# fernandezdaniel/MOBOCMF

Hardware: AMD Instinct MI355X
Metric: ELBO steps/sec (MFDGP d=8 M=512 N=8192 S=8) (higher is better)
Workload: dtype f64

## Files before the change

mobocmf_amd/csrc/api.hip:

```cpp
#include "common.h"

int launch_gram_fwd(const GramArgs& g, hipStream_t s);
int launch_gram_bwd(const GramArgs& g, bool want_dx, hipStream_t s);
void gram_grid(const GramArgs& g, dim3* grid);
int launch_sum_partials(const double* part, int64_t P, int64_t stride, double* out, int64_t len, double scale,
                        int accumulate, hipStream_t s);
int launch_potrf(double* A, int64_t ld, int Mp, int M, double* Dinv, double* Ld, int32_t* info, hipStream_t s);
int launch_trtri(const double* L, int64_t ld, int Mp, const double* Dinv, double* Linv, double* T, double* ws,
                 int64_t ws_elems, hipStream_t s);
int launch_pad_tril(const double* src, int64_t lds, int M, double* dst, int Mp, hipStream_t s);
int launch_pad_vec(const double* src, int64_t n, double* dst, int64_t np, hipStream_t s);
int launch_transpose(const double* in, int64_t ldi, double* out, int64_t ldo, int64_t rows, int64_t cols, hipStream_t s);
int launch_gemv_rows(const double* Mat, int64_t ld, const double* vec, double* out, int rows, int64_t cols, double scale,
                     int accumulate, hipStream_t s);
int launch_kl(const double* L, const double* LSp, const double* U, const double* a, int M, int Mp, double* kl,
              double* part, hipStream_t s);
int launch_moments_finish(const double* qpart, const double* mupart, const double* rpart, int nrb, int64_t Np, int64_t N,
                          const double* knn, int branch, double min_var, double* q, double* r, double* varraw,
                          double* mean, double* var, int32_t* zero_word, hipStream_t s);
int launch_moments_bwd_prep(const double* g_mean, const double* g_var, const double* knn, const double* q,
                            const double* varraw, int branch, double min_var, int64_t N, int64_t Np, double* gmu,
                            double* gv, double* gv2, double* cgv, int32_t* nclamped, int zeroed, int32_t* blkact, hipStream_t s);
int launch_reduce_slabs_sym(const double* slabs, int64_t slab_stride, int nslab, int nslab_diag, double* out, int Mp, const int32_t* flag,
                            const double* fallback, hipStream_t s);
int launch_reduce_slabs_sym2(const double* slabs, const double* slabs2, int64_t slab_stride, int nslab, int nslab_diag,
                             double* out, double* out2, int Mp, const int32_t* flag, hipStream_t s);
int launch_add_kl_terms(double* dU, const double* U, double* da, const double* a, const double* gkl, int Mp, hipStream_t s);
int launch_rank1_add(double* X, const double* u, const double* v, int Mp, hipStream_t s);
int launch_dl_from_t2(const double* T2, const double* L, const double* gkl, int M, int Mp, double* dL, hipStream_t s);
int launch_phi(const double* T3, int Mp, double* P, hipStream_t s);
int launch_symmetrize(const double* S, int Mp, double* G, hipStream_t s);
int launch_gls_out(const double* X, const double* LSp, const double* gkl, int M, int Mp, double* gLS, hipStream_t s);
int launch_copy_block(const double* src, int64_t lds, double* dst, int64_t ldd, int64_t rows, int64_t cols, hipStream_t s);
int launch_tril_inplace(double* A, int64_t ld, int n, hipStream_t s);
int launch_mf_combine(const double* Ks, const double* Kn, int64_t ld, const double* s1, const double* s2, const int32_t* l1,
                      const int32_t* l2, const double* ntab, int64_t n1, int64_t n2, double diag, double* out, int64_t ldo,
                      int64_t rows_p, int64_t cols_p, hipStream_t s);
int launch_copy_pad_identity(const double* src, int64_t lds, int n, double* dst, int np, hipStream_t s);
int launch_exact_gp_mll(const double* L, int64_t ld, const double* a, int n, double* mll, hipStream_t s);
int launch_exact_gp_finish(const double* qpart, const double* mupart, int nparts, int64_t ntp, int64_t nt, const double* kss,
                           double* mean, double* var, hipStream_t s);
int launch_mirror_lower(const double* src, int64_t lds, double* dst, int64_t ldd, int64_t row0, int64_t rows, int64_t cols,
                        int64_t n_real, hipStream_t s);
int launch_potrf_z(double* A, int64_t ld, int Mp, int M, double* Dinv, double* Ld, int32_t* const* info, int nz, int64_t zs,
                   double* zero0, double* zero1, void* sync, int* inverse_done, hipStream_t s);
int launch_chain_outputs_z(const double* X, const double* LSp, const double* LinvT, const double* da_tot, int M, int Mp,
                           const double* const* gkl, double* const* gLS, double* const* gm, int nz, int64_t zs, hipStream_t s);
int launch_pad_params_z(const double* const* LS, const double* const* m, int M, double* LSp, double* mp, int Mp, int nz,
                        int64_t zs, hipStream_t s);
int launch_trtri_z(const double* L, int64_t ld, int Mp, const double* Dinv, double* Linv, double* T, double* ws,
                   int64_t ws_elems, int nz, int64_t zs, hipStream_t s);
int launch_transpose_z(const double* in, int64_t ldi, double* out, int64_t ldo, int64_t rows, int64_t cols, int nz,
                       int64_t zs, hipStream_t s);
int launch_gemv_rows_z(const double* Mat, int64_t ld, const double* vec, double* out, int rows, int64_t cols, double scale,
                       int accumulate, int nz, int64_t zs, hipStream_t s);
int launch_transpose_pad_z(const double* in, double* out, int Mp, const double* const* LS, const double* const* m, int M,
                           double* LSp, double* mp, int nz, int64_t zs, hipStream_t s);
int launch_transpose_gemv_z(const double* in, double* out, int Mp, const double* Mat, const double* vec, double* vout, int nz,
                            int64_t zs, hipStream_t s);
int launch_kl_z(const double* L, const double* LSp, const double* U, const double* a, int M, int Mp, double* const* kl,
                double* part, int nz, int64_t zs, hipStream_t s);
int launch_dutot_y_z(const double* G1, const double* G2, const double* Hc, const double* U, const double* da, const double* a,
                     const double* const* gkl, int Mp, double* dU, double* da_tot, double* Y, int nz, int64_t zs, hipStream_t s);
int launch_dl_from_t2_z(const double* T2, const double* L, const double* const* gkl, int M, int Mp, double* dL, int nz,
                        int64_t zs, hipStream_t s);
int launch_phi_z(const double* T3, int Mp, double* P, int nz, int64_t zs, hipStream_t s);
int launch_symmetrize_z(const double* S, int Mp, double* G, int nz, int64_t zs, hipStream_t s);

static const mobocmf_tuning kDefaultTuning = {(uint32_t)sizeof(mobocmf_tuning), 384, 512, 0, 0, 1024, 32, 0, 1, 0};
static thread_local const mobocmf_tuning* t_tuning = nullptr;
static thread_local void* const* t_probe = nullptr;
const mobocmf_tuning& tune() { return t_tuning ? *t_tuning : kDefaultTuning; }
bool tuning_ok(const mobocmf_tuning* t) {
    if (!t) return true;
    return t->struct_size == sizeof(mobocmf_tuning) && t->small_gemm_max >= 1 && t->small_gemm_max <= 512 &&
           t->small_panel_max >= 1 && t->small_panel_max <= 512 && (t->tile_rows == 0 || t->tile_rows == 64 || t->tile_rows == 128) &&
           t->pair_mode >= 0 && t->pair_mode <= 2 && t->mid_gemm_max >= 0 && t->mid_gemm_max <= 4096 &&
           (t->mid_gemm_waves == 4 || t->mid_gemm_waves == 8 || t->mid_gemm_waves == 32) &&
           (t->syrk_workgroups == 0 || (t->syrk_workgroups >= 16 && t->syrk_workgroups <= 4096)) &&
           (t->sparse_backward == 0 || t->sparse_backward == 1) && (t->potrf_cols == 0 || t->potrf_cols == 1 || t->potrf_cols == 4);
}
TuneScope::TuneScope(const mobocmf_tuning* t, void* const* probe) : prev_t(t_tuning), prev_p(t_probe) {
    t_tuning = t;
    t_probe = probe;
}
TuneScope::~TuneScope() {
    t_tuning = prev_t;
    t_probe = prev_p;
}
void probe_at(int i, hipStream_t s) {
    if (t_probe && i < MOBOCMF_PROBE_EVENTS && t_probe[i]) (void)hipEventRecord((hipEvent_t)t_probe[i], s);
}
static void set_pairing(GemmArgs& g) { g.pair_mode = tune().pair_mode; }
static int panel_tile_rows(int, int64_t) { return tune().tile_rows; }

#define TRY(x)              \
    do {                    \
        int _rc = (x);      \
        if (_rc) return _rc; \
    } while (0)

namespace {

struct Bump {
    uintptr_t base;
    size_t off, cap;
    bool ok;
    Bump(void* p, size_t c) : base((uintptr_t)p), off(0), cap(c), ok(true) {}
    double* take(int64_t n) {
        size_t bytes = ((size_t)n * sizeof(double) + 255) & ~(size_t)255;
        if (bytes > cap || off > cap - bytes) { ok = false; off += bytes; return nullptr; }
        double* r = base ? (double*)(base + off) : nullptr;
        off += bytes;
        return r;
    }
};

struct Dims {
    int M, Mp, nrb, H;
    int64_t N, Np, nbase;
    int splitk;
    dim3 ggrid_mn, ggrid_mm;
};

GemmArgs gemm_args(const double* A, int64_t lda, const double* B, int64_t ldb, double* C, int64_t ldc, int Mr, int64_t Nc,
                   int64_t Kd, int tri, double alpha) {
    GemmArgs g = {};
    g.A = A; g.lda = lda; g.B = B; g.ldb = ldb; g.C = C; g.ldc = ldc;
    g.Mr = Mr; g.Nc = Nc; g.Kd = Kd; g.tri = tri; g.alpha = alpha;
    return g;
}

int syrk_splitk(int Mp, int64_t Np, int* sD) {
    const int nrb = Mp / TILE;
    const int64_t nF = (int64_t)nrb * (nrb - 1) / 2, nD = nrb, ksteps = Np / 16;
    int cap = (int)(ksteps / 8);
    if (cap > 128) cap = 128;
    if (cap < 1) cap = 1;
    *sD = 0;
    if (nF == 0) {
        int sk = 512 < cap ? 512 : cap;
        if (sk >= 8) sk &= ~7;
        return sk;
    }
    int budget = tune().syrk_workgroups;
    if (budget <= 0) budget = Np <= 16384 ? 256 : 512;
    double best = 1e30;
    int bF = 1, bD = 1;
    for (int f = 1; f <= cap; ++f)
        for (int d = 1; d <= f; ++d) {
            if (nF * f + nD * d > budget) break;
            const double cf = (double)((ksteps + f - 1) / f), cd = 0.625 * (double)((ksteps + d - 1) / d);
            double c = cf > cd ? cf : cd;
            if ((f & 7) || (d & 7)) c *= 1.10;
            c += 1e-3 * (f + d);
            if (c < best) { best = c; bF = f; bD = d; }
        }
    *sD = bD;
    return bF;
}
int64_t syrk_slab_elems(int Mp, int64_t Np) {
    int sD;
    const int sk = syrk_splitk(Mp, Np, &sD);
    return (int64_t)(sk > 16 ? sk : 16) * Mp * Mp;
}
int weighted_syrk(const double* A, int64_t lda, const double* w, int Mp, int64_t Np, double* slabs, double* H,
                  const int32_t* skip, const double* fallback, const int32_t* kact, hipStream_t s) {
    const int64_t mm = (int64_t)Mp * Mp;
    GemmArgs ga = gemm_args(A, lda, A, lda, slabs, Mp, Mp, Mp, Np, TRI_NONE, 1.0);
    ga.bscale = w; ga.lower_out = 1; ga.sym_out = 1; ga.slab_stride = mm; ga.skip_if_zero = skip;
    ga.kact = kact;
    int sD = 0;
    const int sF = syrk_splitk(Mp, Np, &sD);
    const int nsl = gemm_nt_slabs(ga, sF);
    if (gemm_nt_is_small(ga) && !skip) {
        ga.C = H; ga.ldc = Mp; ga.sym_full = 1;
        return launch_gemm(ga, true, 1, s);
    }
    if (nsl > 1) ga.splitk_diag = sD;
    TRY(launch_gemm(ga, true, nsl, s));
    return launch_reduce_slabs_sym(slabs, mm, nsl, (nsl > 1 && sD > 0) ? sD : nsl, H, Mp, skip, fallback, s);
}

int weighted_syrk_pair(const double* A, int64_t lda, const double* w, const double* w2, int Mp, int64_t Np, double* slabs,
                       double* slabs2, double* H, double* Hc, const int32_t* flag, const int32_t* kact, hipStream_t s) {
    const int64_t mm = (int64_t)Mp * Mp;
    GemmArgs ga = gemm_args(A, lda, A, lda, slabs, Mp, Mp, Mp, Np, TRI_NONE, 1.0);
    ga.bscale = w; ga.lower_out = 1; ga.sym_out = 1; ga.slab_stride = mm;
    int sD = 0;
    const int sF = syrk_splitk(Mp, Np, &sD);
    const int nsl = gemm_nt_slabs(ga, sF);
    if (gemm_nt_is_small(ga)) {
        ga.C = H; ga.ldc = Mp; ga.sym_full = 1;
        ga.bscale2 = w2; ga.C2 = Hc;
        return launch_gemm(ga, true, 1, s);
    }
    if (nsl <= 1) {
        TRY(weighted_syrk(A, lda, w, Mp, Np, slabs, H, nullptr, nullptr, kact, s));
        return weighted_syrk(A, lda, w2, Mp, Np, slabs, Hc, flag, H, kact, s);
    }
    ga.splitk_diag = sD;
    ga.dual_flag = flag; ga.bscale2 = w2; ga.C2 = slabs2; ga.kact = kact;
    TRY(launch_gemm(ga, true, nsl, s));
    return launch_reduce_slabs_sym2(slabs, slabs2, mm, nsl, sD > 0 ? sD : nsl, H, Hc, Mp, flag, s);
}

bool valid_desc(const mobocmf_layer_desc* d) {
    return d && tuning_ok(d->tuning) && (d->kind == 0 || d->kind == 1) && d->d >= 1 && d->d <= MOBOCMF_MAX_D && d->M >= 1 && d->xdiv >= 1 &&
           d->xdiv <= MOBOCMF_MAX_XDIV && d->Np >= 1 && d->Np % d->xdiv == 0 && (d->branch == 0 || d->branch == 1) && d->phase >= 0 &&
           d->phase <= MOBOCMF_PHASE_PANEL_INPUTS;
}

Dims dims_of(const mobocmf_layer_desc* d) {
    Dims D;
    D.M = d->M;
    D.Mp = (int)round_up(d->M, TILE);
    D.nrb = D.Mp / TILE;
    D.N = d->Np;
    D.Np = round_up(d->Np, TILE);
    D.nbase = d->Np / d->xdiv;
    D.H = hyp_len(d->kind, d->d);
    { int sD; D.splitk = syrk_splitk(D.Mp, D.Np, &sD); }
    GramArgs g = {};
    g.xdiv = d->xdiv;
    g.Np = D.Np;
    g.Mp = D.Mp;
    gram_grid(g, &D.ggrid_mn);
    g.xdiv = 1;
    g.Np = D.Mp;
    gram_grid(g, &D.ggrid_mm);
    return D;
}

struct ChainWs {
    double *L, *Linv, *LinvT, *U, *UT, *LSp, *a, *mp;
    double *Dinv, *Ld, *T, *ws, *klpart;
    int64_t ws_elems;
    double *H, *Hc, *da, *flag;
    double *W[8], *da_tot, *slabs, *hyp_part2, *df_part2, *dzf_part2;
    int64_t slab_elems;
};

struct PanelSaved { double *A, *C, *knn, *q, *r, *varraw; };
struct PanelFwd { double *K, *qpart, *mupart, *rpart; };
struct PanelBwd { double *gmu, *gv, *gv2, *cgv, *dA, *dK, *slabs, *slabs2, *dapart, *hyp_part, *df_part, *dzf_part, *dx_part; int64_t slab_elems; int32_t* blkact; };

void carve_chain_state(Bump& b, const Dims& D, ChainWs& S) {
    int64_t mm = (int64_t)D.Mp * D.Mp;
    S.L = b.take(mm); S.Linv = b.take(mm); S.LinvT = b.take(mm); S.U = b.take(mm); S.UT = b.take(mm); S.LSp = b.take(mm);
    S.a = b.take(D.Mp); S.mp = b.take(D.Mp);
}
void carve_panel_saved(Bump& b, const Dims& D, PanelSaved& S) {
    int64_t mn = (int64_t)D.Mp * D.Np;
    S.A = b.take(mn); S.C = b.take(mn);
    S.knn = b.take(D.Np); S.q = b.take(D.Np); S.r = b.take(D.Np); S.varraw = b.take(D.Np);
}
void carve_chain_fwd(Bump& b, const Dims& D, ChainWs& S) {
    S.Dinv = b.take((int64_t)(D.Mp / NB) * NB * NB);
    S.Ld = b.take((int64_t)(D.Mp / NB) * NB * NB);
    S.T = b.take((int64_t)D.Mp * D.Mp);
    S.ws_elems = (int64_t)16 * D.Mp * D.Mp;
    S.ws = b.take(S.ws_elems);
    S.klpart = b.take(D.Mp);
}
void carve_panel_fwd(Bump& b, const Dims& D, PanelFwd& S) {
    S.K = b.take((int64_t)D.Mp * D.Np);
    S.qpart = b.take((int64_t)4 * D.nrb * D.Np);
    S.mupart = b.take((int64_t)4 * D.nrb * D.Np);
    S.rpart = b.take((int64_t)4 * D.nrb * D.Np);
}
void carve_chain_bwd_in(Bump& b, const Dims& D, ChainWs& S) {
    int64_t mm = (int64_t)D.Mp * D.Mp;
    S.H = b.take(mm); S.Hc = b.take(mm); S.da = b.take(D.Mp); S.flag = b.take(4);
}
void carve_chain_bwd(Bump& b, const Dims& D, ChainWs& S) {
    int64_t mm = (int64_t)D.Mp * D.Mp;
    for (int i = 0; i < 8; ++i) S.W[i] = b.take(mm);
    S.da_tot = b.take(D.Mp);
    S.hyp_part2 = b.take((int64_t)D.ggrid_mm.x * D.ggrid_mm.y * hyp_len(1, MOBOCMF_MAX_D));
    S.df_part2 = b.take((int64_t)D.ggrid_mm.y * D.Mp);
    S.dzf_part2 = b.take((int64_t)D.ggrid_mm.x * D.Mp);
}
void carve_panel_bwd(Bump& b, const Dims& D, const mobocmf_layer_desc* d, PanelBwd& S) {
    int64_t mm = (int64_t)D.Mp * D.Mp, mn = (int64_t)D.Mp * D.Np;
    S.gmu = b.take(D.Np); S.gv = b.take(D.Np); S.gv2 = b.take(D.Np); S.cgv = b.take(D.Np);
    S.blkact = (int32_t*)b.take((D.Np / TILE + 1) / 2);
    S.dA = b.take(mn); S.dK = b.take(mn);
    S.slab_elems = syrk_slab_elems(D.Mp, D.Np);
    S.slabs = b.take(S.slab_elems);
    S.slabs2 = d->branch == 0 ? b.take(S.slab_elems) : nullptr;
    S.dapart = b.take((D.Np <= 8192 ? D.Np / 16 : D.Np / 64) * (int64_t)D.Mp);
    S.hyp_part = b.take((int64_t)D.ggrid_mn.x * D.ggrid_mn.y * D.H);
    S.df_part = S.dzf_part = nullptr;
    if (d->kind == 1) {
        S.df_part = b.take((int64_t)D.ggrid_mn.y * D.Np);
        S.dzf_part = b.take((int64_t)D.ggrid_mn.x * D.Mp);
    }
    S.dx_part = d->want_dx ? b.take((int64_t)D.ggrid_mn.y * D.nbase * d->d) : nullptr;
}

bool carve_single_saved(void* saved, size_t bytes, const Dims& D, ChainWs& c, PanelSaved& p, size_t* used = nullptr) {
    Bump b(saved, bytes);
    carve_chain_state(b, D, c);
    carve_panel_saved(b, D, p);
    if (used) *used = b.off;
    return b.ok;
}
bool carve_single_fwd(void* scratch, size_t bytes, const Dims& D, ChainWs& c, PanelFwd& p, size_t* used = nullptr) {
    Bump b(scratch, bytes);
    carve_chain_fwd(b, D, c);
    carve_panel_fwd(b, D, p);
    if (used) *used = b.off;
    return b.ok;
}
bool carve_single_bwd(void* scratch, size_t bytes, const Dims& D, const mobocmf_layer_desc* d, ChainWs& c, PanelBwd& p,
                      size_t* used = nullptr) {
    Bump b(scratch, bytes);
    carve_panel_bwd(b, D, d, p);
    carve_chain_bwd_in(b, D, c);
    carve_chain_bwd(b, D, c);
    c.slabs = p.slabs;
    c.slab_elems = p.slab_elems;
    if (used) *used = b.off;
    return b.ok;
}
bool carve_chain_block(void* block, size_t bytes, const Dims& D, ChainWs& c, size_t* state_bytes = nullptr,
                       size_t* used = nullptr) {
    Bump b(block, bytes);
    carve_chain_state(b, D, c);
    if (state_bytes) *state_bytes = b.off;
    carve_chain_fwd(b, D, c);
    carve_chain_bwd_in(b, D, c);
    carve_chain_bwd(b, D, c);
    c.slabs = c.ws;
    c.slab_elems = c.ws_elems;
    if (used) *used = b.off;
    return b.ok;
}

struct ChainIO {
    const mobocmf_layer_desc* const* desc;
    const double* const* Zx; const double* const* zf; const double* const* hyp;
    const double* const* m; const double* const* L_S;
    double* const* kl; int32_t* const* info;
    const double* const* g_kl; double* const* g_zf; double* const* g_hyp;
    double* const* g_m; double* const* g_LS;
};

GramArgs kmm_gram(const mobocmf_layer_desc* d, const Dims& D, const double* Zx, const double* zf, const double* hyp) {
    GramArgs g = {};
    g.kind = d->kind; g.d = d->d; g.xdiv = 1; g.zdiv = 1;
    g.x = Zx; g.f = zf; g.nbase = D.M; g.Zx = Zx; g.zf = zf; g.M = D.M; g.hyp = hyp;
    g.ldk = D.Mp; g.Mp = D.Mp; g.Np = D.Mp; g.knn = nullptr; g.jitter = d->jitter; g.is_kmm = 1;
    return g;
}

int chain_gemm(GemmArgs g, bool B_T, const ChainWs& c, int n, int64_t zs, hipStream_t s) {
    if (n > 1) { g.zlayers = n; g.zsA = g.zsB = g.zsC = zs; }
    return launch_gemm_auto(g, B_T, c.slabs, c.slab_elems, s);
}

int chain_forward(int n, const ChainWs& c, int64_t zs, const ChainIO& io, const Dims& D, hipStream_t s) {
    const int Mp = D.Mp;
    const int64_t mm = (int64_t)Mp * Mp;
    for (int z = 0; z < n; ++z) {
        GramArgs g = kmm_gram(io.desc[z], D, io.Zx[z], io.zf[z], io.hyp[z]);
        g.K = c.L + z * zs;
        TRY(launch_gram_fwd(g, s));
    }
    int inv_done = 0;
    TRY(launch_potrf_z(c.L, Mp, Mp, D.M, c.Dinv, c.Ld, io.info, n, zs, c.Linv, c.U, c.ws, &inv_done, s));
    if (!inv_done) TRY(launch_trtri_z(c.L, Mp, Mp, c.Dinv, c.Linv, c.T, c.ws, c.ws_elems, n, zs, s));
    TRY(launch_transpose_pad_z(c.Linv, c.LinvT, Mp, io.L_S, io.m, D.M, c.LSp, c.mp, n, zs, s));
    {
        GemmArgs ga = gemm_args(c.Linv, Mp, c.LSp, Mp, c.U, Mp, Mp, Mp, Mp, TRI_LOWER_A | TRI_LOWER_B, 1.0);
        ga.lower_out = 1;
        ga.Kreal = D.M;
        GemmArgs gz = ga;
        if (n > 1) { gz.zlayers = n; gz.zsA = gz.zsB = gz.zsC = zs; }
        TRY(launch_gemm_auto(gz, false, c.ws, c.ws_elems, s));
    }
    TRY(launch_transpose_gemv_z(c.U, c.UT, Mp, c.Linv, c.mp, c.a, n, zs, s));
    TRY(launch_kl_z(c.L, c.LSp, c.U, c.a, D.M, Mp, io.kl, c.klpart, n, zs, s));
    return MOBOCMF_OK;
}

int panel_forward(const mobocmf_layer_desc* desc, const Dims& D, const ChainWs& c, const PanelSaved& P, const PanelFwd& F,
                  const double* x, const double* f, const double* Zx, const double* zf, const double* hyp, double* mean,
                  double* var, bool block_layout, hipStream_t s) {
    const int Mp = D.Mp;
    const int64_t Np = D.Np;
    GramArgs g = {};
    g.kind = desc->kind; g.d = desc->d; g.zdiv = 1; g.Zx = Zx; g.zf = zf; g.M = D.M; g.hyp = hyp; g.Mp = Mp;
    g.xdiv = desc->xdiv; g.x = x; g.f = f; g.nbase = D.nbase; g.jitter = desc->jitter;
    g.K = F.K; g.ldk = Np; g.Np = Np; g.knn = P.knn; g.is_kmm = 0;
    probe_at(9, s);
    TRY(launch_gram_fwd(g, s));
    probe_at(0, s);
    GemmArgs ga = gemm_args(c.Linv, Mp, F.K, Np, P.A, Np, Mp, Np, Mp, TRI_LOWER_A, 1.0);
    ga.epi = EPI_COLSTATS; ga.colsq_part = F.qpart; ga.coldot_part = F.mupart; ga.avec = c.a;
    ga.Kreal = D.M;
    ga.rm = panel_tile_rows(Mp, Np);
    set_pairing(ga);
    TRY(launch_gemm(ga, false, 1, s));
    probe_at(1, s);
    GemmArgs gc = gemm_args(c.UT, Mp, P.A, Np, P.C, Np, Mp, Np, Mp, TRI_UPPER_A, 1.0);
    gc.epi = EPI_COLSTATS; gc.colsq_part = F.rpart; gc.coldot_part = nullptr; gc.avec = c.a;
    gc.Kreal = D.M;
    gc.stream_out = (desc->branch == 0 && Np * Mp * 8 >= ((int64_t)64 << 20)) ? 1 : 0;
    gc.rm = ga.rm; gc.pair_mode = ga.pair_mode;
    TRY(launch_gemm(gc, false, 1, s));
    probe_at(2, s);
    TRY(launch_moments_finish(F.qpart, F.mupart, F.rpart, gemm_colstat_rows(ga), Np, D.N, P.knn, desc->branch, desc->min_var, P.q, P.r,
                              P.varraw, mean, var, block_layout ? (int32_t*)c.flag : nullptr, s));
    return MOBOCMF_OK;
}

int panel_backward(const mobocmf_layer_desc* desc, const Dims& D, const ChainWs& c, const PanelSaved& P, const PanelBwd& B,
                   bool inputs_only, bool block_layout, const double* x, const double* f, const double* Zx, const double* zf,
                   const double* hyp, const double* g_mean, const double* g_var, double* g_f, double* g_zf, double* g_hyp,
                   double* g_x, hipStream_t s) {
    const int Mp = D.Mp;
    const int64_t Np = D.Np, mm = (int64_t)Mp * Mp;
    int32_t* nclamped = (int32_t*)c.flag;
    double* Hc = desc->branch != 0 ? c.H : c.Hc;
    const int32_t* act = tune().sparse_backward ? B.blkact : nullptr;
    TRY(launch_moments_bwd_prep(g_mean, g_var, P.knn, P.q, P.varraw, desc->branch, desc->min_var, D.N, Np, B.gmu, B.gv,
                                B.gv2, B.cgv, nclamped, block_layout ? 1 : 0, (int32_t*)act, s));
    int da_parts = 0;
    {
        GemmArgs ga = gemm_args(c.U, Mp, P.C, Np, B.dA, Np, Mp, Np, Mp, TRI_LOWER_A, 2.0);
        ga.bscale = B.gv; ga.epi = EPI_DA; ga.avec = c.a; ga.gmu = B.gmu; ga.cgv = B.cgv; ga.Aaux = P.A;
        ga.Kreal = D.M;
        ga.rowdot_part = inputs_only ? nullptr : B.dapart;
        ga.colact = act;
        ga.rm = panel_tile_rows(Mp, Np);
        set_pairing(ga);
        probe_at(3, s);
        TRY(launch_gemm(ga, false, 1, s));
        probe_at(4, s);
        da_parts = inputs_only ? 0 : gemm_rowdot_parts(ga);
    }
    if (!inputs_only) {
        probe_at(5, s);
        if (desc->branch == 0) TRY(weighted_syrk_pair(P.A, Np, B.gv, B.cgv, Mp, Np, B.slabs, B.slabs2, c.H, Hc, nclamped, act, s));
        else TRY(weighted_syrk(P.A, Np, B.gv, Mp, Np, B.slabs, c.H, nullptr, nullptr, act, s));
        probe_at(6, s);
    }
    {
        GemmArgs ga = gemm_args(c.LinvT, Mp, B.dA, Np, B.dK, Np, Mp, Np, Mp, TRI_UPPER_A, 1.0);
        ga.Kreal = D.M;
        ga.rm = panel_tile_rows(Mp, Np);
        set_pairing(ga);
        ga.colact = act;
        probe_at(7, s);
        TRY(launch_gemm(ga, false, 1, s));
        probe_at(8, s);
    }
    GramArgs g = {};
    g.kind = desc->kind; g.d = desc->d; g.zdiv = 1; g.Zx = Zx; g.zf = zf; g.M = D.M; g.hyp = hyp; g.Mp = Mp;
    g.xdiv = desc->xdiv; g.x = x; g.f = f; g.nbase = D.nbase;
    g.ldk = Np; g.Np = Np; g.G = B.dK; g.gknn = B.cgv; g.colact = act;
    g.hyp_part = B.hyp_part; g.df_part = B.df_part; g.dzf_part = B.dzf_part; g.dx_part = B.dx_part;
    TRY(launch_gram_bwd(g, desc->want_dx != 0, s));
    probe_at(10, s);
    SumTask tk[5];
    int nt = 0;
    if (da_parts > 0) tk[nt++] = {B.dapart, da_parts, Mp, nullptr, 0, 0, c.da, Mp, 0};
    tk[nt++] = {B.hyp_part, (int64_t)D.ggrid_mn.x * D.ggrid_mn.y, D.H, nullptr, 0, 0, g_hyp, D.H, 0};
    if (desc->kind == 1) {
        tk[nt++] = {B.df_part, D.ggrid_mn.y, Np, nullptr, 0, 0, g_f, D.N, 0};
        tk[nt++] = {B.dzf_part, D.ggrid_mn.x, Mp, nullptr, 0, 0, g_zf, D.M, 0};
    }
    if (desc->want_dx)
        tk[nt++] = {B.dx_part, D.ggrid_mn.y, D.nbase * desc->d, nullptr, 0, 0, g_x, D.nbase * desc->d, 0};
    return launch_sum_partials_multi(tk, nt, s);
}

int chain_backward(int n, const ChainWs& c, int64_t zs, const ChainIO& io, const Dims& D, const bool* zero, const int* acc,
                   const bool* fold, hipStream_t s) {
    const int Mp = D.Mp;
    const int64_t mm = (int64_t)Mp * Mp;
    double *G1 = c.W[0], *G2 = c.W[1], *X = c.W[2], *dU = c.W[3], *Y = c.W[4], *T1 = c.W[5], *T2 = c.W[6], *LT = c.W[7];
    double *dL = G1, *T4 = G2, *Gm = X;
    bool any_clamp_branch = false;
    for (int z = 0; z < n; ++z) {
        if (zero[z]) {
            TRY(launch_zero32(c.H + z * zs, mm * 2, s));
            TRY(launch_zero32(c.Hc + z * zs, mm * 2, s));
            TRY(launch_zero32(c.da + z * zs, (int64_t)Mp * 2, s));
        }
        any_clamp_branch = any_clamp_branch || io.desc[z]->branch == 0;
    }
    for (int z = 0; z < n; ++z)
        if (io.desc[z]->branch != 0 && !zero[z] && (n > 1 || any_clamp_branch))
            TRY(launch_copy_block(c.H + z * zs, Mp, c.Hc + z * zs, Mp, Mp, Mp, s));
    const double* Hc = (n == 1 && io.desc[0]->branch != 0) ? c.H : c.Hc;
    {
        GemmArgs g1 = gemm_args(c.UT, Mp, c.H, Mp, G1, Mp, Mp, Mp, Mp, TRI_UPPER_A, 1.0);
        g1.Kreal = D.M;
        TRY(chain_gemm(g1, false, c, n, zs, s));
        GemmArgs g2 = gemm_args(c.U, Mp, G1, Mp, G2, Mp, Mp, Mp, Mp, TRI_LOWER_A, 1.0);
        g2.Kreal = D.M;
        TRY(chain_gemm(g2, false, c, n, zs, s));
        TRY(launch_dutot_y_z(G1, G2, Hc, c.U, c.da, c.a, io.g_kl, Mp, dU, c.da_tot, Y, n, zs, s));
    }
    {
        GemmArgs g4 = gemm_args(dU, Mp, c.UT, Mp, Y, Mp, Mp, Mp, Mp, TRI_LOWER_A | TRI_UPPER_B, 1.0);
        g4.accumulate = 1;
        g4.Kreal = D.M;
        GemmArgs ga = gemm_args(c.LinvT, Mp, dU, Mp, T1, Mp, Mp, Mp, Mp, TRI_UPPER_A | TRI_LOWER_B, 1.0);
        ga.lower_out = 1;
        ga.Kreal = D.M;
        if (n > 1) {
            g4.zlayers = ga.zlayers = n;
            g4.zsA = g4.zsB = g4.zsC = ga.zsA = ga.zsB = ga.zsC = zs;
        }
        TRY(launch_gemm_auto_pair(g4, ga, c.slabs, c.slab_elems, s));
        TRY(launch_chain_outputs_z(T1, c.LSp, c.LinvT, c.da_tot, D.M, Mp, io.g_kl, io.g_LS, io.g_m, n, zs, s));
    }
    {
        GemmArgs ga = gemm_args(c.LinvT, Mp, Y, Mp, T2, Mp, Mp, Mp, Mp, TRI_UPPER_A, 1.0);
        ga.lower_out = 1;
        ga.Kreal = D.M;
        TRY(chain_gemm(ga, false, c, n, zs, s));
        TRY(launch_dl_from_t2_z(T2, c.L, io.g_kl, D.M, Mp, dL, n, zs, s));
    }
    {
        TRY(launch_transpose_z(c.L, Mp, LT, Mp, Mp, Mp, n, zs, s));
        GemmArgs ga = gemm_args(LT, Mp, dL, Mp, T2, Mp, Mp, Mp, Mp, TRI_UPPER_A | TRI_LOWER_B, 1.0);
        ga.Kreal = D.M;
        TRY(chain_gemm(ga, false, c, n, zs, s));
        TRY(launch_phi_z(T2, Mp, T1, n, zs, s));
        GemmArgs gb = gemm_args(c.LinvT, Mp, T1, Mp, T4, Mp, Mp, Mp, Mp, TRI_UPPER_A | TRI_LOWER_B, 1.0);
        gb.Kreal = D.M;
        TRY(chain_gemm(gb, false, c, n, zs, s));
        GemmArgs gc = gemm_args(T4, Mp, c.Linv, Mp, T2, Mp, Mp, Mp, Mp, TRI_LOWER_B, 1.0);
        gc.Kreal = D.M;
        TRY(chain_gemm(gc, false, c, n, zs, s));
        TRY(launch_symmetrize_z(T2, Mp, Gm, n, zs, s));
    }
    SumTask tk[2 * MAX_ZL];
    int nt = 0;
    for (int z = 0; z < n; ++z) {
        const mobocmf_layer_desc* d = io.desc[z];
        GramArgs g = kmm_gram(d, D, io.Zx[z], io.zf[z], io.hyp[z]);
        g.G = Gm + z * zs; g.gknn = nullptr;
        g.hyp_part = c.hyp_part2 + z * zs; g.df_part = c.df_part2 + z * zs; g.dzf_part = c.dzf_part2 + z * zs;
        g.dx_part = nullptr;
        TRY(launch_gram_bwd(g, false, s));
        const int H = hyp_len(d->kind, d->d);
        tk[nt++] = {g.hyp_part, (int64_t)D.ggrid_mm.x * D.ggrid_mm.y, H, nullptr, 0, 0, io.g_hyp[z], H, acc[z]};
        if (d->kind == 1) {
            if (fold[z])
                tk[nt++] = {g.df_part, D.ggrid_mm.y, Mp, g.dzf_part, D.ggrid_mm.x, Mp, io.g_m[z - 1], D.M, 1,
                            acc[z] ? io.g_zf[z] : nullptr};
            else
                tk[nt++] = {g.df_part, D.ggrid_mm.y, Mp, g.dzf_part, D.ggrid_mm.x, Mp, io.g_zf[z], D.M, acc[z], nullptr};
        }
    }
    return launch_sum_partials_multi(tk, nt, s);
}

bool same_chain_shape(int n, const mobocmf_layer_desc* const* d) {
    for (int z = 0; z < n; ++z)
        if (!valid_desc(d[z]) || d[z]->M != d[0]->M) return false;
    return true;
}

}

namespace {
int64_t gcd64(int64_t a, int64_t b) { while (b) { int64_t t = a % b; a = b; b = t; } return a; }
int64_t covpanel_cols(const mobocmf_layer_desc* d, int64_t Np) {
    const int64_t l = (int64_t)TILE / gcd64(TILE, d->xdiv) * d->xdiv;
    int64_t w = l * (2048 / l > 1 ? 2048 / l : 1);
    return w < Np ? w : Np;
}
struct CovWs { double *Knm, *AT, *CT, *Cv; };
bool carve_cov(void* scratch, size_t bytes, const mobocmf_layer_desc* d, const Dims& D, CovWs& w, size_t* used = nullptr) {
    Bump b(scratch, bytes);
    const int64_t nm = D.Np * D.Mp;
    w.Knm = b.take(nm); w.AT = b.take(nm); w.CT = b.take(nm);
    w.Cv = b.take(D.Np * covpanel_cols(d, D.Np));
    if (used) *used = b.off;
    return b.ok;
}
}

extern "C" {

int mobocmf_version(void) { return 200; }

int mobocmf_device_arch_ok(void) {
    int dev = 0;
    if (hipGetDevice(&dev) != hipSuccess) return 0;
    hipDeviceProp_t p;
    if (hipGetDeviceProperties(&p, dev) != hipSuccess) return 0;
    const char* a = p.gcnArchName;
    return (a[0] == 'g' && a[1] == 'f' && a[2] == 'x' && a[3] == '9' && a[4] == '5' && a[5] == '0') ? 1 : 0;
}

int mobocmf_layer_workspace_bytes(const mobocmf_layer_desc* desc, size_t* saved_bytes, size_t* scratch_bytes) {
    if (!valid_desc(desc) || !saved_bytes || !scratch_bytes) return MOBOCMF_BAD_ARG;
    TuneScope tune_scope(desc->tuning, desc->probe_events);
    Dims D = dims_of(desc);
    const size_t big = ~(size_t)0 >> 1;
    ChainWs c;
    PanelSaved P;
    PanelFwd F;
    PanelBwd B;
    size_t sv = 0, sf = 0, sb = 0;
    carve_single_saved(nullptr, big, D, c, P, &sv);
    carve_single_fwd(nullptr, big, D, c, F, &sf);
    carve_single_bwd(nullptr, big, D, desc, c, B, &sb);
    *saved_bytes = sv;
    *scratch_bytes = sf > sb ? sf : sb;
    return MOBOCMF_OK;
}

int mobocmf_layer_chain_state_bytes(const mobocmf_layer_desc* desc, size_t* bytes) {
    if (!valid_desc(desc) || !bytes) return MOBOCMF_BAD_ARG;
    TuneScope tune_scope(desc->tuning, desc->probe_events);
    Dims D = dims_of(desc);
    Bump b(nullptr, ~(size_t)0 >> 1);
    ChainWs c;
    carve_chain_state(b, D, c);
    *bytes = b.off;
    return MOBOCMF_OK;
}

int mobocmf_layer_forward(const mobocmf_layer_desc* desc, const double* x, const double* f, const double* Zx,
                          const double* zf, const double* hyp, const double* m, const double* L_S, double* mean,
                          double* var, double* kl, int32_t* info, void* saved, size_t saved_bytes, void* scratch,
                          size_t scratch_bytes, mobocmf_stream_t stream) {
    if (!valid_desc(desc) || desc->phase == MOBOCMF_PHASE_CHAIN_ONLY || !Zx || !hyp || !saved || !scratch)
        return MOBOCMF_BAD_ARG;
    TuneScope tune_scope(desc->tuning, desc->probe_events);
    const bool do_chain = desc->phase == MOBOCMF_PHASE_ALL || desc->phase == MOBOCMF_PHASE_CHAIN;
    const bool do_panel = desc->phase != MOBOCMF_PHASE_CHAIN;
    if (do_chain && (!m || !L_S || !kl || !info)) return MOBOCMF_BAD_ARG;
    if (do_panel && (!x || !mean || !var)) return MOBOCMF_BAD_ARG;
    if (desc->kind == 1 && (!zf || (do_panel && !f))) return MOBOCMF_BAD_ARG;
    hipStream_t s = (hipStream_t)stream;
    Dims D = dims_of(desc);
    ChainWs c = {};
    PanelSaved P;
    PanelFwd F;
    if (!carve_single_saved(saved, saved_bytes, D, c, P) || !carve_single_fwd(scratch, scratch_bytes, D, c, F))
        return MOBOCMF_WORKSPACE_TOO_SMALL;
    if (do_chain) {
        ChainIO io = {};
        io.desc = &desc; io.Zx = &Zx; io.zf = &zf; io.hyp = &hyp; io.m = &m; io.L_S = &L_S; io.kl = &kl; io.info = &info;
        TRY(chain_forward(1, c, 0, io, D, s));
    }
    if (!do_panel) return MOBOCMF_OK;
    return panel_forward(desc, D, c, P, F, x, f, Zx, zf, hyp, mean, var, false, s);
}

int mobocmf_layer_backward(const mobocmf_layer_desc* desc, const double* x, const double* f, const double* Zx,
                           const double* zf, const double* hyp, const double* m, const double* L_S,
                           const double* g_mean, const double* g_var, const double* g_kl, double* g_f, double* g_zf,
                           double* g_hyp, double* g_m, double* g_LS, double* g_x, void* saved, size_t saved_bytes,
                           void* scratch, size_t scratch_bytes, mobocmf_stream_t stream) {
    if (!valid_desc(desc) || !Zx || !hyp || !g_hyp || !saved || !scratch) return MOBOCMF_BAD_ARG;
    TuneScope tune_scope(desc->tuning, desc->probe_events);
    const bool inputs_only = desc->phase == MOBOCMF_PHASE_PANEL_INPUTS;
    const bool do_panel = desc->phase == MOBOCMF_PHASE_ALL || desc->phase == MOBOCMF_PHASE_PANEL || inputs_only;
    const bool do_chain = desc->phase == MOBOCMF_PHASE_ALL || desc->phase == MOBOCMF_PHASE_CHAIN ||
                          desc->phase == MOBOCMF_PHASE_CHAIN_ONLY;
    if (do_panel && (!x || !g_mean || !g_var || (desc->want_dx && !g_x))) return MOBOCMF_BAD_ARG;
    if (do_chain && (!g_kl || !g_m || !g_LS)) return MOBOCMF_BAD_ARG;
    if (desc->kind == 1 && (!zf || !g_zf || (do_panel && (!f || !g_f)))) return MOBOCMF_BAD_ARG;
    hipStream_t s = (hipStream_t)stream;
    Dims D = dims_of(desc);
    ChainWs c = {};
    PanelSaved P;
    PanelBwd B;
    if (!carve_single_saved(saved, saved_bytes, D, c, P) || !carve_single_bwd(scratch, scratch_bytes, D, desc, c, B))
        return MOBOCMF_WORKSPACE_TOO_SMALL;
    if (do_panel)
        TRY(panel_backward(desc, D, c, P, B, inputs_only, false, x, f, Zx, zf, hyp, g_mean, g_var, g_f, g_zf, g_hyp, g_x, s));
    if (!do_chain) return MOBOCMF_OK;
    ChainIO io = {};
    io.desc = &desc; io.Zx = &Zx; io.zf = &zf; io.hyp = &hyp; io.m = &m; io.L_S = &L_S;
    io.g_kl = &g_kl; io.g_zf = &g_zf; io.g_hyp = &g_hyp; io.g_m = &g_m; io.g_LS = &g_LS;
    const bool zero = desc->phase == MOBOCMF_PHASE_CHAIN_ONLY;
    const int acc = desc->phase == MOBOCMF_PHASE_ALL ? 1 : 0;
    const bool fold = false;
    return chain_backward(1, c, 0, io, D, &zero, &acc, &fold, s);
}

int mobocmf_chain_block_bytes(const mobocmf_layer_desc* desc, size_t* block_bytes, size_t* state_bytes) {
// ... 90 lines not shown
    PanelSaved P;
    PanelFwd F;
    carve_panel_saved(bs, D, P);
    carve_panel_fwd(bf, D, F);
    if (!bs.ok || !bf.ok) return MOBOCMF_WORKSPACE_TOO_SMALL;
    return panel_forward(desc, D, c, P, F, x, f, Zx, zf, hyp, mean, var, true, (hipStream_t)stream);
}

int mobocmf_layer_panel_backward(const mobocmf_layer_desc* desc, const double* x, const double* f, const double* Zx,
                                 const double* zf, const double* hyp, const double* g_mean, const double* g_var,
                                 double* g_f, double* g_zf, double* g_hyp, double* g_x, void* chain_block,
                                 size_t block_bytes, void* saved, size_t saved_bytes, void* scratch, size_t scratch_bytes,
                                 mobocmf_stream_t stream) {
    if (!valid_desc(desc) || !x || !Zx || !hyp || !g_mean || !g_var || !g_hyp || !chain_block || !saved || !scratch ||
        (desc->want_dx && !g_x))
        return MOBOCMF_BAD_ARG;
    TuneScope tune_scope(desc->tuning, desc->probe_events);
    if (desc->kind == 1 && (!zf || !f || !g_f || !g_zf)) return MOBOCMF_BAD_ARG;
    Dims D = dims_of(desc);
    ChainWs c = {};
    if (!carve_chain_block(chain_block, block_bytes, D, c)) return MOBOCMF_WORKSPACE_TOO_SMALL;
    Bump bs(saved, saved_bytes), bb(scratch, scratch_bytes);
    PanelSaved P;
    PanelBwd B;
    carve_panel_saved(bs, D, P);
    carve_panel_bwd(bb, D, desc, B);
    if (!bs.ok || !bb.ok) return MOBOCMF_WORKSPACE_TOO_SMALL;
    return panel_backward(desc, D, c, P, B, desc->phase == MOBOCMF_PHASE_PANEL_INPUTS, true, x, f, Zx, zf, hyp, g_mean, g_var,
                          g_f, g_zf, g_hyp, g_x, (hipStream_t)stream);
}

int mobocmf_predictive_covariance_workspace_bytes(const mobocmf_layer_desc* desc, size_t* scratch_bytes) {
    if (!valid_desc(desc) || !scratch_bytes) return MOBOCMF_BAD_ARG;
    TuneScope tune_scope(desc->tuning, desc->probe_events);
    Dims D = dims_of(desc);
    CovWs w;
    carve_cov(nullptr, ~(size_t)0 >> 1, desc, D, w, scratch_bytes);
    return MOBOCMF_OK;
}

int mobocmf_predictive_covariance(const mobocmf_layer_desc* desc, const double* x, const double* f, const double* Zx,
                                  const double* zf, const double* hyp, double* cov, int64_t ldcov, const void* chain_state,
                                  size_t chain_state_bytes, void* scratch, size_t scratch_bytes, mobocmf_stream_t stream) {
    if (!valid_desc(desc) || !x || !Zx || !hyp || !cov || !chain_state || !scratch || ldcov < desc->Np) return MOBOCMF_BAD_ARG;
    TuneScope tune_scope(desc->tuning, desc->probe_events);
    if (desc->kind == 1 && (!f || !zf)) return MOBOCMF_BAD_ARG;
    hipStream_t s = (hipStream_t)stream;
    Dims D = dims_of(desc);
    ChainWs cw = {};
    {
        Bump b((void*)chain_state, chain_state_bytes);
        carve_chain_state(b, D, cw);
        if (!b.ok) return MOBOCMF_WORKSPACE_TOO_SMALL;
    }
    CovWs w;
    if (!carve_cov(scratch, scratch_bytes, desc, D, w)) return MOBOCMF_WORKSPACE_TOO_SMALL;
    const int Mp = D.Mp;
    const int64_t Np = D.Np;
    if (Np > 0x7fffff80) return MOBOCMF_BAD_ARG;
    GramArgs g = {};
    g.kind = desc->kind; g.d = desc->d; g.xdiv = 1; g.zdiv = desc->xdiv;
    g.x = Zx; g.f = zf; g.nbase = D.M; g.Zx = x; g.zf = f; g.M = (int)D.N; g.hyp = hyp;
    g.K = w.Knm; g.ldk = Mp; g.Mp = (int)Np; g.Np = Mp; g.knn = nullptr; g.jitter = 0.0; g.is_kmm = 0;
    TRY(launch_gram_fwd(g, s));
    {
        GemmArgs ga = gemm_args(w.Knm, Mp, cw.Linv, Mp, w.AT, Mp, (int)Np, Mp, Mp, TRI_UPPER_B, 1.0);
        TRY(launch_gemm(ga, true, 1, s));
        GemmArgs gc = gemm_args(w.AT, Mp, cw.U, Mp, w.CT, Mp, (int)Np, Mp, Mp, TRI_LOWER_B, 1.0);
        TRY(launch_gemm(gc, false, 1, s));
    }
    const int64_t W = covpanel_cols(desc, Np);
    for (int64_t J0 = 0; J0 < Np && J0 < D.N; J0 += W) {
        const int64_t Wp = Np - J0 < W ? Np - J0 : W, R = Np - J0, b0 = J0 / desc->xdiv;
        GramArgs k = {};
        k.kind = desc->kind; k.d = desc->d; k.xdiv = desc->xdiv; k.zdiv = desc->xdiv;
        k.x = x + b0 * desc->d; k.f = f ? f + J0 : nullptr; k.nbase = D.nbase - b0;
        k.Zx = x + b0 * desc->d; k.zf = f ? f + J0 : nullptr; k.M = (int)(D.N - J0); k.hyp = hyp;
        k.K = w.Cv; k.ldk = Wp; k.Mp = (int)R; k.Np = Wp; k.knn = nullptr; k.jitter = 0.0; k.is_kmm = 0;
        TRY(launch_gram_fwd(k, s));
        GemmArgs ga = gemm_args(w.AT + J0 * Mp, Mp, w.AT + J0 * Mp, Mp, w.Cv, Wp, (int)R, Wp, Mp, TRI_NONE, -1.0);
        ga.accumulate = 1; ga.lower_out = 1;
        TRY(launch_gemm(ga, true, 1, s));
        GemmArgs gc = gemm_args(w.CT + J0 * Mp, Mp, w.CT + J0 * Mp, Mp, w.Cv, Wp, (int)R, Wp, Mp, TRI_NONE, 1.0);
        gc.accumulate = 1; gc.lower_out = 1;
        TRY(launch_gemm(gc, true, 1, s));
        TRY(launch_mirror_lower(w.Cv, Wp, cov, ldcov, J0, R, Wp, D.N, s));
    }
    return MOBOCMF_OK;
}

}

namespace {
struct ExactState { double *L, *Linv, *a, *yp; };
struct ExactFactorWs { double *Dinv, *Ld, *T, *ws; int64_t ws_elems; };
void carve_exact_state(Bump& b, int np, ExactState& S) {
    const int64_t mm = (int64_t)np * np;
    S.L = b.take(mm); S.Linv = b.take(mm); S.a = b.take(np); S.yp = b.take(np);
}
void carve_exact_factor(Bump& b, int np, ExactFactorWs& W) {
    W.Dinv = b.take((int64_t)(np / NB) * NB * NB);
    W.Ld = b.take((int64_t)(np / NB) * NB * NB);
    W.T = b.take((int64_t)np * np);
    W.ws_elems = (int64_t)16 * np * np;
    W.ws = b.take(W.ws_elems);
}
struct ExactPredictWs { double *Kp, *A, *qpart, *mupart; };
void carve_exact_predict(Bump& b, int np, int64_t ntp, ExactPredictWs& W) {
    W.Kp = b.take((int64_t)np * ntp); W.A = b.take((int64_t)np * ntp);
    W.qpart = b.take((int64_t)4 * (np / TILE) * ntp); W.mupart = b.take((int64_t)4 * (np / TILE) * ntp);
}
}

extern "C" {

int mobocmf_mf_kernel_combine(int64_t n1, int64_t n2, const double* Ks, const double* Kn, int64_t ld, const double* s1,
                              const double* s2, const int32_t* l1, const int32_t* l2, const double* ntab, double diag,
                              double* out, int64_t ldo, int64_t rows_p, int64_t cols_p, mobocmf_stream_t stream) {
    if (n1 < 1 || n2 < 1 || !Ks || !Kn || !l1 || !l2 || !ntab || !out || ld < n2 || rows_p < n1 || cols_p < n2 || ldo < cols_p)
        return MOBOCMF_BAD_ARG;
    return launch_mf_combine(Ks, Kn, ld, s1, s2, l1, l2, ntab, n1, n2, diag, out, ldo, rows_p, cols_p, (hipStream_t)stream);
}

int mobocmf_exact_gp_workspace_bytes(int32_t n, int64_t nt, size_t* state_bytes, size_t* scratch_bytes) {
    if (n < 1 || nt < 0 || !state_bytes || !scratch_bytes) return MOBOCMF_BAD_ARG;
    const int np = (int)round_up(n, TILE);
    const int64_t ntp = round_up(nt > 0 ? nt : 1, TILE);
    const size_t big = ~(size_t)0 >> 1;
    Bump bs(nullptr, big), bf(nullptr, big), bp(nullptr, big);
    ExactState S; ExactFactorWs F; ExactPredictWs P;
    carve_exact_state(bs, np, S);
    carve_exact_factor(bf, np, F);
    carve_exact_predict(bp, np, ntp, P);
    *state_bytes = bs.off;
    *scratch_bytes = bf.off > bp.off ? bf.off : bp.off;
    return MOBOCMF_OK;
}

int mobocmf_exact_gp_factor(int32_t n, const double* K, int64_t ldk, const double* y, double* mll, int32_t* info, void* state,
                            size_t state_bytes, void* scratch, size_t scratch_bytes, const mobocmf_tuning* tuning,
                            mobocmf_stream_t stream) {
    if (n < 1 || !K || ldk < n || !y || !mll || !info || !state || !scratch || !tuning_ok(tuning)) return MOBOCMF_BAD_ARG;
    TuneScope tune_scope(tuning);
    hipStream_t s = (hipStream_t)stream;
    const int np = (int)round_up(n, TILE);
    Bump bs(state, state_bytes), bf(scratch, scratch_bytes);
    ExactState S; ExactFactorWs F;
    carve_exact_state(bs, np, S);
    carve_exact_factor(bf, np, F);
    if (!bs.ok || !bf.ok) return MOBOCMF_WORKSPACE_TOO_SMALL;
    TRY(launch_copy_pad_identity(K, ldk, n, S.L, np, s));
    TRY(launch_pad_vec(y, n, S.yp, np, s));
    int inv_done = 0;
    TRY(launch_potrf_z(S.L, np, np, n, F.Dinv, F.Ld, &info, 1, 0, S.Linv, nullptr, F.ws, &inv_done, s));
    if (!inv_done) TRY(launch_trtri(S.L, np, np, F.Dinv, S.Linv, F.T, F.ws, F.ws_elems, s));
    TRY(launch_gemv_rows(S.Linv, np, S.yp, S.a, np, np, 1.0, 0, s));
    return launch_exact_gp_mll(S.L, np, S.a, n, mll, s);
}

int mobocmf_exact_gp_predict(int32_t n, int64_t nt, const double* Kts, int64_t ld, const double* kss, double* mean,
                             double* var, const void* state, size_t state_bytes, void* scratch, size_t scratch_bytes,
                             const mobocmf_tuning* tuning, mobocmf_stream_t stream) {
    if (n < 1 || nt < 1 || !Kts || ld < nt || !kss || !mean || !var || !state || !scratch || !tuning_ok(tuning)) return MOBOCMF_BAD_ARG;
    TuneScope tune_scope(tuning);
    hipStream_t s = (hipStream_t)stream;
    const int np = (int)round_up(n, TILE);
    const int64_t ntp = round_up(nt, TILE);
    Bump bs((void*)state, state_bytes), bp(scratch, scratch_bytes);
    ExactState S; ExactPredictWs P;
    carve_exact_state(bs, np, S);
    carve_exact_predict(bp, np, ntp, P);
    if (!bs.ok || !bp.ok) return MOBOCMF_WORKSPACE_TOO_SMALL;
    TRY(launch_zero32(P.Kp, (int64_t)np * ntp * 2, s));
    TRY(launch_copy_block(Kts, ld, P.Kp, ntp, n, nt, s));
    GemmArgs ga = gemm_args(S.Linv, np, P.Kp, ntp, P.A, ntp, np, ntp, np, TRI_LOWER_A, 1.0);
    ga.epi = EPI_COLSTATS; ga.colsq_part = P.qpart; ga.coldot_part = P.mupart; ga.avec = S.a;
    ga.Kreal = n;
    TRY(launch_gemm(ga, false, 1, s));
    return launch_exact_gp_finish(P.qpart, P.mupart, gemm_colstat_rows(ga), ntp, nt, kss, mean, var, s);
}

}

extern "C" {

int mobocmf_gemm_f64(int32_t tri, int32_t trans_b, int32_t Mr, int64_t Nc, int64_t Kd, const double* A, int64_t lda,
                     const double* B, int64_t ldb, double* C, int64_t ldc, double alpha, int32_t accumulate,
                     const mobocmf_tuning* tuning, mobocmf_stream_t stream) {
    if (!A || !B || !C || Mr <= 0 || Nc <= 0 || Kd <= 0 || (lda & 1) || (ldb & 1) || !tuning_ok(tuning)) return MOBOCMF_BAD_ARG;
    TuneScope tune_scope(tuning);
    GemmArgs g = gemm_args(A, lda, B, ldb, C, ldc, Mr, Nc, Kd, tri, alpha);
    g.accumulate = accumulate;
    return launch_gemm_auto(g, trans_b != 0, nullptr, 0, (hipStream_t)stream);
}

int mobocmf_gram_forward(int32_t kind, int32_t d, const double* x1, const double* f1, int64_t n1, const double* x2,
                         const double* f2, int64_t n2, const double* hyp, double* K, int64_t ldk, mobocmf_stream_t stream) {
    if ((kind != 0 && kind != 1) || d < 1 || d > MOBOCMF_MAX_D || !x1 || !x2 || !hyp || !K || n1 < 1 || n2 < 1 ||
        n1 > 0x7fffffff || ldk < n2 || (kind == 1 && (!f1 || !f2)))
        return MOBOCMF_BAD_ARG;
    GramArgs g = {};
    g.kind = kind; g.d = d; g.xdiv = 1; g.zdiv = 1;
    g.x = x2; g.f = f2; g.nbase = n2; g.Zx = x1; g.zf = f1; g.M = (int)n1; g.hyp = hyp;
    g.K = K; g.ldk = ldk; g.Mp = (int)round_up(n1, 32); g.Np = n2; g.knn = nullptr; g.jitter = 0.0; g.is_kmm = 0;
    return launch_gram_fwd(g, (hipStream_t)stream);
}

int mobocmf_gemm_f64_epilogue(int32_t tri, int32_t epi, int32_t Mr, int64_t Nc, int64_t Kd, const double* A, int64_t lda,
                              const double* B, int64_t ldb, double* C, int64_t ldc, double alpha, int32_t stream_out,
                              double* colsq_part, double* coldot_part, const double* avec, const double* bscale,
                              const double* gmu, const double* cgv, const double* Aaux, double* rowdot_part,
                              const int32_t* col_activity, const mobocmf_tuning* tuning, mobocmf_stream_t stream) {
    if (!A || !B || !C || Mr <= 0 || Nc <= 0 || Kd <= 0 || (lda & 1) || (ldb & 1) || !tuning_ok(tuning)) return MOBOCMF_BAD_ARG;
    if (epi < EPI_STORE || epi > EPI_DA) return MOBOCMF_BAD_ARG;
    if (epi == EPI_COLSTATS && (!colsq_part || !avec)) return MOBOCMF_BAD_ARG;
    if (epi == EPI_DA && (!avec || !gmu || !cgv || !Aaux)) return MOBOCMF_BAD_ARG;
    TuneScope tune_scope(tuning);
    GemmArgs g = gemm_args(A, lda, B, ldb, C, ldc, Mr, Nc, Kd, tri, alpha);
    g.epi = epi; g.stream_out = stream_out;
    g.colsq_part = colsq_part; g.coldot_part = coldot_part; g.avec = avec;
    g.bscale = epi == EPI_DA ? bscale : nullptr; g.gmu = gmu; g.cgv = cgv; g.Aaux = Aaux; g.rowdot_part = rowdot_part;
    g.rm = panel_tile_rows(Mr, Nc);
    set_pairing(g);
    g.colact = col_activity;
    return launch_gemm(g, false, 1, (hipStream_t)stream);
}

int mobocmf_gemm_colstat_rows(int32_t tri, int32_t Mr, int64_t Nc, int64_t Kd, const mobocmf_tuning* tuning, int32_t* rows) {
    if (!rows || Mr <= 0 || Nc <= 0 || Kd <= 0 || !tuning_ok(tuning)) return MOBOCMF_BAD_ARG;
    TuneScope tune_scope(tuning);
    GemmArgs g = gemm_args(nullptr, Kd, nullptr, Nc, nullptr, Nc, Mr, Nc, Kd, tri, 1.0);
    g.epi = EPI_COLSTATS;
    g.rm = panel_tile_rows(Mr, Nc);
    *rows = gemm_colstat_rows(g);
    return MOBOCMF_OK;
}

int mobocmf_syrk_workspace_bytes(int32_t Mr, int64_t Kd, const mobocmf_tuning* tuning, size_t* bytes) {
    if (!bytes || Mr <= 0 || Kd <= 0 || Mr % TILE || Kd % TILE || !tuning_ok(tuning)) return MOBOCMF_BAD_ARG;
    TuneScope tune_scope(tuning);
    *bytes = (size_t)syrk_slab_elems(Mr, Kd) * sizeof(double);
    return MOBOCMF_OK;
}

int mobocmf_syrk_weighted_f64(int32_t Mr, int64_t Kd, const double* A, int64_t lda, const double* w, double* H,
                              void* workspace, int64_t workspace_bytes, const int32_t* k_activity,
                              const mobocmf_tuning* tuning, mobocmf_stream_t stream) {
    if (!A || !w || !H || !workspace || Mr <= 0 || Kd <= 0 || Mr % TILE || Kd % TILE || (lda & 1) || !tuning_ok(tuning))
        return MOBOCMF_BAD_ARG;
    TuneScope tune_scope(tuning);
    if (workspace_bytes < syrk_slab_elems(Mr, Kd) * (int64_t)sizeof(double)) return MOBOCMF_WORKSPACE_TOO_SMALL;
    return weighted_syrk(A, lda, w, Mr, Kd, (double*)workspace, H, nullptr, nullptr, k_activity, (hipStream_t)stream);
}

int mobocmf_tuning_init(mobocmf_tuning* t) {
    if (!t) return MOBOCMF_BAD_ARG;
    *t = kDefaultTuning;
    return MOBOCMF_OK;
}

#ifdef MOBOCMF_HOST_FUZZ
static void touch(double* p, int64_t n, int* cnt) {
    if (!p || n <= 0) return;
    p[0] = 1.0;
    p[n - 1] = 2.0;
    ++*cnt;
}
int mobocmf_debug_touch_workspaces(const mobocmf_layer_desc* desc, void* saved, size_t saved_bytes, void* scratch,
                                   size_t scratch_bytes, void* block, size_t block_bytes, void* psaved, size_t psaved_bytes,
                                   void* pscratch, size_t pscratch_bytes, void* cov, size_t cov_bytes, int32_t* regions) {
    if (!valid_desc(desc) || !regions) return MOBOCMF_BAD_ARG;
    TuneScope tune_scope(desc->tuning, desc->probe_events);
    Dims D = dims_of(desc);
    const int64_t mm = (int64_t)D.Mp * D.Mp, mn = (int64_t)D.Mp * D.Np;
    int n = 0;
    auto chain_state = [&](ChainWs& c) {
        touch(c.L, mm, &n); touch(c.Linv, mm, &n); touch(c.LinvT, mm, &n); touch(c.U, mm, &n); touch(c.UT, mm, &n);
        touch(c.LSp, mm, &n); touch(c.a, D.Mp, &n); touch(c.mp, D.Mp, &n);
    };
    auto chain_fwd = [&](ChainWs& c) {
        touch(c.Dinv, (int64_t)(D.Mp / NB) * NB * NB, &n); touch(c.Ld, (int64_t)(D.Mp / NB) * NB * NB, &n);
        touch(c.T, mm, &n); touch(c.ws, c.ws_elems, &n); touch(c.klpart, D.Mp, &n);
    };
    auto chain_bwd = [&](ChainWs& c) {
        touch(c.H, mm, &n); touch(c.Hc, mm, &n); touch(c.da, D.Mp, &n); touch(c.flag, 4, &n);
        for (int i = 0; i < 8; ++i) touch(c.W[i], mm, &n);
        touch(c.da_tot, D.Mp, &n);
        touch(c.hyp_part2, (int64_t)D.ggrid_mm.x * D.ggrid_mm.y * hyp_len(1, MOBOCMF_MAX_D), &n);
        touch(c.df_part2, (int64_t)D.ggrid_mm.y * D.Mp, &n); touch(c.dzf_part2, (int64_t)D.ggrid_mm.x * D.Mp, &n);
        touch(c.slabs, c.slab_elems, &n);
    };
    auto panel_saved = [&](PanelSaved& P) {
        touch(P.A, mn, &n); touch(P.C, mn, &n); touch(P.knn, D.Np, &n); touch(P.q, D.Np, &n); touch(P.r, D.Np, &n);
        touch(P.varraw, D.Np, &n);
    };
    auto panel_fwd = [&](PanelFwd& F) {
        touch(F.K, mn, &n); touch(F.qpart, (int64_t)2 * D.nrb * D.Np, &n); touch(F.mupart, (int64_t)2 * D.nrb * D.Np, &n);
        touch(F.rpart, (int64_t)2 * D.nrb * D.Np, &n);
    };
    auto panel_bwd = [&](PanelBwd& B) {
        touch(B.gmu, D.Np, &n); touch(B.gv, D.Np, &n); touch(B.gv2, D.Np, &n); touch(B.cgv, D.Np, &n);
        touch((double*)B.blkact, (D.Np / TILE + 1) / 2, &n);
        touch(B.dA, mn, &n); touch(B.dK, mn, &n); touch(B.slabs, B.slab_elems, &n); touch(B.slabs2, B.slab_elems, &n);
        touch(B.dapart, (D.Np <= 8192 ? D.Np / 16 : D.Np / 64) * (int64_t)D.Mp, &n);
        touch(B.hyp_part, (int64_t)D.ggrid_mn.x * D.ggrid_mn.y * D.H, &n);
        if (desc->kind == 1) { touch(B.df_part, (int64_t)D.ggrid_mn.y * D.Np, &n); touch(B.dzf_part, (int64_t)D.ggrid_mn.x * D.Mp, &n); }
        if (desc->want_dx) touch(B.dx_part, (int64_t)D.ggrid_mn.y * D.nbase * desc->d, &n);
    };
    if (saved && scratch) {
        ChainWs c = {}; PanelSaved P; PanelFwd F; PanelBwd B;
        if (!carve_single_saved(saved, saved_bytes, D, c, P) || !carve_single_fwd(scratch, scratch_bytes, D, c, F))
            return MOBOCMF_WORKSPACE_TOO_SMALL;
        chain_state(c); panel_saved(P); chain_fwd(c); panel_fwd(F);
        ChainWs c2 = {};
        if (!carve_single_saved(saved, saved_bytes, D, c2, P) || !carve_single_bwd(scratch, scratch_bytes, D, desc, c2, B))
            return MOBOCMF_WORKSPACE_TOO_SMALL;
        panel_bwd(B); chain_bwd(c2);
    }
    if (block) {
        ChainWs c = {};
        if (!carve_chain_block(block, block_bytes, D, c)) return MOBOCMF_WORKSPACE_TOO_SMALL;
        chain_state(c); chain_fwd(c); chain_bwd(c);
    }
    if (psaved && pscratch) {
        Bump bs(psaved, psaved_bytes), bf(pscratch, pscratch_bytes), bb(pscratch, pscratch_bytes);
        PanelSaved P; PanelFwd F; PanelBwd B;
        carve_panel_saved(bs, D, P); carve_panel_fwd(bf, D, F); carve_panel_bwd(bb, D, desc, B);
        if (!bs.ok || !bf.ok || !bb.ok) return MOBOCMF_WORKSPACE_TOO_SMALL;
        panel_saved(P); panel_fwd(F); panel_bwd(B);
    }
    if (cov) {
        CovWs w;
        if (!carve_cov(cov, cov_bytes, desc, D, w)) return MOBOCMF_WORKSPACE_TOO_SMALL;
        touch(w.Knm, mn, &n); touch(w.AT, mn, &n); touch(w.CT, mn, &n); touch(w.Cv, D.Np * covpanel_cols(desc, D.Np), &n);
    }
    *regions = n;
    return MOBOCMF_OK;
}
#endif

int mobocmf_check_info(const int32_t* info, int32_t* pivot, mobocmf_stream_t stream) {
    int32_t h = 0;
    if (hipMemcpyAsync(&h, info, sizeof(int32_t), hipMemcpyDeviceToHost, (hipStream_t)stream) != hipSuccess)
        return MOBOCMF_HIP_ERROR;
    if (hipStreamSynchronize((hipStream_t)stream) != hipSuccess) return MOBOCMF_HIP_ERROR;
    if (pivot) *pivot = h;
    return h == 0 ? MOBOCMF_OK : MOBOCMF_NOT_PD;
}

}
```

mobocmf_amd/csrc/chol.hip:

```cpp
#include "common.h"
#include "inlaunch.h"
#include "tile16.h"
#include <cstdlib>

typedef double v4f64 __attribute__((ext_vector_type(4)));

__device__ __forceinline__ double bcast(double v, int src) {
    int lo = __builtin_amdgcn_readlane(__double2loint(v), src);
    int hi = __builtin_amdgcn_readlane(__double2hiint(v), src);
    return __hiloint2double(hi, lo);
}

typedef double v2f64c __attribute__((ext_vector_type(2)));

__device__ __forceinline__ double rsqrt_nr(double a) {
    double y = __builtin_amdgcn_rsq(a);
    y = y * (1.5 - (0.5 * a) * y * y);
    const double t = a * y;
    const double e = __builtin_fma(-t, y, 1.0);
    return __builtin_fma(0.5 * y, e, y);
}

struct InfoZ { int32_t* p[MAX_ZL]; };

// ... 731 lines not shown
            pc_load64(S1, Dinv + (int64_t)jb * NB * NB, NB, tid);
            pc_load64(S2, A + (int64_t)(jb + 1) * NB * ld + j0, ld, tid);
            if (tw == 0) {
                do_row(jb, jb + 2, true);
                if (NR == 0)
                    for (int i = jb + 3; i < nreal; ++i) do_row(jb, i, false);
            } else {
                for (int i = jb + 3 + tw - 1; i < nreal; i += NR) do_row(jb, i, false);
            }
            if (!il_barrier<2>(BART, (unsigned)NT, status, ticks, &flag)) return;
            if (tw == 0 && NI > 0) il_publish_store(XD, (unsigned long long)(jb + 1));
            const int nrem = nreal - jb - 2, ntr = nrem * (nrem + 1) / 2;
            auto task = [&](int u) {
                int b = 0, rest = u;
                while (rest >= nrem - b) { rest -= nrem - b; ++b; }
                const int ci = jb + 2 + b, ri = ci + rest;
                return PcTask{A + (int64_t)ri * NB * ld + j0, ld, A + (int64_t)ci * NB * ld + j0, ld,
                              A + (int64_t)ri * NB * ld + (int64_t)ci * NB, ld};
            };
            const int nspecial = nrem >= 2 ? 3 : 1;
            auto rest_task = [&](int v) {
                int u = v + (nrem >= 2 ? 2 : 1);
                if (nrem >= 2 && u >= nrem) ++u;
                return task(u);
            };
            if (tw == 0) {
                if (nrem >= 2) pc_tasks<true>(0, 2, 1, [&](int v) { return task(v ? nrem : 1); }, -1.0, S0, S3, tid, wr, wc, lane);
                if (NR == 0) pc_tasks<true>(0, ntr - nspecial, 1, rest_task, -1.0, S0, S3, tid, wr, wc, lane);
            } else {
                pc_tasks<true>(tw - 1, ntr - nspecial, NR, rest_task, -1.0, S0, S3, tid, wr, wc, lane);
                if (jb + 3 < nreal && !il_barrier<2>(BART + 3, (unsigned)NR, status, ticks, &flag))
                    return;
            }
        }
        return;
    }
    const int iw = w - NT - 1;
    const int64_t ldi = (int64_t)nblk * NB;
    for (int u = iw; u < nblk * nblk; u += NI) {
        const int bi = u / nblk, bj = u - bi * nblk;
        pc_gw g = (pc_gw)(Linv + (int64_t)bi * NB * ldi + (int64_t)bj * NB);
        const bool eye = bi == bj && bi >= nreal;
#pragma unroll
        for (int q = 0; q < 8; ++q) {
            const int r = (tid >> 6) + 8 * q, c = tid & 63;
            g[(int64_t)r * ldi + c] = eye && r == c ? 1.0 : 0.0;
        }
    }
    if (!il_barrier<2>(BARI, (unsigned)NI, status, ticks, &flag)) return;
    for (int jb = 0; jb < nreal; ++jb) {
        if (!il_wait_ge<2>(F, (unsigned long long)(jb + 1), status, ticks, &flag) ||
            (jb + 2 < nreal && !il_wait_ge<2>(XD, (unsigned long long)(jb + 1), status, ticks, &flag)))
            return;
        const int64_t j0 = (int64_t)jb * NB;
        pc_load64(S1, Dinv + (int64_t)jb * NB * NB, NB, tid);
        __syncthreads();
        for (int c = iw; c <= jb; c += NI) {
            double* Xc = Linv + (int64_t)jb * NB * ldi + (int64_t)c * NB;
            if (c == jb) {
#pragma unroll
                for (int q = 0; q < 8; ++q) {
                    const int r = (tid >> 6) + 8 * q, cc = tid & 63;
                    ((pc_gw)Xc)[(int64_t)r * ldi + cc] = S1[r * LD64 + cc];
                }
            } else {
                pc_load64(S0, Xc, ldi, tid);
                __syncthreads();
                v4f64 acc[2];
                pc_mm64<false>(S1, S0, acc, wr, wc, lane);
#pragma unroll
                for (int t = 0; t < 2; ++t)
#pragma unroll
                    for (int r = 0; r < 4; ++r)
                        ((pc_gw)Xc)[(int64_t)(wr * 32 + t * 16 + lk + 4 * r) * ldi + wc * 16 + li] = -acc[t][r];
                __syncthreads();
            }
        }
        if (jb + 1 == nreal) break;
        if (!il_barrier<2>(BARI, (unsigned)NI, status, ticks, &flag)) return;
        const int nc = jb + 1, ntask = (nreal - jb - 1) * nc;
        pc_tasks<false>(iw, ntask, NI,
                        [&](int u) {
                            const int i = jb + 1 + u / nc, c = u % nc;
                            return PcTask{A + (int64_t)i * NB * ld + j0, ld, Linv + (int64_t)jb * NB * ldi + (int64_t)c * NB, ldi,
                                          Linv + (int64_t)i * NB * ldi + (int64_t)c * NB, ldi};
                        },
                        1.0, S0, S3, tid, wr, wc, lane);
        if (!il_barrier<2>(BARI, (unsigned)NI, status, ticks, &flag)) return;
    }
}

__global__ void tril_inplace_kernel(double* A, int64_t ld, int n) {
    int64_t idx = (int64_t)blockIdx.x * blockDim.x + threadIdx.x;
    if (idx >= (int64_t)n * n) return;
    int i = (int)(idx / n), j = (int)(idx % n);
    if (j > i) A[(int64_t)i * ld + j] = 0.0;
}

int launch_tril_inplace(double* A, int64_t ld, int n, hipStream_t s) {
    int64_t n2 = (int64_t)n * n;
    hipLaunchKernelGGL(tril_inplace_kernel, dim3((unsigned)((n2 + 255) / 256)), dim3(256), 0, s, A, ld, n);
    return hipGetLastError() == hipSuccess ? MOBOCMF_OK : MOBOCMF_HIP_ERROR;
}

__global__ void finish_l_kernel(double* A, int64_t ld, int n, double* Ld, double* Dinv, int nreal, int64_t zs, double* z0,
                                double* z1, const unsigned long long* sync, InfoZ infoz, double* Linv) {
    int64_t idx = (int64_t)blockIdx.x * blockDim.x + threadIdx.x;
    if (idx >= (int64_t)n * n) return;
    A += blockIdx.z * zs; Ld += blockIdx.z * zs; Dinv += blockIdx.z * zs;
    if (z0) z0[blockIdx.z * zs + idx] = 0.0;
    if (z1) z1[blockIdx.z * zs + idx] = 0.0;
    int i = (int)(idx / n), j = (int)(idx % n);
    if (sync && *(const unsigned*)(sync + blockIdx.z * PC_WORDS + PC_STATUS) != 0) {
        if (idx == 0) *infoz.p[blockIdx.z] = -1;
        if (i == j) {
            const double nan = __builtin_nan("");
            A[(int64_t)i * ld + i] = nan;
            Dinv[(int64_t)(i / NB) * NB * NB + (i % NB) * (NB + 1)] = nan;
            if (Linv) Linv[blockIdx.z * zs + idx] = nan;
            return;
        }
    }
    if (i / NB == j / NB) {
        const int b = i / NB;
        const int64_t e = (int64_t)b * NB * NB + (i % NB) * NB + (j % NB);
        if (b >= nreal) {
            const double v = i == j ? 1.0 : 0.0;
            Ld[e] = v;
            Dinv[e] = v;
            A[(int64_t)i * ld + j] = v;
            return;
        }
        A[(int64_t)i * ld + j] = j > i ? 0.0 : Ld[e];
        return;
    }
    if (j > i) A[(int64_t)i * ld + j] = 0.0;
}

static void potrf_coop_workgroups(int nreal, int nz, bool inverse, int& nt, int& ni) {
    int cap = 84 / nz - 1;
    cap = cap < 15 ? 15 : cap;
    const int y0 = (nreal - 2) * (nreal - 1) / 2, z0 = inverse ? ((nreal + 1) / 2) * (nreal / 2) : 0;
    ni = z0 > 16 ? 16 : z0;
    if (ni > cap / 3 + 2) ni = cap / 3 + 2;
    nt = y0 < 1 ? 1 : y0 > 32 ? 32 : y0;
    if (nt > cap - ni) nt = cap - ni;
#ifdef PC_STAMPS
    if (const char* e = getenv("MOBOCMF_DEBUG_POTRF_NT")) nt = atoi(e);
    if (const char* e = getenv("MOBOCMF_DEBUG_POTRF_NI")) ni = inverse ? atoi(e) : 0;
#endif
}
int64_t potrf_sync_bytes(int nz) { return (int64_t)nz * PC_WORDS * 8; }

int launch_potrf_z(double* A, int64_t ld, int Mp, int M, double* Dinv, double* Ld, int32_t* const* info, int nz, int64_t zs,
                   double* zero0, double* zero1, void* sync, int* inverse_done, hipStream_t s) {
    if (inverse_done) *inverse_done = 0;
    const int nblk = Mp / NB;
    const int nreal = (M + NB - 1) / NB;
    InfoZ iz = {};
    for (int z = 0; z < nz; ++z) iz.p[z] = info[z];
    bool one_launch = false;
    double* linv = nullptr;
    if (sync && tune().potrf_cols == 0 && nreal >= 3 && nreal <= 16) {
        double* Linv = inverse_done && zero0 ? zero0 : nullptr;
        int NT = 1, NI = 0;
        potrf_coop_workgroups(nreal, nz, Linv != nullptr, NT, NI);
        const int G = 1 + NT + NI;
        const size_t shm = (size_t)PC_LDS_DOUBLES * sizeof(double);
        IlGuard gd;
        if (const int rc = il_guard((const void*)potrf_coop_kernel, PC_T, shm, (int)shm, gd)) return rc;
        if ((int64_t)G * nz <= gd.resident) {
            HIP_TRY(hipMemsetAsync(sync, 0, (size_t)potrf_sync_bytes(nz), s));
            hipLaunchKernelGGL(potrf_coop_kernel, dim3(G, nz), dim3(PC_T), shm, s, A, ld, nreal, Dinv, Ld, iz, zs,
                               (unsigned long long*)sync, Linv, Mp / NB, NT, gd.wait_ticks);
            one_launch = true;
            if (Linv) {
                *inverse_done = 1;
                linv = Linv;
                zero0 = nullptr;
            }
        }
    }
    for (int jb = 0; jb < nreal && !one_launch; ++jb) {
        int nact = M - jb * NB;
        nact = nact >= NB ? NB : (nact + 15) & ~15;
        const dim3 grid(nreal - jb, nz);
        if (nact == 16) hipLaunchKernelGGL(potrf_panel_pad_kernel<16>, grid, dim3(64), 0, s, A, ld, jb, Dinv, Ld, iz, zs);
        else if (tune().potrf_cols == 1)
            hipLaunchKernelGGL(potrf_panel2_kernel, grid, dim3(128), 0, s, A, ld, jb, Dinv, Ld, iz, zs);
        else hipLaunchKernelGGL(potrf_panel4_kernel, grid, dim3(128), 0, s, A, ld, jb, Dinv, Ld, iz, zs);
        int nt = nreal - jb - 1;
        if (nt > 0) hipLaunchKernelGGL(syrk64_update_kernel, dim3(nt, nt, nz), dim3(256), 0, s, A, ld, jb, zs);
    }
    (void)nblk;
    int64_t n2 = (int64_t)Mp * Mp;
    hipLaunchKernelGGL(finish_l_kernel, dim3((unsigned)((n2 + 255) / 256), 1, nz), dim3(256), 0, s, A, ld, Mp, Ld, Dinv, nreal,
                       zs, zero0, zero1, one_launch ? (const unsigned long long*)sync : nullptr, iz, linv);
    return hipGetLastError() == hipSuccess ? MOBOCMF_OK : MOBOCMF_HIP_ERROR;
}

int launch_potrf(double* A, int64_t ld, int Mp, int M, double* Dinv, double* Ld, int32_t* info, hipStream_t s) {
    int32_t* one[1] = {info};
    return launch_potrf_z(A, ld, Mp, M, Dinv, Ld, one, 1, 0, nullptr, nullptr, nullptr, nullptr, s);
}

__global__ __launch_bounds__(256) void trtri_level0_kernel(const double* L, int64_t ld, const double* Dinv, double* Linv,
                                                           int64_t ldi, int64_t zs) {
    const int b = blockIdx.x;
    L += blockIdx.y * zs; Dinv += blockIdx.y * zs; Linv += blockIdx.y * zs;
    __shared__ double S0[NB * LD64], S1[NB * LD64];
    const int tid = threadIdx.x, lane = tid & 63, wave = tid >> 6, wr = wave >> 1, wc = wave & 1;
    const int li = lane & 15, lk = lane >> 4;
    const double* D0 = Dinv + (int64_t)(2 * b) * NB * NB;
    const double* D1 = Dinv + (int64_t)(2 * b + 1) * NB * NB;
    const int64_t o = (int64_t)b * 128;
    load64(S0, L + (o + 64) * ld + o, ld, tid);
    load64(S1, D0, NB, tid);
    __syncthreads();
    v4f64 acc[2][2];
#pragma unroll
    for (int i = 0; i < 2; ++i)
#pragma unroll
        for (int j = 0; j < 2; ++j) acc[i][j] = (v4f64){0, 0, 0, 0};
    mm64<false>(S0, S1, acc, wr, wc, lane);
    __syncthreads();
    {
        const int r = tid >> 2, c0 = (tid & 3) * 16;
#pragma unroll
        for (int c = 0; c < 16; ++c) {
            Linv[(o + r) * ldi + o + c0 + c] = S1[r * LD64 + c0 + c];
            Linv[(o + r) * ldi + o + 64 + c0 + c] = 0.0;
        }
    }
    __syncthreads();
#pragma unroll
    for (int i = 0; i < 2; ++i)
#pragma unroll
        for (int j = 0; j < 2; ++j)
#pragma unroll
            for (int r = 0; r < 4; ++r) S0[(wr * 32 + i * 16 + lk + 4 * r) * LD64 + wc * 32 + j * 16 + li] = acc[i][j][r];
    load64(S1, D1, NB, tid);
    __syncthreads();
    {
        const int r = tid >> 2, c0 = (tid & 3) * 16;
#pragma unroll
        for (int c = 0; c < 16; ++c) Linv[(o + 64 + r) * ldi + o + 64 + c0 + c] = S1[r * LD64 + c0 + c];
    }
#pragma unroll
    for (int i = 0; i < 2; ++i)
#pragma unroll
        for (int j = 0; j < 2; ++j) acc[i][j] = (v4f64){0, 0, 0, 0};
    mm64<false>(S1, S0, acc, wr, wc, lane);
#pragma unroll
    for (int i = 0; i < 2; ++i)
#pragma unroll
        for (int j = 0; j < 2; ++j)
#pragma unroll
            for (int r = 0; r < 4; ++r)
                Linv[(o + 64 + wr * 32 + i * 16 + lk + 4 * r) * ldi + o + wc * 32 + j * 16 + li] = -acc[i][j][r];
}

int launch_trtri_z(const double* L, int64_t ld, int Mp, const double* Dinv, double* Linv, double* T, double* ws,
                   int64_t ws_elems, int nz, int64_t zs, hipStream_t s) {
    const int nb = Mp / TILE;
    const int zl = nz > 1 ? nz : 0;
    auto layered = [&](GemmArgs& g) { g.zlayers = zl; g.zsA = g.zsB = g.zsC = zs; };
    hipLaunchKernelGGL(trtri_level0_kernel, dim3(nb, nz), dim3(256), 0, s, L, ld, Dinv, Linv, (int64_t)Mp, zs);
    if ((nb & (nb - 1)) == 0) {
        for (int sz = TILE; sz < Mp; sz *= 2) {
            const int nmerge = Mp / (2 * sz);
            const int64_t bs = (int64_t)2 * sz * Mp + 2 * sz;
            GemmArgs g = {};
            g.A = L + (int64_t)sz * ld;  g.lda = ld;
            g.B = Linv;                  g.ldb = Mp;
            g.C = T + (int64_t)sz * Mp;  g.ldc = Mp;
            g.Mr = sz; g.Nc = sz; g.Kd = sz; g.tri = TRI_LOWER_B; g.alpha = 1.0;
            GemmArgs h = {};
            h.A = Linv + (int64_t)sz * Mp + sz; h.lda = Mp;
            h.B = T + (int64_t)sz * Mp;         h.ldb = Mp;
            h.C = Linv + (int64_t)sz * Mp;      h.ldc = Mp;
            h.Mr = sz; h.Nc = sz; h.Kd = sz; h.tri = TRI_LOWER_A; h.alpha = -1.0;
            layered(g);
            layered(h);
            int rc;
            if (nmerge > 1) {
                g.batched = h.batched = nmerge;
                g.strideA = (int64_t)2 * sz * ld + 2 * sz; g.strideB = bs; g.strideC = bs;
                h.strideA = bs; h.strideB = bs; h.strideC = bs;
                rc = launch_gemm(g, false, 1, s);
                if (rc) return rc;
                rc = launch_gemm(h, false, 1, s);
            } else {
                rc = launch_gemm_auto(g, false, ws, ws_elems, s);
                if (rc) return rc;
                rc = launch_gemm_auto(h, false, ws, ws_elems, s);
            }
            if (rc) return rc;
        }
        return hipGetLastError() == hipSuccess ? MOBOCMF_OK : MOBOCMF_HIP_ERROR;
    }
    for (int i = 1; i < nb; ++i) {
        GemmArgs g = {};
        g.A = L + (int64_t)i * TILE * ld;
        g.lda = ld;
        g.B = Linv;
        g.ldb = Mp;
        g.C = T;
        g.ldc = Mp;
        g.Mr = TILE;
        g.Nc = (int64_t)i * TILE;
        g.Kd = (int64_t)i * TILE;
        g.tri = TRI_LOWER_B;
        g.alpha = 1.0;
        layered(g);
        int rc = launch_gemm_auto(g, false, ws, ws_elems, s);
        if (rc) return rc;
        GemmArgs h = {};
        h.A = Linv + (int64_t)i * TILE * Mp + (int64_t)i * TILE;
        h.lda = Mp;
        h.B = T;
        h.ldb = Mp;
        h.C = Linv + (int64_t)i * TILE * Mp;
        h.ldc = Mp;
        h.Mr = TILE;
        h.Nc = (int64_t)i * TILE;
        h.Kd = TILE;
        h.alpha = -1.0;
        layered(h);
        rc = zl ? launch_gemm_auto(h, false, ws, ws_elems, s) : launch_gemm(h, false, 1, s);
        if (rc) return rc;
    }
    return hipGetLastError() == hipSuccess ? MOBOCMF_OK : MOBOCMF_HIP_ERROR;
}

int launch_trtri(const double* L, int64_t ld, int Mp, const double* Dinv, double* Linv, double* T, double* ws,
                 int64_t ws_elems, hipStream_t s) {
    return launch_trtri_z(L, ld, Mp, Dinv, Linv, T, ws, ws_elems, 1, 0, s);
}
```

mobocmf_amd/csrc/common.h:

```cpp
#pragma once
#include <hip/hip_runtime.h>
#include <stdint.h>

#include "../../include/mobocmf_hip.h"

#define TILE 128
#define NB 64

static inline int64_t round_up(int64_t v, int64_t m) { return (v + m - 1) / m * m; }

#define HIP_TRY(expr)                                   \
    do {                                                \
        hipError_t _e = (expr);                         \
        if (_e != hipSuccess) return MOBOCMF_HIP_ERROR; \
    } while (0)

const mobocmf_tuning& tune();
bool tuning_ok(const mobocmf_tuning* t);
void probe_at(int i, hipStream_t s);
struct TuneScope {
    const mobocmf_tuning* prev_t;
    void* const* prev_p;
    explicit TuneScope(const mobocmf_tuning* t, void* const* probe = nullptr);
    ~TuneScope();
    TuneScope(const TuneScope&) = delete;
    TuneScope& operator=(const TuneScope&) = delete;
};

enum { TRI_NONE = 0, TRI_LOWER_A = 1, TRI_UPPER_A = 2, TRI_LOWER_B = 4, TRI_UPPER_B = 8 };
enum { EPI_STORE = 0, EPI_COLSTATS = 1, EPI_DA = 2 };

struct GemmArgs {
    const double* A;
    const double* B;
    double* C;
    int64_t lda, ldb, ldc;
    int Mr;
    int64_t Nc;
    int64_t Kd;
    int tri;
    int lower_out;
    int sym_out;
    int sym_full;
    int splitk_diag;
    double alpha;
    int accumulate;
    int rm;
    int pair_mode;
    int64_t slab_stride;
    int64_t strideA, strideB, strideC;
    int batched;
    int zlayers;
    int64_t zsA, zsB, zsC;
    const double* bscale;
    int64_t Kreal;
    double* rowdot_part;
    int stream_out;
    const int32_t* skip_if_zero;
    const int32_t* dual_flag;
    const double* bscale2;
    double* C2;
    const int32_t* colact;
    const int32_t* kact;
    int epi;
    double* colsq_part;
    double* coldot_part;
    const double* avec;
    const double* gmu;
    const double* cgv;
    const double* Aaux;
};

int launch_gemm(const GemmArgs& g, bool B_T, int splitk, hipStream_t s);
struct SumTask {
    const double* part; int64_t P, stride;
    const double* part2; int64_t P2, stride2;
    double* out; int64_t len; int accumulate;
    const double* extra;
};
int launch_sum_partials_multi(const SumTask* tasks, int n, hipStream_t s);
int gemm_nt_slabs(const GemmArgs& g, int splitk);
bool gemm_nt_is_small(const GemmArgs& g);
int gemm_rowdot_parts(const GemmArgs& g);
int gemm_colstat_rows(const GemmArgs& g);
int launch_gemm_auto(const GemmArgs& g, bool B_T, double* ws, int64_t ws_elems, hipStream_t s);
int launch_gemm_auto_pair(const GemmArgs& a, const GemmArgs& b, double* ws, int64_t ws_elems, hipStream_t s);
int launch_reduce_slabs(const double* slabs, int64_t slab_stride, int nslab, double* out, int64_t ld, int Mr,
                        double scale, int lower_only, int accumulate, hipStream_t s);

int launch_zero32(void* ptr, int64_t nwords, hipStream_t s);
int launch_zero32_z(void* ptr, int64_t nwords, int nz, int64_t zs_bytes, hipStream_t s);
#define MAX_ZL 4

struct GramArgs {
    int kind, d, xdiv, zdiv;
    const double* x;
    const double* f;
    int64_t nbase;
    const double* Zx;
    const double* zf;
    int M;
    const double* hyp;
    double* K;
    int64_t ldk;
    int Mp;
    int64_t Np;
    double* knn;
    double jitter;
    int is_kmm;
    int gm;
    const double* G;
    const double* gknn;
    double* hyp_part;
    double* df_part;
    double* dzf_part;
    double* dx_part;
    const int32_t* colact;
};

static inline int hyp_len(int kind, int d) { return kind == 0 ? 1 + d : 5 + 2 * d; }
#define MAX_D MOBOCMF_MAX_D

__device__ __forceinline__ void philox4x32_10(uint32_t c0, uint32_t c1, uint32_t c2, uint32_t c3, uint32_t k0, uint32_t k1,
                                              uint32_t (&out)[4]) {
#pragma unroll
    for (int r = 0; r < 10; ++r) {
        const uint32_t hi0 = __umulhi(0xD2511F53u, c0), lo0 = 0xD2511F53u * c0;
        const uint32_t hi1 = __umulhi(0xCD9E8D57u, c2), lo1 = 0xCD9E8D57u * c2;
        c0 = hi1 ^ c1 ^ k0; c1 = lo1; c2 = hi0 ^ c3 ^ k1; c3 = lo0;
        k0 += 0x9E3779B9u; k1 += 0xBB67AE85u;
    }
    out[0] = c0; out[1] = c1; out[2] = c2; out[3] = c3;
}
__device__ __forceinline__ double philox_normal(uint64_t seed, uint64_t call, uint64_t idx) {
    uint32_t r[4];
    philox4x32_10((uint32_t)idx, (uint32_t)(idx >> 32), (uint32_t)call, (uint32_t)(call >> 32), (uint32_t)seed,
                  (uint32_t)(seed >> 32), r);
    const double u1 = ((double)(((uint64_t)(r[0] >> 5) << 26) | (uint64_t)(r[1] >> 6)) + 0.5) * 1.1102230246251565e-16;
    const double u2 = ((double)(((uint64_t)(r[2] >> 5) << 26) | (uint64_t)(r[3] >> 6)) + 0.5) * 1.1102230246251565e-16;
    return sqrt(-2.0 * log(u1)) * cospi(2.0 * u2);
}
__device__ __forceinline__ double philox_uniform(uint64_t seed, uint64_t call, uint64_t idx) {
    uint32_t r[4];
    philox4x32_10((uint32_t)idx, (uint32_t)(idx >> 32), (uint32_t)call, (uint32_t)(call >> 32), (uint32_t)seed,
                  (uint32_t)(seed >> 32), r);
    return ((double)(((uint64_t)(r[0] >> 5) << 26) | (uint64_t)(r[1] >> 6)) + 0.5) * 1.1102230246251565e-16;
}
```

mobocmf_amd/csrc/elementwise.hip:

```cpp
#include "common.h"

#define LOG_2PI 1.8378770664093454835606594728112

__device__ __forceinline__ double wave_sum(double v) {
    v += __shfl_xor(v, 1);
    v += __shfl_xor(v, 2);
    v += __shfl_xor(v, 4);
    v += __shfl_xor(v, 8);
    v += __shfl_xor(v, 16);
    v += __shfl_xor(v, 32);
    return v;
}

__device__ __forceinline__ double block_sum(double v, double* sh) {
    v = wave_sum(v);
    const int lane = threadIdx.x & 63, wave = threadIdx.x >> 6;
    __syncthreads();
    if (lane == 0) sh[wave] = v;
    __syncthreads();
    double t = 0.0;
    if (threadIdx.x == 0)
        for (int w = 0; w < (int)(blockDim.x >> 6); ++w) t += sh[w];
    return t;
}

__device__ __forceinline__ double block_sum_wide(double v, double* sh) {
    v = wave_sum(v);
    const int lane = threadIdx.x & 63, wave = threadIdx.x >> 6;
    __syncthreads();
    if (lane == 0) sh[wave] = v;
    __syncthreads();
    double t = 0.0;
    if (threadIdx.x == 0)
        for (int w = 0; w < (int)((blockDim.x + 63) >> 6); ++w) t += sh[w];
    return t;
}

#define GRID1(n) dim3((unsigned)(((n) + 255) / 256)), dim3(256)
#define CHECK_LAUNCH() (hipGetLastError() == hipSuccess ? MOBOCMF_OK : MOBOCMF_HIP_ERROR)

__global__ void zero32_kernel(uint32_t* p, int64_t n) {
    int64_t i = (int64_t)blockIdx.x * blockDim.x + threadIdx.x;
    if (i < n) p[i] = 0u;
}
int launch_zero32(void* ptr, int64_t nwords, hipStream_t s) {
    if (nwords <= 0) return MOBOCMF_OK;
    hipLaunchKernelGGL(zero32_kernel, GRID1(nwords), 0, s, (uint32_t*)ptr, nwords);
    return CHECK_LAUNCH();
}
#define GRIDZ(n, nz) dim3((unsigned)(((n) + 255) / 256), 1, (unsigned)(nz)), dim3(256)
struct ScalZ { const double* p[MAX_ZL]; };
__global__ void zero32_z_kernel(uint32_t* p, int64_t n, int64_t zs_words) {
    int64_t i = (int64_t)blockIdx.x * blockDim.x + threadIdx.x;
    if (i < n) p[blockIdx.z * zs_words + i] = 0u;
}
int launch_zero32_z(void* ptr, int64_t nwords, int nz, int64_t zs_bytes, hipStream_t s) {
    if (nwords <= 0) return MOBOCMF_OK;
    hipLaunchKernelGGL(zero32_z_kernel, GRIDZ(nwords, nz), 0, s, (uint32_t*)ptr, nwords, zs_bytes / 4);
    return CHECK_LAUNCH();
}

__global__ void pad_tril_kernel(const double* src, int64_t lds, int M, double* dst, int Mp) {
    int64_t idx = (int64_t)blockIdx.x * blockDim.x + threadIdx.x;
    if (idx >= (int64_t)Mp * Mp) return;
    int i = (int)(idx / Mp), j = (int)(idx % Mp);
    dst[idx] = (i < M && j <= i) ? src[(int64_t)i * lds + j] : 0.0;
}
int launch_pad_tril(const double* src, int64_t lds, int M, double* dst, int Mp, hipStream_t s) {
    hipLaunchKernelGGL(pad_tril_kernel, GRID1((int64_t)Mp * Mp), 0, s, src, lds, M, dst, Mp);
    return CHECK_LAUNCH();
}

__global__ void pad_vec_kernel(const double* src, int64_t n, double* dst, int64_t np) {
    int64_t i = (int64_t)blockIdx.x * blockDim.x + threadIdx.x;
    if (i < np) dst[i] = (src && i < n) ? src[i] : 0.0;
}
int launch_pad_vec(const double* src, int64_t n, double* dst, int64_t np, hipStream_t s) {
    hipLaunchKernelGGL(pad_vec_kernel, GRID1(np), 0, s, src, n, dst, np);
    return CHECK_LAUNCH();
}

struct PadZ { const double* LS[MAX_ZL]; const double* m[MAX_ZL]; };
__global__ void pad_params_z_kernel(PadZ t, int M, double* LSp, double* mp, int Mp, int64_t zs) {
    int64_t idx = (int64_t)blockIdx.x * blockDim.x + threadIdx.x;
    if (idx >= (int64_t)Mp * Mp) return;
    const int z = blockIdx.z;
    int i = (int)(idx / Mp), j = (int)(idx % Mp);
    LSp[z * zs + idx] = (i < M && j <= i) ? t.LS[z][(int64_t)i * M + j] : 0.0;
    if (idx < Mp) mp[z * zs + idx] = idx < M ? t.m[z][idx] : 0.0;
}
int launch_pad_params_z(const double* const* LS, const double* const* m, int M, double* LSp, double* mp, int Mp, int nz,
                        int64_t zs, hipStream_t s) {
    PadZ t = {};
    for (int z = 0; z < nz; ++z) { t.LS[z] = LS[z]; t.m[z] = m[z]; }
    hipLaunchKernelGGL(pad_params_z_kernel, GRIDZ((int64_t)Mp * Mp, nz), 0, s, t, M, LSp, mp, Mp, zs);
    return CHECK_LAUNCH();
}

__global__ void transpose_kernel(const double* in, int64_t ldi, double* out, int64_t ldo, int64_t rows, int64_t cols,
                                 int64_t zs) {
    __shared__ double t[32][33];
    in += blockIdx.z * zs;
    out += blockIdx.z * zs;
    int64_t c = (int64_t)blockIdx.x * 32 + threadIdx.x, r0 = (int64_t)blockIdx.y * 32;
    for (int k = threadIdx.y; k < 32; k += 8)
        if (r0 + k < rows && c < cols) t[k][threadIdx.x] = in[(r0 + k) * ldi + c];
    __syncthreads();
    int64_t r = r0 + threadIdx.x, c0 = (int64_t)blockIdx.x * 32;
    for (int k = threadIdx.y; k < 32; k += 8)
        if (c0 + k < cols && r < rows) out[(c0 + k) * ldo + r] = t[threadIdx.x][k];
}
int launch_transpose_z(const double* in, int64_t ldi, double* out, int64_t ldo, int64_t rows, int64_t cols, int nz,
                       int64_t zs, hipStream_t s) {
    dim3 grid((unsigned)((cols + 31) / 32), (unsigned)((rows + 31) / 32), (unsigned)nz);
    hipLaunchKernelGGL(transpose_kernel, grid, dim3(32, 8), 0, s, in, ldi, out, ldo, rows, cols, zs);
    return CHECK_LAUNCH();
}
__global__ void transpose_pad_z_kernel(const double* in, double* out, int Mp, int64_t zs, PadZ t, int M, double* LSp, double* mp) {
    __shared__ double tl[32][33];
    const int z = blockIdx.z;
    in += z * zs; out += z * zs;
    const int64_t c = (int64_t)blockIdx.x * 32 + threadIdx.x, r0 = (int64_t)blockIdx.y * 32;
    for (int k = threadIdx.y; k < 32; k += 8) {
        const int64_t i = r0 + k;
        tl[k][threadIdx.x] = in[i * Mp + c];
        LSp[z * zs + i * Mp + c] = (i < M && c <= i) ? t.LS[z][i * M + c] : 0.0;
        if (i == 0) mp[z * zs + c] = c < M ? t.m[z][c] : 0.0;
    }
    __syncthreads();
    const int64_t r = r0 + threadIdx.x, c0 = (int64_t)blockIdx.x * 32;
    for (int k = threadIdx.y; k < 32; k += 8) out[(c0 + k) * Mp + r] = tl[threadIdx.x][k];
}
int launch_transpose_pad_z(const double* in, double* out, int Mp, const double* const* LS, const double* const* m, int M,
                           double* LSp, double* mp, int nz, int64_t zs, hipStream_t s) {
    PadZ t = {};
    for (int z = 0; z < nz; ++z) { t.LS[z] = LS[z]; t.m[z] = m[z]; }
    hipLaunchKernelGGL(transpose_pad_z_kernel, dim3((unsigned)(Mp / 32), (unsigned)(Mp / 32), (unsigned)nz), dim3(32, 8), 0, s, in,
                       out, Mp, zs, t, M, LSp, mp);
    return CHECK_LAUNCH();
}
__global__ void transpose_gemv_z_kernel(const double* in, double* out, int Mp, int64_t zs, const double* Mat, const double* vec,
                                        double* vout) {
    __shared__ double tl[32][33];
    const int z = blockIdx.z;
    in += z * zs; out += z * zs; Mat += z * zs; vec += z * zs; vout += z * zs;
    const int64_t c = (int64_t)blockIdx.x * 32 + threadIdx.x, r0 = (int64_t)blockIdx.y * 32;
    for (int k = threadIdx.y; k < 32; k += 8) tl[k][threadIdx.x] = in[(r0 + k) * Mp + c];
    {
        const int tid = threadIdx.y * 32 + threadIdx.x, wave = tid >> 6, lane = tid & 63;
        const int nblk = gridDim.x * gridDim.y, b = blockIdx.y * gridDim.x + blockIdx.x;
        for (int row = 4 * b + wave; row < Mp; row += 4 * nblk) {
            const double* p = Mat + (int64_t)row * Mp;
            double sacc = 0.0;
            for (int j = lane; j < Mp; j += 64) sacc += p[j] * vec[j];
            sacc = wave_sum(sacc);
            if (lane == 0) vout[row] = sacc;
        }
    }
    __syncthreads();
    const int64_t r = r0 + threadIdx.x, c0 = (int64_t)blockIdx.x * 32;
    for (int k = threadIdx.y; k < 32; k += 8) out[(c0 + k) * Mp + r] = tl[threadIdx.x][k];
}
int launch_transpose_gemv_z(const double* in, double* out, int Mp, const double* Mat, const double* vec, double* vout, int nz,
                            int64_t zs, hipStream_t s) {
    hipLaunchKernelGGL(transpose_gemv_z_kernel, dim3((unsigned)(Mp / 32), (unsigned)(Mp / 32), (unsigned)nz), dim3(32, 8), 0, s, in,
                       out, Mp, zs, Mat, vec, vout);
    return CHECK_LAUNCH();
}
int launch_transpose(const double* in, int64_t ldi, double* out, int64_t ldo, int64_t rows, int64_t cols, hipStream_t s) {
    return launch_transpose_z(in, ldi, out, ldo, rows, cols, 1, 0, s);
}

__global__ void gemv_rows_kernel(const double* Mat, int64_t ld, const double* vec, double* out, int rows, int64_t cols,
                                 double scale, int accumulate, int64_t zs) {
    int row = blockIdx.x * 4 + (threadIdx.x >> 6);
    int lane = threadIdx.x & 63;
    if (row >= rows) return;
    Mat += blockIdx.z * zs; vec += blockIdx.z * zs; out += blockIdx.z * zs;
    const double* p = Mat + (int64_t)row * ld;
    double s = 0.0;
    for (int64_t j = lane; j < cols; j += 64) s += p[j] * vec[j];
    s = wave_sum(s) * scale;
    if (lane == 0) out[row] = accumulate ? out[row] + s : s;
}
int launch_gemv_rows_z(const double* Mat, int64_t ld, const double* vec, double* out, int rows, int64_t cols, double scale,
                       int accumulate, int nz, int64_t zs, hipStream_t s) {
    hipLaunchKernelGGL(gemv_rows_kernel, dim3((rows + 3) / 4, 1, nz), dim3(256), 0, s, Mat, ld, vec, out, rows, cols, scale,
                       accumulate, zs);
    return CHECK_LAUNCH();
}
int launch_gemv_rows(const double* Mat, int64_t ld, const double* vec, double* out, int rows, int64_t cols, double scale,
                     int accumulate, hipStream_t s) {
    return launch_gemv_rows_z(Mat, ld, vec, out, rows, cols, scale, accumulate, 1, 0, s);
}

__global__ void kl_part_kernel(const double* L, const double* LSp, const double* U, const double* a, int M, int Mp,
                               double* part, int64_t zs) {
    __shared__ double sh[4];
    double s = 0.0;
    const int r0 = blockIdx.x * 4;
    L += blockIdx.z * zs; LSp += blockIdx.z * zs; U += blockIdx.z * zs; a += blockIdx.z * zs; part += blockIdx.z * zs;
    for (int rr = 0; rr < 4; ++rr) {
        const int i = r0 + rr;
        if (i >= M) break;
        const double* u = U + (int64_t)i * Mp;
        for (int j = threadIdx.x; j <= i; j += 256) s += u[j] * u[j];
        if (threadIdx.x == 0) {
            double l = L[(int64_t)i * Mp + i], ls = LSp[(int64_t)i * Mp + i];
            s += 2.0 * log(l) - log(ls * ls) + a[i] * a[i];
        }
    }
    s = block_sum(s, sh);
    if (threadIdx.x == 0) part[blockIdx.x] = s;
}
struct KlZ { double* p[MAX_ZL]; };
__global__ void kl_final_kernel(const double* part, int np, int M, KlZ kl, int64_t zs) {
    __shared__ double sh[4];
    double s = 0.0;
    part += blockIdx.x * zs;
    for (int i = threadIdx.x; i < np; i += 256) s += part[i];
    s = block_sum(s, sh);
    if (threadIdx.x == 0) kl.p[blockIdx.x][0] = 0.5 * (s - (double)M);
}
__global__ __launch_bounds__(1024) void kl_one_kernel(const double* L, const double* LSp, const double* U, const double* a, int M,
                                                      int Mp, KlZ kl, int64_t zs) {
    __shared__ double sh[16];
    const int z = blockIdx.x;
    L += z * zs; LSp += z * zs; U += z * zs; a += z * zs;
    double s = 0.0;
    const int total = M * Mp;
#pragma unroll 4
    for (int e = threadIdx.x; e < total; e += 1024) {
        const int i = e / Mp, j = e - i * Mp;
        const double u = U[e];
        s += j <= i ? u * u : 0.0;
    }
    for (int i = threadIdx.x; i < M; i += 1024) {
        const double l = L[(int64_t)i * Mp + i], ls = LSp[(int64_t)i * Mp + i];
        s += 2.0 * log(l) - log(ls * ls) + a[i] * a[i];
    }
    s = wave_sum(s);
    if ((threadIdx.x & 63) == 0) sh[threadIdx.x >> 6] = s;
    __syncthreads();
    if (threadIdx.x == 0) {
        double t = 0.0;
        for (int w = 0; w < 16; ++w) t += sh[w];
        kl.p[z][0] = 0.5 * (t - (double)M);
    }
}
int launch_kl_z(const double* L, const double* LSp, const double* U, const double* a, int M, int Mp, double* const* kl,
                double* part, int nz, int64_t zs, hipStream_t s) {
    if (M <= 128) {
        KlZ kz1 = {};
        for (int z = 0; z < nz; ++z) kz1.p[z] = kl[z];
        hipLaunchKernelGGL(kl_one_kernel, dim3(nz), dim3(1024), 0, s, L, LSp, U, a, M, Mp, kz1, zs);
        return CHECK_LAUNCH();
    }
    const int nb = (M + 3) / 4;
    hipLaunchKernelGGL(kl_part_kernel, dim3(nb, 1, nz), dim3(256), 0, s, L, LSp, U, a, M, Mp, part, zs);
    KlZ kz = {};
    for (int z = 0; z < nz; ++z) kz.p[z] = kl[z];
    hipLaunchKernelGGL(kl_final_kernel, dim3(nz), dim3(256), 0, s, (const double*)part, nb, M, kz, zs);
    return CHECK_LAUNCH();
}
int launch_kl(const double* L, const double* LSp, const double* U, const double* a, int M, int Mp, double* kl,
              double* part, hipStream_t s) {
    double* one[1] = {kl};
    return launch_kl_z(L, LSp, U, a, M, Mp, one, part, 1, 0, s);
}

__global__ void moments_finish_kernel(const double* qpart, const double* mupart, const double* rpart, int nrb,
                                      int64_t Np, int64_t N, const double* knn, int branch, double min_var, double* q,
                                      double* r, double* varraw, double* mean, double* var, int32_t* zero_word) {
    int64_t n = (int64_t)blockIdx.x * blockDim.x + threadIdx.x;
    if (n == 0 && zero_word) zero_word[0] = 0;
    if (n >= Np) return;
    double qs = 0, ms = 0, rs = 0;
    for (int b = 0; b < nrb; ++b) {
        qs += qpart[(int64_t)b * Np + n];
        ms += mupart[(int64_t)b * Np + n];
        rs += rpart[(int64_t)b * Np + n];
    }
    double sres = knn[n] - qs;
    if (!branch && sres < 0.0) sres = 0.0;
    double v = sres + rs;
    q[n] = qs;
    r[n] = rs;
    varraw[n] = v;
    if (n < N) {
        mean[n] = ms;
        var[n] = v < min_var ? min_var : v;
    }
}
int launch_moments_finish(const double* qpart, const double* mupart, const double* rpart, int nrb, int64_t Np, int64_t N,
                          const double* knn, int branch, double min_var, double* q, double* r, double* varraw,
                          double* mean, double* var, int32_t* zero_word, hipStream_t s) {
    hipLaunchKernelGGL(moments_finish_kernel, GRID1(Np), 0, s, qpart, mupart, rpart, nrb, Np, N, knn, branch, min_var, q,
                       r, varraw, mean, var, zero_word);
    return CHECK_LAUNCH();
}

__global__ void moments_bwd_prep_kernel(const double* g_mean, const double* g_var, const double* knn, const double* q,
                                        const double* varraw, int branch, double min_var, int64_t N, int64_t Np,
                                        double* gmu, double* gv, double* gv2, double* cgv, int32_t* nclamped, int32_t* blkact) {
    __shared__ int any_w[4];
    int64_t n = (int64_t)blockIdx.x * blockDim.x + threadIdx.x;
    double gm = 0.0, g = 0.0, c = 0.0;
    if (n < N) {
        gm = g_mean ? g_mean[n] : 0.0;
        g = (g_var && varraw[n] > min_var) ? g_var[n] : 0.0;
        c = (branch || knn[n] - q[n] > 0.0) ? g : 0.0;
        if (c != g) atomicAdd(nclamped, 1);
    }
    if (n < Np) {
        gmu[n] = gm;
        gv[n] = g;
        gv2[n] = 2.0 * g;
        cgv[n] = c;
    }
    if (blkact) {
        const bool any = !(gm == 0.0) || !(g == 0.0);
        const unsigned long long b = __ballot(any);
        if ((threadIdx.x & 63) == 0) any_w[threadIdx.x >> 6] = b != 0ull ? 1 : 0;
        __syncthreads();
        if (threadIdx.x < 2) {
            const int64_t blk = (int64_t)blockIdx.x * 2 + threadIdx.x;
            if (blk * 128 < Np) blkact[blk] = any_w[2 * threadIdx.x] | any_w[2 * threadIdx.x + 1];
        }
    }
}
int launch_moments_bwd_prep(const double* g_mean, const double* g_var, const double* knn, const double* q,
                            const double* varraw, int branch, double min_var, int64_t N, int64_t Np, double* gmu,
                            double* gv, double* gv2, double* cgv, int32_t* nclamped, int zeroed, int32_t* blkact, hipStream_t s) {
    if (!zeroed && launch_zero32(nclamped, 1, s)) return MOBOCMF_HIP_ERROR;
    hipLaunchKernelGGL(moments_bwd_prep_kernel, GRID1(Np), 0, s, g_mean, g_var, knn, q, varraw, branch, min_var, N, Np,
                       gmu, gv, gv2, cgv, nclamped, blkact);
    return CHECK_LAUNCH();
}

__device__ __forceinline__ double slab_sum(const double* p, int64_t slab_stride, int ns) {
    double v = 0.0;
    int z = 0;
    for (; z + 8 <= ns; z += 8) {
        double t[8];
#pragma unroll
        for (int b = 0; b < 8; ++b) t[b] = p[(z + b) * slab_stride];
#pragma unroll
        for (int b = 0; b < 8; ++b) v += t[b];
    }
    for (; z < ns; ++z) v += p[z * slab_stride];
    return v;
}

__global__ void reduce_slabs_sym_kernel(const double* slabs, int64_t slab_stride, int nslab, int nslab_diag, double* out,
                                        int Mp, const int32_t* flag, const double* fallback) {
    int64_t idx = (int64_t)blockIdx.x * blockDim.x + threadIdx.x;
    if (idx >= (int64_t)Mp * Mp) return;
    int i = (int)(idx / Mp), j = (int)(idx % Mp);
    if (flag && *flag == 0) {
        out[idx] = fallback[idx];
        return;
    }
    if (j / TILE > i / TILE) return;
    const double* p = j > i ? slabs + (int64_t)j * Mp + i : slabs + (int64_t)i * Mp + j;
    const int ns = (i / TILE == j / TILE) ? nslab_diag : nslab;
    const double v = slab_sum(p, slab_stride, ns);
    out[idx] = v;
    if (j / TILE < i / TILE) out[(int64_t)j * Mp + i] = v;
}
__global__ void reduce_slabs_sym2_kernel(const double* slabs, const double* slabs2, int64_t slab_stride, int nslab,
                                         int nslab_diag, double* out, double* out2, int Mp, const int32_t* flag) {
    int64_t idx = (int64_t)blockIdx.x * blockDim.x + threadIdx.x;
    if (idx >= (int64_t)Mp * Mp) return;
    int i = (int)(idx / Mp), j = (int)(idx % Mp);
    if (j / TILE > i / TILE) return;
    const int64_t off = j > i ? (int64_t)j * Mp + i : (int64_t)i * Mp + j;
    const int ns = (i / TILE == j / TILE) ? nslab_diag : nslab;
    const double v = slab_sum(slabs + off, slab_stride, ns);
    double v2 = v;
    if (*flag != 0) v2 = slab_sum(slabs2 + off, slab_stride, ns);
    out[idx] = v;
    out2[idx] = v2;
    if (j / TILE < i / TILE) { out[(int64_t)j * Mp + i] = v; out2[(int64_t)j * Mp + i] = v2; }
}
int launch_reduce_slabs_sym2(const double* slabs, const double* slabs2, int64_t slab_stride, int nslab, int nslab_diag,
                             double* out, double* out2, int Mp, const int32_t* flag, hipStream_t s) {
    hipLaunchKernelGGL(reduce_slabs_sym2_kernel, GRID1((int64_t)Mp * Mp), 0, s, slabs, slabs2, slab_stride, nslab, nslab_diag,
                       out, out2, Mp, flag);
    return CHECK_LAUNCH();
}
int launch_reduce_slabs_sym(const double* slabs, int64_t slab_stride, int nslab, int nslab_diag, double* out, int Mp,
                            const int32_t* flag, const double* fallback, hipStream_t s) {
    hipLaunchKernelGGL(reduce_slabs_sym_kernel, GRID1((int64_t)Mp * Mp), 0, s, slabs, slab_stride, nslab, nslab_diag, out, Mp,
                       flag, fallback);
    return CHECK_LAUNCH();
}

__global__ void dutot_y_kernel(const double* G1, const double* G2, const double* Hc, const double* U, const double* da,
                               const double* a, ScalZ gklz, int Mp, double* dU, double* da_tot, double* Y, int64_t zs) {
    __shared__ double tl[32][33];
    const double* gkl = gklz.p[blockIdx.z];
    const double g = gkl ? gkl[0] : 0.0;
    const int64_t zo = blockIdx.z * zs;
    G1 += zo; G2 += zo; Hc += zo; U += zo; da += zo; a += zo; dU += zo; da_tot += zo; Y += zo;
    const int nt = Mp / 32, ti = blockIdx.x / nt, tj = blockIdx.x % nt;
    const int tx = threadIdx.x & 31, ty = threadIdx.x >> 5;
    if (tj <= ti) {
#pragma unroll
        for (int r = ty; r < 32; r += 8) tl[r][tx] = G1[(int64_t)(tj * 32 + r) * Mp + ti * 32 + tx];
    }
    __syncthreads();
#pragma unroll
    for (int r = ty; r < 32; r += 8) {
        const int i = ti * 32 + r, j = tj * 32 + tx;
        const int64_t idx = (int64_t)i * Mp + j;
        const double ai = a[i], aj = a[j], dai = da[i], daj = da[j];
        dU[idx] = j <= i ? 2.0 * tl[tx][r] + g * U[idx] : 0.0;
        Y[idx] = 2.0 * (G2[idx] - Hc[idx]) + ai * daj + (dai + g * ai) * aj;
        if (tj == 0 && tx == 0) da_tot[i] = dai + g * ai;
    }
}
int launch_dutot_y_z(const double* G1, const double* G2, const double* Hc, const double* U, const double* da, const double* a,
                     const double* const* gkl, int Mp, double* dU, double* da_tot, double* Y, int nz, int64_t zs, hipStream_t s) {
    ScalZ t = {};
    for (int z = 0; z < nz; ++z) t.p[z] = gkl[z];
    const int nt = Mp / 32;
    hipLaunchKernelGGL(dutot_y_kernel, dim3((unsigned)(nt * nt), 1, (unsigned)nz), dim3(256), 0, s, G1, G2, Hc, U, da, a, t, Mp,
                       dU, da_tot, Y, zs);
    return CHECK_LAUNCH();
}


__global__ void add_kl_terms_kernel(double* dU, const double* U, double* da, const double* a, const double* gkl, int Mp) {
    int64_t idx = (int64_t)blockIdx.x * blockDim.x + threadIdx.x;
    const double g = gkl ? gkl[0] : 0.0;
    if (idx < (int64_t)Mp * Mp) dU[idx] += g * U[idx];
    if (idx < Mp) da[idx] += g * a[idx];
}
int launch_add_kl_terms(double* dU, const double* U, double* da, const double* a, const double* gkl, int Mp, hipStream_t s) {
    hipLaunchKernelGGL(add_kl_terms_kernel, GRID1((int64_t)Mp * Mp), 0, s, dU, U, da, a, gkl, Mp);
    return CHECK_LAUNCH();
}

__global__ void rank1_add_kernel(double* X, const double* u, const double* v, int Mp) {
    int64_t idx = (int64_t)blockIdx.x * blockDim.x + threadIdx.x;
    if (idx >= (int64_t)Mp * Mp) return;
    int i = (int)(idx / Mp), j = (int)(idx % Mp);
    X[idx] += u[i] * v[j];
}
int launch_rank1_add(double* X, const double* u, const double* v, int Mp, hipStream_t s) {
    hipLaunchKernelGGL(rank1_add_kernel, GRID1((int64_t)Mp * Mp), 0, s, X, u, v, Mp);
    return CHECK_LAUNCH();
}

__global__ void dl_from_t2_kernel(const double* T2, const double* L, ScalZ gklz, int M, int Mp, double* dL, int64_t zs) {
    int64_t idx = (int64_t)blockIdx.x * blockDim.x + threadIdx.x;
    if (idx >= (int64_t)Mp * Mp) return;
    const double* gkl = gklz.p[blockIdx.z];
    T2 += blockIdx.z * zs; L += blockIdx.z * zs; dL += blockIdx.z * zs;
    int i = (int)(idx / Mp), j = (int)(idx % Mp);
    double v = 0.0;
    if (i < M && j <= i) {
        v = -T2[idx];
        if (i == j && gkl) v += gkl[0] / L[idx];
    }
    dL[idx] = v;
}
int launch_dl_from_t2_z(const double* T2, const double* L, const double* const* gkl, int M, int Mp, double* dL, int nz,
                        int64_t zs, hipStream_t s) {
    ScalZ t = {};
    for (int z = 0; z < nz; ++z) t.p[z] = gkl[z];
    hipLaunchKernelGGL(dl_from_t2_kernel, GRIDZ((int64_t)Mp * Mp, nz), 0, s, T2, L, t, M, Mp, dL, zs);
    return CHECK_LAUNCH();
}
int launch_dl_from_t2(const double* T2, const double* L, const double* gkl, int M, int Mp, double* dL, hipStream_t s) {
    const double* one[1] = {gkl};
    return launch_dl_from_t2_z(T2, L, one, M, Mp, dL, 1, 0, s);
}

__global__ void phi_kernel(const double* T3, int Mp, double* P, int64_t zs) {
    int64_t idx = (int64_t)blockIdx.x * blockDim.x + threadIdx.x;
    if (idx >= (int64_t)Mp * Mp) return;
    T3 += blockIdx.z * zs; P += blockIdx.z * zs;
    int i = (int)(idx / Mp), j = (int)(idx % Mp);
    P[idx] = j < i ? T3[idx] : (j == i ? 0.5 * T3[idx] : 0.0);
}
int launch_phi_z(const double* T3, int Mp, double* P, int nz, int64_t zs, hipStream_t s) {
    hipLaunchKernelGGL(phi_kernel, GRIDZ((int64_t)Mp * Mp, nz), 0, s, T3, Mp, P, zs);
    return CHECK_LAUNCH();
}
int launch_phi(const double* T3, int Mp, double* P, hipStream_t s) { return launch_phi_z(T3, Mp, P, 1, 0, s); }

__global__ void symmetrize_kernel(const double* S, int Mp, double* G, int64_t zs) {
    int64_t idx = (int64_t)blockIdx.x * blockDim.x + threadIdx.x;
    if (idx >= (int64_t)Mp * Mp) return;
    S += blockIdx.z * zs; G += blockIdx.z * zs;
    int i = (int)(idx / Mp), j = (int)(idx % Mp);
    G[idx] = 0.5 * (S[idx] + S[(int64_t)j * Mp + i]);
}
int launch_symmetrize_z(const double* S, int Mp, double* G, int nz, int64_t zs, hipStream_t s) {
    hipLaunchKernelGGL(symmetrize_kernel, GRIDZ((int64_t)Mp * Mp, nz), 0, s, S, Mp, G, zs);
    return CHECK_LAUNCH();
}
int launch_symmetrize(const double* S, int Mp, double* G, hipStream_t s) { return launch_symmetrize_z(S, Mp, G, 1, 0, s); }

__global__ void gls_out_kernel(const double* X, const double* LSp, const double* gkl, int M, int Mp, double* gLS) {
    int64_t idx = (int64_t)blockIdx.x * blockDim.x + threadIdx.x;
    if (idx >= (int64_t)M * M) return;
    int i = (int)(idx / M), j = (int)(idx % M);
    double v = 0.0;
    if (j <= i) {
        v = X[(int64_t)i * Mp + j];
        if (i == j && gkl) v -= gkl[0] / LSp[(int64_t)i * Mp + i];
    }
    gLS[idx] = v;
}
int launch_gls_out(const double* X, const double* LSp, const double* gkl, int M, int Mp, double* gLS, hipStream_t s) {
    hipLaunchKernelGGL(gls_out_kernel, GRID1((int64_t)M * M), 0, s, X, LSp, gkl, M, Mp, gLS);
    return CHECK_LAUNCH();
}

struct ChainOutZ { const double* gkl[MAX_ZL]; double* gLS[MAX_ZL]; double* gm[MAX_ZL]; };
__global__ void chain_outputs_z_kernel(const double* X, const double* LSp, const double* LinvT, const double* da_tot, int M,
                                       int Mp, ChainOutZ t, int nb_ls, int64_t zs) {
    const int z = blockIdx.y;
    X += z * zs; LSp += z * zs; LinvT += z * zs; da_tot += z * zs;
    if ((int)blockIdx.x < nb_ls) {
        const int64_t idx = (int64_t)blockIdx.x * blockDim.x + threadIdx.x;
        if (idx >= (int64_t)M * M) return;
        const int i = (int)(idx / M), j = (int)(idx % M);
        double v = 0.0;
        if (j <= i) {
            v = X[(int64_t)i * Mp + j];
            if (i == j && t.gkl[z]) v -= t.gkl[z][0] / LSp[(int64_t)i * Mp + i];
        }
        t.gLS[z][idx] = v;
        return;
    }
    const int row = ((int)blockIdx.x - nb_ls) * 4 + (threadIdx.x >> 6), lane = threadIdx.x & 63;
    if (row >= M) return;
    const double* p = LinvT + (int64_t)row * Mp;
    double sacc = 0.0;
    for (int j = lane; j < Mp; j += 64) sacc += p[j] * da_tot[j];
    sacc = wave_sum(sacc);
    if (lane == 0) t.gm[z][row] = sacc;
}
int launch_chain_outputs_z(const double* X, const double* LSp, const double* LinvT, const double* da_tot, int M, int Mp,
                           const double* const* gkl, double* const* gLS, double* const* gm, int nz, int64_t zs, hipStream_t s) {
    ChainOutZ t = {};
    for (int z = 0; z < nz; ++z) { t.gkl[z] = gkl[z]; t.gLS[z] = gLS[z]; t.gm[z] = gm[z]; }
    const int nb_ls = (int)(((int64_t)M * M + 255) / 256), nb_m = (M + 3) / 4;
    hipLaunchKernelGGL(chain_outputs_z_kernel, dim3((unsigned)(nb_ls + nb_m), (unsigned)nz), dim3(256), 0, s, X, LSp, LinvT, da_tot,
                       M, Mp, t, nb_ls, zs);
    return CHECK_LAUNCH();
}

__global__ void copy_block_kernel(const double* src, int64_t lds, double* dst, int64_t ldd, int64_t rows, int64_t cols) {
    int64_t idx = (int64_t)blockIdx.x * blockDim.x + threadIdx.x;
    if (idx >= rows * cols) return;
    int64_t i = idx / cols, j = idx % cols;
    dst[i * ldd + j] = src[i * lds + j];
}
int launch_copy_block(const double* src, int64_t lds, double* dst, int64_t ldd, int64_t rows, int64_t cols, hipStream_t s) {
    hipLaunchKernelGGL(copy_block_kernel, GRID1(rows * cols), 0, s, src, lds, dst, ldd, rows, cols);
    return CHECK_LAUNCH();
}

__global__ __launch_bounds__(256) void mirror_lower_kernel(const double* src, int64_t lds_, double* dst, int64_t ldd,
                                                           int64_t row0, int64_t rows, int64_t cols, int64_t n_real) {
    __shared__ double t[32][33];
    const int64_t ti = blockIdx.y, tj = blockIdx.x;
    if (tj > ti) return;
    const int tx = threadIdx.x & 31, ty = threadIdx.x >> 5;
    for (int r = ty; r < 32; r += 8) {
        const int64_t i = ti * 32 + r, j = tj * 32 + tx;
        double v = 0.0;
        if (i < rows && j < cols) v = src[i * lds_ + j];
        t[r][tx] = v;
        if (i >= j && row0 + i < n_real && row0 + j < n_real && j < cols) dst[(row0 + i) * ldd + row0 + j] = v;
    }
    __syncthreads();
    for (int r = ty; r < 32; r += 8) {
        const int64_t j = tj * 32 + r, i = ti * 32 + tx;
        if (i > j && row0 + i < n_real && row0 + j < n_real && j < cols && i < rows) dst[(row0 + j) * ldd + row0 + i] = t[tx][r];
    }
}
int launch_mirror_lower(const double* src, int64_t lds_, double* dst, int64_t ldd, int64_t row0, int64_t rows, int64_t cols,
                        int64_t n_real, hipStream_t s) {
    const dim3 grid((unsigned)((cols + 31) / 32), (unsigned)((rows + 31) / 32));
    hipLaunchKernelGGL(mirror_lower_kernel, grid, dim3(256), 0, s, src, lds_, dst, ldd, row0, rows, cols, n_real);
    return CHECK_LAUNCH();
}

__global__ void mf_combine_kernel(const double* Ks, const double* Kn, int64_t ld, const double* s1, const double* s2,
                                  const int32_t* l1, const int32_t* l2, const double* ntab, int64_t n1, int64_t n2,
                                  double diag, double* out, int64_t ldo, int64_t rows_p, int64_t cols_p) {
    const int64_t idx = (int64_t)blockIdx.x * blockDim.x + threadIdx.x;
    if (idx >= rows_p * cols_p) return;
    const int64_t i = idx / cols_p, j = idx % cols_p;
    double v = 0.0;
    if (i < n1 && j < n2) {
        const int a = l1[i], b = l2[j];
        v = (s1 ? s1[i] : 1.0) * (s2 ? s2[j] : 1.0) * Ks[i * ld + j] + ntab[a < b ? a : b] * Kn[i * ld + j];
        if (i == j) v += diag;
    } else if (i == j && diag != 0.0) {
        v = 1.0;
    }
    out[i * ldo + j] = v;
}
int launch_mf_combine(const double* Ks, const double* Kn, int64_t ld, const double* s1, const double* s2, const int32_t* l1,
                      const int32_t* l2, const double* ntab, int64_t n1, int64_t n2, double diag, double* out, int64_t ldo,
                      int64_t rows_p, int64_t cols_p, hipStream_t s) {
    hipLaunchKernelGGL(mf_combine_kernel, GRID1(rows_p * cols_p), 0, s, Ks, Kn, ld, s1, s2, l1, l2, ntab, n1, n2, diag, out,
                       ldo, rows_p, cols_p);
    return CHECK_LAUNCH();
}
__global__ void copy_pad_identity_kernel(const double* src, int64_t lds_, int n, double* dst, int np) {
    const int64_t idx = (int64_t)blockIdx.x * blockDim.x + threadIdx.x;
    if (idx >= (int64_t)np * np) return;
    const int i = (int)(idx / np), j = (int)(idx % np);
    dst[idx] = (i < n && j < n) ? src[(int64_t)i * lds_ + j] : (i == j ? 1.0 : 0.0);
}
int launch_copy_pad_identity(const double* src, int64_t lds_, int n, double* dst, int np, hipStream_t s) {
    hipLaunchKernelGGL(copy_pad_identity_kernel, GRID1((int64_t)np * np), 0, s, src, lds_, n, dst, np);
    return CHECK_LAUNCH();
}
__global__ void exact_gp_mll_kernel(const double* L, int64_t ld, const double* a, int n, double* mll) {
    __shared__ double sh[4];
    double s = 0.0;
    for (int i = threadIdx.x; i < n; i += blockDim.x) s += -0.5 * a[i] * a[i] - log(L[(int64_t)i * ld + i]);
    s = block_sum(s, sh);
    if (threadIdx.x == 0) mll[0] = s - 0.5 * n * 1.8378770664093453;
}
int launch_exact_gp_mll(const double* L, int64_t ld, const double* a, int n, double* mll, hipStream_t s) {
    hipLaunchKernelGGL(exact_gp_mll_kernel, dim3(1), dim3(256), 0, s, L, ld, a, n, mll);
    return CHECK_LAUNCH();
}
__global__ void exact_gp_finish_kernel(const double* qpart, const double* mupart, int nparts, int64_t ntp, int64_t nt,
                                       const double* kss, double* mean, double* var) {
    const int64_t j = (int64_t)blockIdx.x * blockDim.x + threadIdx.x;
    if (j >= nt) return;
    double q = 0.0, m = 0.0;
    for (int p = 0; p < nparts; ++p) { q += qpart[(int64_t)p * ntp + j]; m += mupart[(int64_t)p * ntp + j]; }
    mean[j] = m;
    var[j] = kss[j] - q;
}
int launch_exact_gp_finish(const double* qpart, const double* mupart, int nparts, int64_t ntp, int64_t nt, const double* kss,
                           double* mean, double* var, hipStream_t s) {
    hipLaunchKernelGGL(exact_gp_finish_kernel, GRID1(nt), 0, s, qpart, mupart, nparts, ntp, nt, kss, mean, var);
    return CHECK_LAUNCH();
}

__global__ void propagate_fwd_kernel(const double* mean, const double* var, const double* eps, double* f, int64_t n,
                                     int div) {
    int64_t i = (int64_t)blockIdx.x * blockDim.x + threadIdx.x;
    if (i >= n) return;
    int64_t b = i / div;
    f[i] = mean[b] + sqrt(var[b]) * eps[i];
}
__global__ void propagate_rng_fwd_kernel(const double* mean, const double* var, int64_t* rng_state, double* f, double* eps_out,
                                         int64_t n, int div) {
    const uint64_t seed = (uint64_t)rng_state[0], call = (uint64_t)__atomic_load_n(&rng_state[1], __ATOMIC_RELAXED);
    const int64_t i = (int64_t)blockIdx.x * blockDim.x + threadIdx.x;
    if (i < n) {
        const int64_t b = i / div;
        const double e = philox_normal(seed, call, (uint64_t)i);
        eps_out[i] = e;
        f[i] = mean[b] + sqrt(var[b]) * e;
    }
    __syncthreads();
    if (threadIdx.x == 0) {
        const unsigned long long t = atomicAdd((unsigned long long*)&rng_state[2], 1ull);
        if (t == (unsigned long long)gridDim.x - 1) {
            __atomic_store_n(&rng_state[2], (int64_t)0, __ATOMIC_RELAXED);
            __atomic_store_n(&rng_state[1], (int64_t)(call + 1), __ATOMIC_RELAXED);
        }
    }
}
__global__ void propagate_bwd_kernel(const double* var, const double* eps, const double* gf, double* gmean, double* gvar,
                                     int64_t nbase, int div, int64_t nprev, const double* add_mean, const double* add_var) {
    int64_t b = (int64_t)blockIdx.x * blockDim.x + threadIdx.x;
    if (b >= nprev) return;
    const double am = add_mean ? add_mean[b] : 0.0, av = add_var ? add_var[b] : 0.0;
    if (b >= nbase) {
        gmean[b] = am;
        gvar[b] = av;
        return;
    }
    double sm = 0.0, sv = 0.0;
    for (int s = 0; s < div; ++s) {
        double g = gf[b * div + s];
        sm += g;
        sv += g * eps[b * div + s];
    }
    gmean[b] = sm + am;
    gvar[b] = sv * 0.5 / sqrt(var[b]) + av;
}

__device__ __forceinline__ double elp_term(double y, double mu, double v, double tau, double ltau) {
    double dlt = y - mu;
    return -0.5 * ((dlt * dlt + v) / tau + ltau + LOG_2PI);
}
__global__ void elbo_fwd_kernel(const double* mean, const double* var, const double* y, const double* fid,
                                const double* tau_p, double lo, double hi, double level, int64_t n, int div, double* part) {
    __shared__ double sh[4];
    const double tau = hi > lo ? lo + (hi - lo) / (1.0 + exp(-tau_p[0])) : tau_p[0], ltau = log(tau);
// ... 818 lines not shown
```

mobocmf_amd/csrc/gemm_f64.hip:

```cpp
#include "common.h"
#include <type_traits>
#include <atomic>

typedef double v4f64 __attribute__((ext_vector_type(4)));
typedef double v2f64 __attribute__((ext_vector_type(2)));

#define BM 128
#define BN 128
#define BK 16
#define KL_MAX 1024
#define TILE_ELEMS (BM * BK)

#ifndef GEMM_MI
#define GEMM_MI 16
#endif
#if GEMM_MI == 16
#define IMG_SWZ(row) ((((row) >> 1) & 1) | ((((row) >> 3) & 1) << 2))
#else
#define IMG_SWZ(row) ((((row) >> 1) & 1) << 2)
#endif


template <int CTRL>
__device__ __forceinline__ double dpp_mov(double v) {
// ... 1156 lines not shown
        __syncthreads();                                                                                    \
          \
        MD_FETCH(((ST) + 2 < nst ? (ST) + 2 : nst - 1), RA, RB)                                             \
              \
        MD_LOADF(0, fa0, fb0)                                                                               \
        MD_LOADF(1, fa1, fb1) MD_MMA(fa0, fb0) __builtin_amdgcn_sched_barrier(0);                           \
        MD_LOADF(2, fa0, fb0) MD_MMA(fa1, fb1) __builtin_amdgcn_sched_barrier(0);                           \
        MD_LOADF(3, fa1, fb1) MD_MMA(fa0, fb0) __builtin_amdgcn_sched_barrier(0);                           \
        MD_MMA(fa1, fb1)                                                                                    \
    }
    v2f64 fa0[2][4], fa1[2][4];
    double fb0[2][2], fb1[2][2];
#define MD_LOADF(G, FA, FB)                                                                                 \
    {                                                                                                       \
        constexpr int kq = ((G) >> 1) * 16 + ((G) & 1) * 2;       \
        if (B_T) {                                                                                          \
            _Pragma("unroll") for (int nt = 0; nt < 2; ++nt) {                                             \
                const v2f64 v = *(const v2f64*)(Bs + bt_off + nt * MD_LDA + kq);                            \
                FB[0][nt] = v[0];                                                                           \
                FB[1][nt] = v[1];                                                                           \
            }                                                                                               \
        } else {                                                                                            \
            _Pragma("unroll") for (int e = 0; e < 2; ++e) {                                                \
                const v2f64 v = *(const v2f64*)(Bs + bn_off + (kq + e) * MD_LDB);                           \
                FB[e][0] = v[0];                                                                            \
                FB[e][1] = v[1];                                                                            \
            }                                                                                               \
        }                                                                                                   \
        _Pragma("unroll") for (int mt = 0; mt < 2; ++mt)                                                   \
            _Pragma("unroll") for (int r = 0; r < 4; ++r)                                                  \
                FA[mt][r] = *(const v2f64*)(As + a_off + (mt * 32 + 4 * r) * MD_LDA + kq);                  \
    }
#define MD_MMA(FA, FB)                                                                                      \
    _Pragma("unroll") for (int e = 0; e < 2; ++e)                                                          \
        _Pragma("unroll") for (int mt = 0; mt < 2; ++mt)                                                   \
            _Pragma("unroll") for (int r = 0; r < 4; ++r)                                                  \
                _Pragma("unroll") for (int nt = 0; nt < 2; ++nt)                                           \
                    acc[mt][nt][r] = __builtin_amdgcn_mfma_f64_4x4x4f64(FA[mt][r][e], FB[e][nt], acc[mt][nt][r], 0, 0, 0);
    int st = 0;
    for (; st + 1 < nst; st += 2) {
        MD_STAGE(st, ra0, rb0)
        MD_STAGE(st + 1, ra1, rb1)
    }
    if (st < nst) MD_STAGE(st, ra0, rb0)
#undef MD_STAGE
#undef MD_FETCH
#undef MD_LOADF
#undef MD_MMA
    double* cp = C + ((int64_t)rb * MD_BM + wr * 16 + lk) * g.ldc + (int64_t)cb * MD_BN + wc * 32 + 2 * li;
#pragma unroll
    for (int mt = 0; mt < 2; ++mt)
#pragma unroll
        for (int r = 0; r < 4; ++r) {
            double* q = cp + (int64_t)(mt * 32 + 4 * r) * g.ldc;
            v2f64 v = (v2f64){g.alpha * acc[mt][0][r], g.alpha * acc[mt][1][r]};
            if (g.accumulate) v += *(const v2f64*)q;
            *(v2f64*)q = v;
        }
}

template <bool B_T>
__device__ __forceinline__ void gemm_mid8_body(const GemmArgs& g, int nrb, int ncb) {
    __shared__ __attribute__((aligned(16))) double As[MD_BM * MD_LDA];
    __shared__ __attribute__((aligned(16))) double Bs[B_T ? MD_BN * MD_LDA : MD_BK * MD_LDB];
    const int tid = threadIdx.x, lane = tid & 63, wave = tid >> 6;
    const int wr = wave >> 2, wc = wave & 3, li = lane & 15, lk = lane >> 4;
    const int rb = nrb - 1 - (int)(blockIdx.x / ncb), cb = (int)(blockIdx.x % ncb);
    if (g.lower_out && cb > (rb | 1)) return;
    const int z = blockIdx.z;
    const double* A = g.A + (g.zlayers > 1 ? z * g.zsA : 0);
    const double* B = g.B + (g.zlayers > 1 ? z * g.zsB : 0);
    double* C = g.C + (g.zlayers > 1 ? z * g.zsC : 0);
    int64_t k0 = 0, k1 = g.Kd;
    if (g.Kreal > 0) { const int64_t ke = (g.Kreal + MD_BK - 1) / MD_BK * MD_BK; if (k1 > ke) k1 = ke; }
    if (g.tri & TRI_LOWER_A) { const int64_t e = (int64_t)(rb + 1) * MD_BM; if (k1 > e) k1 = e; }
    if (g.tri & TRI_UPPER_A) { const int64_t b = (int64_t)rb * MD_BM; if (k0 < b) k0 = b; }
    if (g.tri & TRI_LOWER_B) { const int64_t b = (int64_t)cb * MD_BN; if (k0 < b) k0 = b; }
    if (g.tri & TRI_UPPER_B) { const int64_t e = (int64_t)(cb + 1) * MD_BN; if (k1 > e) k1 = e; }
    const int nst = k1 > k0 ? (int)((k1 - k0) / MD_BK) : 0;
    const int ar = tid >> 3, ak = (tid & 7) * 4;
    const int bk = tid >> 4, bc = (tid & 15) * 4;
    const double* Ag = A + ((int64_t)rb * MD_BM + ar) * g.lda + ak;
    const double* Bg = B_T ? B + ((int64_t)cb * MD_BN + ar) * g.ldb + ak : B + (int64_t)bk * g.ldb + (int64_t)cb * MD_BN + bc;
    v2f64 ra[2], rbv[2];
    auto fetch = [&](int st) {
        const int64_t k = k0 + (int64_t)st * MD_BK;
        ra[0] = *(const v2f64*)(Ag + k);
        ra[1] = *(const v2f64*)(Ag + k + 2);
        const double* bp = B_T ? Bg + k : Bg + k * g.ldb;
        rbv[0] = *(const v2f64*)bp;
        rbv[1] = *(const v2f64*)(bp + 2);
    };
    v4f64 acc[2];
    acc[0] = acc[1] = (v4f64){0.0, 0.0, 0.0, 0.0};
    if (nst > 0) fetch(0);
    const int a_off = (wr * 16 + (lane & 3)) * MD_LDA + 4 * lk;
    const int bn_off = (4 * lk) * MD_LDB + wc * 16 + li;
    const int bt_off = (wc * 16 + li) * MD_LDA + 4 * lk;
    for (int st = 0; st < nst; ++st) {
        __syncthreads();
        *(v2f64*)(As + ar * MD_LDA + ak) = ra[0];
        *(v2f64*)(As + ar * MD_LDA + ak + 2) = ra[1];
        if (B_T) {
            *(v2f64*)(Bs + ar * MD_LDA + ak) = rbv[0];
            *(v2f64*)(Bs + ar * MD_LDA + ak + 2) = rbv[1];
        } else {
            *(v2f64*)(Bs + bk * MD_LDB + bc) = rbv[0];
            *(v2f64*)(Bs + bk * MD_LDB + bc + 2) = rbv[1];
        }
        __syncthreads();
        if (st + 1 < nst) fetch(st + 1);
#pragma unroll
        for (int G = 0; G < 4; ++G) {
            const int kq = (G >> 1) * 16 + (G & 1) * 2;
            double fb[2];
            if (B_T) {
                const v2f64 v = *(const v2f64*)(Bs + bt_off + kq);
                fb[0] = v[0];
                fb[1] = v[1];
            } else {
                fb[0] = Bs[bn_off + kq * MD_LDB];
                fb[1] = Bs[bn_off + (kq + 1) * MD_LDB];
            }
            v2f64 fa[2][4];
#pragma unroll
            for (int mt = 0; mt < 2; ++mt)
#pragma unroll
                for (int r = 0; r < 4; ++r) fa[mt][r] = *(const v2f64*)(As + a_off + (mt * 32 + 4 * r) * MD_LDA + kq);
#pragma unroll
            for (int e = 0; e < 2; ++e)
#pragma unroll
                for (int mt = 0; mt < 2; ++mt)
#pragma unroll
                    for (int r = 0; r < 4; ++r)
                        acc[mt][r] = __builtin_amdgcn_mfma_f64_4x4x4f64(fa[mt][r][e], fb[e], acc[mt][r], 0, 0, 0);
        }
    }
    double* cp = C + ((int64_t)rb * MD_BM + wr * 16 + lk) * g.ldc + (int64_t)cb * MD_BN + wc * 16 + li;
#pragma unroll
    for (int mt = 0; mt < 2; ++mt)
#pragma unroll
        for (int r = 0; r < 4; ++r) {
            double* q = cp + (int64_t)(mt * 32 + 4 * r) * g.ldc;
            double v = g.alpha * acc[mt][r];
            if (g.accumulate) v += *q;
            *q = v;
        }
}

#define MS_BM 32
#define MS_BK 64
#define MS_LDA (MS_BK + 2)
#define MS_ASWZ(row) ((((row) & 1) << 1) | ((((row) >> 1) & 1) << 4))
template <bool B_T>
__device__ __forceinline__ void gemm_mid32_body(const GemmArgs& g, int nrb, int ncb) {
    __shared__ __attribute__((aligned(16))) double As[MS_BM * MS_BK];
    __shared__ __attribute__((aligned(16))) double Bs[B_T ? MD_BN * MS_LDA : MS_BK * MD_LDB];
    const int tid = threadIdx.x, lane = tid & 63, wave = tid >> 6;
    const int wr = wave >> 1, wc = wave & 1, li = lane & 15, lk = lane >> 4;
    const int rb = nrb - 1 - (int)(blockIdx.x / ncb), cb = (int)(blockIdx.x % ncb);
    if (g.lower_out && cb > (rb >> 1 | 1)) return;
    const int z = blockIdx.z;
    const double* A = g.A + (g.zlayers > 1 ? z * g.zsA : 0);
    const double* B = g.B + (g.zlayers > 1 ? z * g.zsB : 0);
    double* C = g.C + (g.zlayers > 1 ? z * g.zsC : 0);
    int64_t k0 = 0, k1 = g.Kd;
    if (g.Kreal > 0) { const int64_t ke = (g.Kreal + MS_BK - 1) / MS_BK * MS_BK; if (k1 > ke) k1 = ke; }
    if (g.tri & TRI_LOWER_A) { const int64_t e = (int64_t)(rb / 2 + 1) * 64; if (k1 > e) k1 = e; }
    if (g.tri & TRI_UPPER_A) { const int64_t b = (int64_t)(rb / 2) * 64; if (k0 < b) k0 = b; }
    if (g.tri & TRI_LOWER_B) { const int64_t b = (int64_t)cb * MD_BN; if (k0 < b) k0 = b; }
    if (g.tri & TRI_UPPER_B) { const int64_t e = (int64_t)(cb + 1) * MD_BN; if (k1 > e) k1 = e; }
    const int nst = k1 > k0 ? (int)((k1 - k0) / MS_BK) : 0;
    const int fr = tid >> 5, fc = (tid & 31) * 2;
    const double* Ag = A + ((int64_t)rb * MS_BM + fr) * g.lda + fc;
    const double* Bg = B_T ? B + ((int64_t)cb * MD_BN + fr) * g.ldb + fc : B + (int64_t)fr * g.ldb + (int64_t)cb * MD_BN + fc;
    v2f64 ra[4], rbv[8];
    auto fetch = [&](int st) {
        const int64_t k = k0 + (int64_t)st * MS_BK;
        const double* bp = B_T ? Bg + k : Bg + k * g.ldb;
#pragma unroll
        for (int i = 0; i < 4; ++i) ra[i] = *(const v2f64*)(Ag + (int64_t)(8 * i) * g.lda + k);
#pragma unroll
        for (int i = 0; i < 8; ++i) rbv[i] = *(const v2f64*)(bp + (int64_t)(8 * i) * g.ldb);
    };
    v4f64 acc[2];
    acc[0] = acc[1] = (v4f64){0.0, 0.0, 0.0, 0.0};
    if (nst > 0) fetch(0);
    const int a_row = (wr * 16 + (lane & 3)) * MS_BK, a_swz = MS_ASWZ(lane);
    const int bn_off = (4 * lk) * MD_LDB + wc * 32 + 2 * li;
    const int bt_off = (wc * 32 + 2 * li) * MS_LDA + 4 * lk;
    for (int st = 0; st < nst; ++st) {
        __syncthreads();
#pragma unroll
        for (int i = 0; i < 4; ++i) *(v2f64*)(As + (fr + 8 * i) * MS_BK + (fc ^ MS_ASWZ(fr))) = ra[i];
#pragma unroll
        for (int i = 0; i < 8; ++i) *(v2f64*)(Bs + (fr + 8 * i) * (B_T ? MS_LDA : MD_LDB) + fc) = rbv[i];
        __syncthreads();
        fetch(st + 1 < nst ? st + 1 : st);
        v2f64 fa[2][4];
        v2f64 fb[2][2];
        auto frag = [&](auto SET, int gi) {
            constexpr int S = decltype(SET)::value;
            const int kk = 16 * (gi >> 1) + 2 * (gi & 1);
            if (B_T) {
#pragma unroll
                for (int nt = 0; nt < 2; ++nt) fb[S][nt] = *(const v2f64*)(Bs + bt_off + nt * MS_LDA + kk);
            } else {
#pragma unroll
                for (int e = 0; e < 2; ++e) fb[S][e] = *(const v2f64*)(Bs + bn_off + (kk + e) * MD_LDB);
            }
#pragma unroll
            for (int r = 0; r < 4; ++r) fa[S][r] = *(const v2f64*)(As + a_row + (4 * r) * MS_BK + ((4 * lk + kk) ^ a_swz));
        };
        auto mma = [&](auto SET) {
            constexpr int S = decltype(SET)::value;
#pragma unroll
            for (int e = 0; e < 2; ++e)
#pragma unroll
                for (int r = 0; r < 4; ++r)
#pragma unroll
                    for (int nt = 0; nt < 2; ++nt)
                        acc[nt][r] = __builtin_amdgcn_mfma_f64_4x4x4f64(fa[S][r][e], B_T ? fb[S][nt][e] : fb[S][e][nt], acc[nt][r], 0, 0, 0);
        };
        using I0 = std::integral_constant<int, 0>;
        using I1 = std::integral_constant<int, 1>;
        frag(I0{}, 0);
#pragma unroll
        for (int gp = 0; gp < 4; ++gp) {
            frag(I1{}, 2 * gp + 1);
            __builtin_amdgcn_sched_barrier(0);
            mma(I0{});
            __builtin_amdgcn_sched_barrier(0);
            if (gp < 3) frag(I0{}, 2 * gp + 2);
            __builtin_amdgcn_sched_barrier(0);
            mma(I1{});
            __builtin_amdgcn_sched_barrier(0);
        }
    }
    double* cp = C + ((int64_t)rb * MS_BM + wr * 16 + lk) * g.ldc + (int64_t)cb * MD_BN + wc * 32 + 2 * li;
#pragma unroll
    for (int r = 0; r < 4; ++r) {
        double* q = cp + (int64_t)(4 * r) * g.ldc;
        v2f64 v = (v2f64){g.alpha * acc[0][r], g.alpha * acc[1][r]};
        if (g.accumulate) v += *(const v2f64*)q;
        *(v2f64*)q = v;
    }
}
template <bool B_T>
__global__ __launch_bounds__(256) void gemm_mid32_kernel(GemmArgs g, int nrb, int ncb) {
    gemm_mid32_body<B_T>(g, nrb, ncb);
}
__global__ __launch_bounds__(256) void gemm_mid32x2_kernel(GemmArgs g0, GemmArgs g1, int nrb, int ncb) {
    if (blockIdx.y == 0) gemm_mid32_body<false>(g0, nrb, ncb);
    else gemm_mid32_body<false>(g1, nrb, ncb);
}

template <bool B_T>
__global__ __launch_bounds__(256) void gemm_mid_kernel(GemmArgs g, int nrb, int ncb) {
    gemm_mid_body<B_T>(g, nrb, ncb);
}
template <bool B_T>
__global__ __launch_bounds__(512) void gemm_mid8_kernel(GemmArgs g, int nrb, int ncb) {
    gemm_mid8_body<B_T>(g, nrb, ncb);
}
__global__ __launch_bounds__(512) void gemm_mid8x2_kernel(GemmArgs g0, GemmArgs g1, int nrb, int ncb) {
    if (blockIdx.y == 0) gemm_mid8_body<false>(g0, nrb, ncb);
    else gemm_mid8_body<false>(g1, nrb, ncb);
}
__global__ __launch_bounds__(256) void gemm_mid2_kernel(GemmArgs g0, GemmArgs g1, int nrb, int ncb) {
    if (blockIdx.y == 0) gemm_mid_body<false>(g0, nrb, ncb);
    else gemm_mid_body<false>(g1, nrb, ncb);
}

static bool mid_gemm_ok(const GemmArgs& g) {
    const int L = tune().mid_gemm_max;
    return g.epi == EPI_STORE && g.batched <= 1 && !g.bscale && !g.skip_if_zero && !g.sym_out && !g.dual_flag && !g.colact &&
           !g.kact && g.Mr <= L && g.Nc <= L && g.Kd <= L && g.Mr % MD_BM == 0 && g.Nc % MD_BN == 0 && g.Kd % MD_BK == 0 &&
           !(g.lda & 1) && !(g.ldb & 1) && !(g.ldc & 1) && !((uintptr_t)g.A & 15) && !((uintptr_t)g.B & 15) &&
           !((uintptr_t)g.C & 15) && (g.zlayers <= 1 || (!(g.zsA & 1) && !(g.zsB & 1) && !(g.zsC & 1)));
}
static int launch_mid_gemm(const GemmArgs& g, bool B_T, hipStream_t s) {
    const int nrb = g.Mr / MD_BM, ncb = (int)(g.Nc / MD_BN);
    const dim3 grid((unsigned)(nrb * ncb), 1, (unsigned)(g.zlayers > 1 ? g.zlayers : 1));
    if (tune().mid_gemm_waves == 32 && g.Kd % MS_BK == 0) {
        const int nrb32 = g.Mr / MS_BM;
        const dim3 grid32((unsigned)(nrb32 * ncb), 1, (unsigned)(g.zlayers > 1 ? g.zlayers : 1));
        if (B_T) hipLaunchKernelGGL(gemm_mid32_kernel<true>, grid32, dim3(256), 0, s, g, nrb32, ncb);
        else hipLaunchKernelGGL(gemm_mid32_kernel<false>, grid32, dim3(256), 0, s, g, nrb32, ncb);
    } else if (tune().mid_gemm_waves == 8) {
        if (B_T) hipLaunchKernelGGL(gemm_mid8_kernel<true>, grid, dim3(512), 0, s, g, nrb, ncb);
        else hipLaunchKernelGGL(gemm_mid8_kernel<false>, grid, dim3(512), 0, s, g, nrb, ncb);
    } else {
        if (B_T) hipLaunchKernelGGL(gemm_mid_kernel<true>, grid, dim3(256), 0, s, g, nrb, ncb);
        else hipLaunchKernelGGL(gemm_mid_kernel<false>, grid, dim3(256), 0, s, g, nrb, ncb);
    }
    return hipGetLastError() == hipSuccess ? MOBOCMF_OK : MOBOCMF_HIP_ERROR;
}

int launch_gemm_auto_pair(const GemmArgs& a, const GemmArgs& b, double* ws, int64_t ws_elems, hipStream_t s) {
    const int nza = a.zlayers > 1 ? a.zlayers : 1, nzb = b.zlayers > 1 ? b.zlayers : 1;
    GemmArgs a1 = a, b1 = b;
    a1.batched = b1.batched = 1;
    const bool small = small_gemm_ok(nza > 1 ? a1 : a, false) || small_gemm_ok(nzb > 1 ? b1 : b, false);
    if (small && nza == nzb && a.Mr == b.Mr && a.Nc == b.Nc && a.batched <= 1 && b.batched <= 1 &&
        small_gemm_ok(nza > 1 ? a1 : a, false) && small_gemm_ok(nzb > 1 ? b1 : b, false) && !a.skip_if_zero && !b.skip_if_zero) {
        GemmArgs x = nza > 1 ? a1 : a, y = nzb > 1 ? b1 : b;
        const dim3 grid((unsigned)(x.Nc / 16), (unsigned)(x.Mr / 16), (unsigned)(2 * nza));
        hipLaunchKernelGGL(small_gemm2_kernel, grid, dim3(256), 0, s, x, y);
        return hipGetLastError() == hipSuccess ? MOBOCMF_OK : MOBOCMF_HIP_ERROR;
    }
    if (!small && nza == nzb && a.Mr == b.Mr && a.Nc == b.Nc && a.batched <= 1 && b.batched <= 1 && mid_gemm_ok(a) && mid_gemm_ok(b)) {
        const int nrb = a.Mr / MD_BM, ncb = (int)(a.Nc / MD_BN);
        if (tune().mid_gemm_waves == 32 && a.Kd % MS_BK == 0 && b.Kd % MS_BK == 0)
            hipLaunchKernelGGL(gemm_mid32x2_kernel, dim3((unsigned)((a.Mr / MS_BM) * ncb), 2, (unsigned)nza), dim3(256), 0, s, a, b,
                               a.Mr / MS_BM, ncb);
        else if (tune().mid_gemm_waves == 8)
            hipLaunchKernelGGL(gemm_mid8x2_kernel, dim3((unsigned)(nrb * ncb), 2, (unsigned)nza), dim3(512), 0, s, a, b, nrb, ncb);
        else
            hipLaunchKernelGGL(gemm_mid2_kernel, dim3((unsigned)(nrb * ncb), 2, (unsigned)nza), dim3(256), 0, s, a, b, nrb, ncb);
        return hipGetLastError() == hipSuccess ? MOBOCMF_OK : MOBOCMF_HIP_ERROR;
    }
    int rc = launch_gemm_auto(a, false, ws, ws_elems, s);
    if (rc) return rc;
    return launch_gemm_auto(b, false, ws, ws_elems, s);
}

int launch_gemm_auto(const GemmArgs& g0, bool B_T, double* ws, int64_t ws_elems, hipStream_t s) {
    const int nz = g0.zlayers > 1 ? g0.zlayers : 1;
    if (nz > 1 && g0.batched > 1) return launch_gemm(g0, B_T, 1, s);
    if (nz > 1) {
        GemmArgs g1 = g0;
        g1.batched = 1;
        if (small_gemm_ok(g1, B_T)) return launch_small_gemm(g1, B_T, s);
    } else if (small_gemm_ok(g0, B_T)) return launch_small_gemm(g0, B_T, s);
    if (mid_gemm_ok(g0)) return launch_mid_gemm(g0, B_T, s);
    GemmArgs g = g0;
    const int nrb = g.Mr / BM;
    const int64_t ncb = g.Nc / BN;
    const int64_t ntile = g.lower_out ? (int64_t)nrb * (nrb + 1) / 2 : (int64_t)nrb * ncb;
    int64_t nk = g.Kd / BK;
    if (g.tri) nk = (nk + 1) / 2;
    int sk = 1;
    if (!g.batched && g.epi == EPI_STORE && ntile * nz < 96 * nz && ntile < 96 && nk >= 8) {
        sk = (int)(512 / (ntile * nz));
        if (sk > nk / 2) sk = (int)(nk / 2);
        if (sk >= 8) sk &= ~7;
        if ((int64_t)sk * g.Mr * g.Nc > ws_elems) sk = (int)(ws_elems / ((int64_t)g.Mr * g.Nc));
        if (sk >= 8) sk &= ~7;
    }
    if (sk < 2) {
        if (nz > 1) { g.batched = 1; return launch_gemm(g, B_T, 1, s); }
        return launch_gemm(g0, B_T, 1, s);
    }
    g.C = ws;
    g.ldc = g.Nc;
    g.slab_stride = (int64_t)g.Mr * g.Nc;
    g.accumulate = 0;
    int rc = launch_gemm(g, B_T, sk, s);
    if (rc) return rc;
    int64_t n = (int64_t)g.Mr * g.Nc;
    hipLaunchKernelGGL(reduce_slabs_kernel, dim3((unsigned)((n + 255) / 256), 1, (unsigned)nz), dim3(256), 0, s,
                       (const double*)ws, g.slab_stride, sk, g0.C, g0.ldc, g.Mr, g.Nc, 1.0, g0.lower_out, 0, g0.accumulate,
                       nz > 1 ? g0.zsC : (int64_t)0, nz > 1 ? g0.zsC : (int64_t)0);
    return hipGetLastError() == hipSuccess ? MOBOCMF_OK : MOBOCMF_HIP_ERROR;
}
```

mobocmf_amd/csrc/gram.hip:

```cpp
#include "common.h"

#define GT 128
#define GM 32


typedef double v2f64_t __attribute__((ext_vector_type(2)));

template <int KIND, int DB, int XD>
__global__ __launch_bounds__(GT) void gram_fwd_kernel(GramArgs g) {
    __shared__ __attribute__((aligned(16))) double stg[XD ? (GT / 64) * 64 * (XD + 2) : 1];
    __shared__ double zs[GM][DB];
    __shared__ double zfs[GM];
    __shared__ double il1[DB], il2[DB];
    const int d = g.d;
    const int tid = threadIdx.x;
    const int gm = g.gm;
    const int m0 = blockIdx.y * gm;
    const double* hyp = g.hyp;
    double a1, af = 0, nu = 0, a2 = 0, ilf = 0;
    if (KIND == 0) {
        a1 = hyp[0];
        if (tid < DB) il1[tid] = tid < d ? 1.0 / hyp[1 + tid] : 0.0;
    } else {
        a1 = hyp[0]; af = hyp[1]; nu = hyp[2]; a2 = hyp[3]; ilf = 1.0 / hyp[4];
        if (tid < DB) { il1[tid] = tid < d ? 1.0 / hyp[5 + tid] : 0.0; il2[tid] = tid < d ? 1.0 / hyp[5 + d + tid] : 0.0; }
    }
    for (int e = tid; e < gm * DB; e += GT) {
        int mm = e / DB, k = e % DB;
        int m = m0 + mm;
        zs[mm][k] = (m < g.M && k < d) ? g.Zx[(int64_t)(m / g.zdiv) * d + k] : 0.0;
    }
    if (KIND == 1 && tid < gm) zfs[tid] = (m0 + tid < g.M) ? g.zf[m0 + tid] : 0.0;
    __syncthreads();

    const int64_t n0 = (int64_t)blockIdx.x * GT + tid;
    const int xdiv = XD ? XD : g.xdiv;
    const int64_t c0 = n0 * xdiv;
    if (c0 >= g.Np) return;
    const bool real = n0 < g.nbase;
    double xr[DB];
#pragma unroll
    for (int k = 0; k < DB; ++k) xr[k] = (real && k < d) ? g.x[n0 * d + k] : 0.0;
    double fr[XD ? XD : 1];
    if (XD && KIND == 1) {
#pragma unroll
        for (int s = 0; s < XD; s += 2) {
            v2f64_t v = real ? *(const v2f64_t*)(g.f + c0 + s) : (v2f64_t){0.0, 0.0};
            fr[s] = v[0];
            fr[s + 1] = v[1];
        }
    }

    const bool full_wave = XD && __ballot(real) == ~0ull;
    (void)full_wave;
    if (g.knn && blockIdx.y == 0) {
        for (int s = 0; s < xdiv; ++s) {
            int64_t n = c0 + s;
            if (n >= g.Np) break;
            double v = 0.0;
            if (real) {
                if (KIND == 0) v = a1;
                else { double fn = g.f[n]; v = a1 * (nu * fn * fn + af) + a2; }
            }
            g.knn[n] = v;
        }
    }
    for (int mm = 0; mm < gm; ++mm) {
        const int m = m0 + mm;
        double* krow = g.K + (int64_t)m * g.ldk;
        if (!real || m >= g.M) {
            for (int s = 0; s < xdiv; ++s) {
                int64_t n = c0 + s;
                if (n >= g.Np) break;
                krow[n] = (g.is_kmm && n == m) ? 1.0 : 0.0;
            }
            continue;
        }
        double d1 = 0.0, d2 = 0.0;
#pragma unroll
        for (int k = 0; k < DB; ++k) {
            double df = xr[k] - zs[mm][k];
            double t1 = df * il1[k];
            d1 += t1 * t1;
            if (KIND == 1) { double t2 = df * il2[k]; d2 += t2 * t2; }
        }
        const double E1 = exp(-0.5 * d1);
        if (KIND == 0) {
            double v = a1 * E1;
            if (g.is_kmm && c0 == m) v += g.jitter;
            krow[c0] = v;
            for (int s = 1; s < xdiv; ++s) krow[c0 + s] = a1 * E1;
        } else if (XD) {
            const double E2 = exp(-0.5 * d2);
            const double zfm = zfs[mm];
            const double c1 = a1 * E1, c2 = a2 * E2;
            const double cp = c1 * nu * zfm, cq = c1 * af;
            const int lane = tid & 63;
            double* my = stg + (tid >> 6) * 64 * (XD + 2);
#pragma unroll
            for (int s = 0; s < XD; s += 2) {
                v2f64_t v;
#pragma unroll
                for (int e = 0; e < 2; ++e) {
                    const double fn = fr[s + e];
                    const double fd = (fn - zfm) * ilf;
                    v[e] = cq * exp(-0.5 * fd * fd) + (cp * fn + c2);
                }
                if (full_wave) *(v2f64_t*)(my + lane * (XD + 2) + s) = v;
                else *(v2f64_t*)(krow + c0 + s) = v;
            }
            if (full_wave) {
                double* wrow = krow + (c0 - (int64_t)lane * XD);
#pragma unroll
                for (int i = 0; i < XD / 2; ++i) {
                    const int e = (i * 64 + lane) * 2;
                    *(v2f64_t*)(wrow + e) = *(const v2f64_t*)(my + (e / XD) * (XD + 2) + e % XD);
                }
            }
        } else {
            const double E2 = exp(-0.5 * d2);
            const double zfm = zfs[mm];
            const double c1 = a1 * E1, c2 = a2 * E2;
            for (int s = 0; s < xdiv; ++s) {
                const int64_t n = c0 + s;
                const double fn = g.f[n];
                const double fd = (fn - zfm) * ilf;
                const double Ef = exp(-0.5 * fd * fd);
                double v = c1 * (nu * fn * zfm + af * Ef) + c2;
                if (g.is_kmm && n == m) v += g.jitter;
                krow[n] = v;
            }
        }
    }
}

__device__ __forceinline__ double wave_sum(double v) {
    v += __shfl_xor(v, 1);
    v += __shfl_xor(v, 2);
    v += __shfl_xor(v, 4);
    v += __shfl_xor(v, 8);
    v += __shfl_xor(v, 16);
    v += __shfl_xor(v, 32);
    return v;
}

template <int KIND, int DB, bool WANT_DX, int XD>
__global__ __launch_bounds__(GT) void gram_bwd_kernel(GramArgs g) {
    __shared__ double zs[GM][DB];
    __shared__ double zfs[GM];
    __shared__ double il1[DB], il2[DB];
    __shared__ double dzf_s[GM];
    __shared__ double red[2][8 + 2 * DB];
    extern __shared__ double dfs[];
    const int d = g.d;
    const int tid = threadIdx.x, lane = tid & 63, wave = tid >> 6;
    const int gm = g.gm;
    const int m0 = blockIdx.y * gm;
    const double* hyp = g.hyp;
    double a1, af = 0, nu = 0, a2 = 0, ilf = 0;
    if (KIND == 0) {
        a1 = hyp[0];
        if (tid < DB) il1[tid] = tid < d ? 1.0 / hyp[1 + tid] : 0.0;
    } else {
        a1 = hyp[0]; af = hyp[1]; nu = hyp[2]; a2 = hyp[3]; ilf = 1.0 / hyp[4];
        if (tid < DB) { il1[tid] = tid < d ? 1.0 / hyp[5 + tid] : 0.0; il2[tid] = tid < d ? 1.0 / hyp[5 + d + tid] : 0.0; }
    }
    for (int e = tid; e < gm * DB; e += GT) {
        int mm = e / DB, k = e % DB;
        int m = m0 + mm;
        zs[mm][k] = (m < g.M && k < d) ? g.Zx[(int64_t)(m / g.zdiv) * d + k] : 0.0;
// ... 370 lines not shown
```

Measured before the change: 1064.

## Fuse small chain kernels into GEMM epilogues and neighbouring launches

Several small launches are folded into neighbouring kernels. The dL and Phi elementwise steps become epilogues of the mid32 GEMM, and the symmetrize step rides in the chain-outputs kernel. KL partial sums are computed inside the transpose-gemv kernel, and the potrf sync-word memset is done by the last gram kernel. This removes launch overhead and extra memory passes per ELBO step, at the cost of more complex kernels and extra code paths that depend on tuning settings.

```diff
diff --git a/mobocmf_amd/csrc/api.hip b/mobocmf_amd/csrc/api.hip
--- a/mobocmf_amd/csrc/api.hip
+++ b/mobocmf_amd/csrc/api.hip
@@ -43,9 +43,12 @@
 int launch_mirror_lower(const double* src, int64_t lds, double* dst, int64_t ldd, int64_t row0, int64_t rows, int64_t cols,
                         int64_t n_real, hipStream_t s);
 int launch_potrf_z(double* A, int64_t ld, int Mp, int M, double* Dinv, double* Ld, int32_t* const* info, int nz, int64_t zs,
-                   double* zero0, double* zero1, void* sync, int* inverse_done, hipStream_t s);
+                   double* zero0, double* zero1, void* sync, bool sync_zeroed, int* inverse_done, hipStream_t s);
+bool potrf_uses_sync_words(int M);
+int64_t potrf_sync_bytes(int nz);
 int launch_chain_outputs_z(const double* X, const double* LSp, const double* LinvT, const double* da_tot, int M, int Mp,
-                           const double* const* gkl, double* const* gLS, double* const* gm, int nz, int64_t zs, hipStream_t s);
+                           const double* const* gkl, double* const* gLS, double* const* gm, const double* sym_in, double* sym_out,
+                           int nz, int64_t zs, hipStream_t s);
 int launch_pad_params_z(const double* const* LS, const double* const* m, int M, double* LSp, double* mp, int Mp, int nz,
                         int64_t zs, hipStream_t s);
 int launch_trtri_z(const double* L, int64_t ld, int Mp, const double* Dinv, double* Linv, double* T, double* ws,
@@ -56,12 +59,14 @@
                        int accumulate, int nz, int64_t zs, hipStream_t s);
 int launch_transpose_pad_z(const double* in, double* out, int Mp, const double* const* LS, const double* const* m, int M,
                            double* LSp, double* mp, int nz, int64_t zs, hipStream_t s);
-int launch_transpose_gemv_z(const double* in, double* out, int Mp, const double* Mat, const double* vec, double* vout, int nz,
-                            int64_t zs, hipStream_t s);
+int launch_transpose_gemv_z(const double* in, double* out, int Mp, const double* Mat, const double* vec, double* vout,
+                            const double* klL, const double* klLS, int M, double* klpart, int nz, int64_t zs, hipStream_t s);
+bool kl_rides_in_transpose(int M, int Mp);
 int launch_kl_z(const double* L, const double* LSp, const double* U, const double* a, int M, int Mp, double* const* kl,
-                double* part, int nz, int64_t zs, hipStream_t s);
+                double* part, bool parts_ready, int nz, int64_t zs, hipStream_t s);
 int launch_dutot_y_z(const double* G1, const double* G2, const double* Hc, const double* U, const double* da, const double* a,
-                     const double* const* gkl, int Mp, double* dU, double* da_tot, double* Y, int nz, int64_t zs, hipStream_t s);
+                     const double* const* gkl, int Mp, double* dU, double* da_tot, double* Y, const double* tr_in, double* tr_out,
+                     int nz, int64_t zs, hipStream_t s);
 int launch_dl_from_t2_z(const double* T2, const double* L, const double* const* gkl, int M, int Mp, double* dL, int nz,
                         int64_t zs, hipStream_t s);
 int launch_phi_z(const double* T3, int Mp, double* P, int nz, int64_t zs, hipStream_t s);
@@ -363,13 +368,15 @@
 int chain_forward(int n, const ChainWs& c, int64_t zs, const ChainIO& io, const Dims& D, hipStream_t s) {
     const int Mp = D.Mp;
     const int64_t mm = (int64_t)Mp * Mp;
+    const bool sync_fold = potrf_uses_sync_words(D.M);
     for (int z = 0; z < n; ++z) {
         GramArgs g = kmm_gram(io.desc[z], D, io.Zx[z], io.zf[z], io.hyp[z]);
         g.K = c.L + z * zs;
+        if (z == n - 1 && sync_fold) { g.zero_words = (unsigned long long*)c.ws; g.n_zero_words = (int)(potrf_sync_bytes(n) / 8); }
         TRY(launch_gram_fwd(g, s));
     }
     int inv_done = 0;
-    TRY(launch_potrf_z(c.L, Mp, Mp, D.M, c.Dinv, c.Ld, io.info, n, zs, c.Linv, c.U, c.ws, &inv_done, s));
+    TRY(launch_potrf_z(c.L, Mp, Mp, D.M, c.Dinv, c.Ld, io.info, n, zs, c.Linv, c.U, c.ws, sync_fold, &inv_done, s));
     if (!inv_done) TRY(launch_trtri_z(c.L, Mp, Mp, c.Dinv, c.Linv, c.T, c.ws, c.ws_elems, n, zs, s));
     TRY(launch_transpose_pad_z(c.Linv, c.LinvT, Mp, io.L_S, io.m, D.M, c.LSp, c.mp, n, zs, s));
     {
@@ -380,8 +387,9 @@
         if (n > 1) { gz.zlayers = n; gz.zsA = gz.zsB = gz.zsC = zs; }
         TRY(launch_gemm_auto(gz, false, c.ws, c.ws_elems, s));
     }
-    TRY(launch_transpose_gemv_z(c.U, c.UT, Mp, c.Linv, c.mp, c.a, n, zs, s));
-    TRY(launch_kl_z(c.L, c.LSp, c.U, c.a, D.M, Mp, io.kl, c.klpart, n, zs, s));
+    const bool klr = kl_rides_in_transpose(D.M, Mp);
+    TRY(launch_transpose_gemv_z(c.U, c.UT, Mp, c.Linv, c.mp, c.a, c.L, c.LSp, D.M, klr ? c.klpart : nullptr, n, zs, s));
+    TRY(launch_kl_z(c.L, c.LSp, c.U, c.a, D.M, Mp, io.kl, c.klpart, klr, n, zs, s));
     return MOBOCMF_OK;
 }
 
@@ -503,7 +511,7 @@
         GemmArgs g2 = gemm_args(c.U, Mp, G1, Mp, G2, Mp, Mp, Mp, Mp, TRI_LOWER_A, 1.0);
         g2.Kreal = D.M;
         TRY(chain_gemm(g2, false, c, n, zs, s));
-        TRY(launch_dutot_y_z(G1, G2, Hc, c.U, c.da, c.a, io.g_kl, Mp, dU, c.da_tot, Y, n, zs, s));
+        TRY(launch_dutot_y_z(G1, G2, Hc, c.U, c.da, c.a, io.g_kl, Mp, dU, c.da_tot, Y, c.L, LT, n, zs, s));
     }
     {
         GemmArgs g4 = gemm_args(dU, Mp, c.UT, Mp, Y, Mp, Mp, Mp, Mp, TRI_LOWER_A | TRI_UPPER_B, 1.0);
@@ -517,28 +525,43 @@
             g4.zsA = g4.zsB = g4.zsC = ga.zsA = ga.zsB = ga.zsC = zs;
         }
         TRY(launch_gemm_auto_pair(g4, ga, c.slabs, c.slab_elems, s));
-        TRY(launch_chain_outputs_z(T1, c.LSp, c.LinvT, c.da_tot, D.M, Mp, io.g_kl, io.g_LS, io.g_m, n, zs, s));
     }
     {
         GemmArgs ga = gemm_args(c.LinvT, Mp, Y, Mp, T2, Mp, Mp, Mp, Mp, TRI_UPPER_A, 1.0);
         ga.lower_out = 1;
         ga.Kreal = D.M;
-        TRY(chain_gemm(ga, false, c, n, zs, s));
-        TRY(launch_dl_from_t2_z(T2, c.L, io.g_kl, D.M, Mp, dL, n, zs, s));
+        if (n > 1) { ga.zlayers = n; ga.zsA = ga.zsB = ga.zsC = zs; }
+        if (gemm_takes_mid_epilogue(ga)) {
+            ga.C = dL;
+            ga.mid_epi = MID_EPI_DL; ga.epi_M = D.M; ga.epi_L = c.L;
+            for (int z = 0; z < n; ++z) ga.epi_gkl[z] = io.g_kl[z];
+            TRY(launch_gemm_auto(ga, false, c.slabs, c.slab_elems, s));
+        } else {
+            TRY(launch_gemm_auto(ga, false, c.slabs, c.slab_elems, s));
+            TRY(launch_dl_from_t2_z(T2, c.L, io.g_kl, D.M, Mp, dL, n, zs, s));
+        }
     }
     {
-        TRY(launch_transpose_z(c.L, Mp, LT, Mp, Mp, Mp, n, zs, s));
+        double* Phi = Y;
         GemmArgs ga = gemm_args(LT, Mp, dL, Mp, T2, Mp, Mp, Mp, Mp, TRI_UPPER_A | TRI_LOWER_B, 1.0);
         ga.Kreal = D.M;
-        TRY(chain_gemm(ga, false, c, n, zs, s));
-        TRY(launch_phi_z(T2, Mp, T1, n, zs, s));
-        GemmArgs gb = gemm_args(c.LinvT, Mp, T1, Mp, T4, Mp, Mp, Mp, Mp, TRI_UPPER_A | TRI_LOWER_B, 1.0);
+        if (n > 1) { ga.zlayers = n; ga.zsA = ga.zsB = ga.zsC = zs; }
+        if (gemm_takes_mid_epilogue(ga)) {
+            ga.C = Phi;
+            ga.mid_epi = MID_EPI_PHI;
+            ga.lower_out = 1;
+            TRY(launch_gemm_auto(ga, false, c.slabs, c.slab_elems, s));
+        } else {
+            TRY(launch_gemm_auto(ga, false, c.slabs, c.slab_elems, s));
+            TRY(launch_phi_z(T2, Mp, Phi, n, zs, s));
+        }
+        GemmArgs gb = gemm_args(c.LinvT, Mp, Phi, Mp, T4, Mp, Mp, Mp, Mp, TRI_UPPER_A | TRI_LOWER_B, 1.0);
         gb.Kreal = D.M;
         TRY(chain_gemm(gb, false, c, n, zs, s));
         GemmArgs gc = gemm_args(T4, Mp, c.Linv, Mp, T2, Mp, Mp, Mp, Mp, TRI_LOWER_B, 1.0);
         gc.Kreal = D.M;
         TRY(chain_gemm(gc, false, c, n, zs, s));
-        TRY(launch_symmetrize_z(T2, Mp, Gm, n, zs, s));
+        TRY(launch_chain_outputs_z(T1, c.LSp, c.LinvT, c.da_tot, D.M, Mp, io.g_kl, io.g_LS, io.g_m, T2, Gm, n, zs, s));
     }
     SumTask tk[2 * MAX_ZL];
     int nt = 0;
@@ -935,7 +958,7 @@
     TRY(launch_copy_pad_identity(K, ldk, n, S.L, np, s));
     TRY(launch_pad_vec(y, n, S.yp, np, s));
     int inv_done = 0;
-    TRY(launch_potrf_z(S.L, np, np, n, F.Dinv, F.Ld, &info, 1, 0, S.Linv, nullptr, F.ws, &inv_done, s));
+    TRY(launch_potrf_z(S.L, np, np, n, F.Dinv, F.Ld, &info, 1, 0, S.Linv, nullptr, F.ws, false, &inv_done, s));
     if (!inv_done) TRY(launch_trtri(S.L, np, np, F.Dinv, S.Linv, F.T, F.ws, F.ws_elems, s));
     TRY(launch_gemv_rows(S.Linv, np, S.yp, S.a, np, np, 1.0, 0, s));
     return launch_exact_gp_mll(S.L, np, S.a, n, mll, s);
@@ -1131,4 +1154,26 @@
     return h == 0 ? MOBOCMF_OK : MOBOCMF_NOT_PD;
 }
 
-}
+int mobocmf_debug_mid_epilogue(int32_t which, int32_t M, int32_t Mp, int32_t nz, const double* A, const double* B, const double* L,
+                               const double* const* gkl, double* fused, double* product, double* twostep,
+                               const mobocmf_tuning* tuning, mobocmf_stream_t stream) {
+    if ((which != MID_EPI_DL && which != MID_EPI_PHI) || M < 1 || M > Mp || Mp % TILE || nz < 1 || nz > MAX_ZL || !tuning_ok(tuning))
+        return MOBOCMF_BAD_ARG;
+    TuneScope tune_scope(tuning);
+    hipStream_t s = (hipStream_t)stream;
+    const int64_t zs = (int64_t)Mp * Mp;
+    GemmArgs g = gemm_args(A, Mp, B, Mp, product, Mp, Mp, Mp, Mp, which == MID_EPI_DL ? TRI_UPPER_A : TRI_UPPER_A | TRI_LOWER_B, 1.0);
+    g.Kreal = M;
+    g.lower_out = which == MID_EPI_DL ? 1 : 0;
+    if (nz > 1) { g.zlayers = nz; g.zsA = g.zsB = g.zsC = zs; }
+    if (!gemm_takes_mid_epilogue(g)) return MOBOCMF_BAD_ARG;
+    TRY(launch_gemm_auto(g, false, nullptr, 0, s));
+    if (which == MID_EPI_DL) TRY(launch_dl_from_t2_z(product, L, gkl, M, Mp, twostep, nz, zs, s));
+    else TRY(launch_phi_z(product, Mp, twostep, nz, zs, s));
+    GemmArgs f = g;
+    f.C = fused; f.mid_epi = which; f.lower_out = 1; f.epi_M = M; f.epi_L = L;
+    for (int z = 0; z < nz; ++z) f.epi_gkl[z] = gkl[z];
+    return launch_gemm_auto(f, false, nullptr, 0, s);
+}
+
+}
diff --git a/mobocmf_amd/csrc/chol.hip b/mobocmf_amd/csrc/chol.hip
--- a/mobocmf_amd/csrc/chol.hip
+++ b/mobocmf_amd/csrc/chol.hip
@@ -907,8 +907,13 @@
 }
 int64_t potrf_sync_bytes(int nz) { return (int64_t)nz * PC_WORDS * 8; }
 
+bool potrf_uses_sync_words(int M) {
+    const int nreal = (M + NB - 1) / NB;
+    return tune().potrf_cols == 0 && nreal >= 3 && nreal <= 16;
+}
+
 int launch_potrf_z(double* A, int64_t ld, int Mp, int M, double* Dinv, double* Ld, int32_t* const* info, int nz, int64_t zs,
-                   double* zero0, double* zero1, void* sync, int* inverse_done, hipStream_t s) {
+                   double* zero0, double* zero1, void* sync, bool sync_zeroed, int* inverse_done, hipStream_t s) {
     if (inverse_done) *inverse_done = 0;
     const int nblk = Mp / NB;
     const int nreal = (M + NB - 1) / NB;
@@ -925,7 +930,7 @@
         IlGuard gd;
         if (const int rc = il_guard((const void*)potrf_coop_kernel, PC_T, shm, (int)shm, gd)) return rc;
         if ((int64_t)G * nz <= gd.resident) {
-            HIP_TRY(hipMemsetAsync(sync, 0, (size_t)potrf_sync_bytes(nz), s));
+            if (!sync_zeroed) HIP_TRY(hipMemsetAsync(sync, 0, (size_t)potrf_sync_bytes(nz), s));
             hipLaunchKernelGGL(potrf_coop_kernel, dim3(G, nz), dim3(PC_T), shm, s, A, ld, nreal, Dinv, Ld, iz, zs,
                                (unsigned long long*)sync, Linv, Mp / NB, NT, gd.wait_ticks);
             one_launch = true;
@@ -956,7 +961,7 @@
 
 int launch_potrf(double* A, int64_t ld, int Mp, int M, double* Dinv, double* Ld, int32_t* info, hipStream_t s) {
     int32_t* one[1] = {info};
-    return launch_potrf_z(A, ld, Mp, M, Dinv, Ld, one, 1, 0, nullptr, nullptr, nullptr, nullptr, s);
+    return launch_potrf_z(A, ld, Mp, M, Dinv, Ld, one, 1, 0, nullptr, nullptr, nullptr, false, nullptr, s);
 }
 
 __global__ __launch_bounds__(256) void trtri_level0_kernel(const double* L, int64_t ld, const double* Dinv, double* Linv,
diff --git a/mobocmf_amd/csrc/common.h b/mobocmf_amd/csrc/common.h
--- a/mobocmf_amd/csrc/common.h
+++ b/mobocmf_amd/csrc/common.h
@@ -29,6 +29,8 @@
 
 enum { TRI_NONE = 0, TRI_LOWER_A = 1, TRI_UPPER_A = 2, TRI_LOWER_B = 4, TRI_UPPER_B = 8 };
 enum { EPI_STORE = 0, EPI_COLSTATS = 1, EPI_DA = 2 };
+enum { MID_EPI_NONE = 0, MID_EPI_DL = 1, MID_EPI_PHI = 2 };
+#define MAX_ZL 4
 
 struct GemmArgs {
     const double* A;
@@ -69,6 +71,10 @@
     const double* gmu;
     const double* cgv;
     const double* Aaux;
+    int mid_epi;
+    int epi_M;
+    const double* epi_L;
+    const double* epi_gkl[MAX_ZL];
 };
 
 int launch_gemm(const GemmArgs& g, bool B_T, int splitk, hipStream_t s);
@@ -84,13 +90,13 @@
 int gemm_rowdot_parts(const GemmArgs& g);
 int gemm_colstat_rows(const GemmArgs& g);
 int launch_gemm_auto(const GemmArgs& g, bool B_T, double* ws, int64_t ws_elems, hipStream_t s);
+bool gemm_takes_mid_epilogue(const GemmArgs& g);
 int launch_gemm_auto_pair(const GemmArgs& a, const GemmArgs& b, double* ws, int64_t ws_elems, hipStream_t s);
 int launch_reduce_slabs(const double* slabs, int64_t slab_stride, int nslab, double* out, int64_t ld, int Mr,
                         double scale, int lower_only, int accumulate, hipStream_t s);
 
 int launch_zero32(void* ptr, int64_t nwords, hipStream_t s);
 int launch_zero32_z(void* ptr, int64_t nwords, int nz, int64_t zs_bytes, hipStream_t s);
-#define MAX_ZL 4
 
 struct GramArgs {
     int kind, d, xdiv, zdiv;
@@ -116,6 +122,8 @@
     double* dzf_part;
     double* dx_part;
     const int32_t* colact;
+    unsigned long long* zero_words;
+    int n_zero_words;
 };
 
 static inline int hyp_len(int kind, int d) { return kind == 0 ? 1 + d : 5 + 2 * d; }
diff --git a/mobocmf_amd/csrc/elementwise.hip b/mobocmf_amd/csrc/elementwise.hip
--- a/mobocmf_amd/csrc/elementwise.hip
+++ b/mobocmf_amd/csrc/elementwise.hip
@@ -140,12 +140,28 @@
     return CHECK_LAUNCH();
 }
 __global__ void transpose_gemv_z_kernel(const double* in, double* out, int Mp, int64_t zs, const double* Mat, const double* vec,
-                                        double* vout) {
+                                        double* vout, const double* klL, const double* klLS, int M, double* klpart) {
     __shared__ double tl[32][33];
+    __shared__ double shk[4];
     const int z = blockIdx.z;
     in += z * zs; out += z * zs; Mat += z * zs; vec += z * zs; vout += z * zs;
     const int64_t c = (int64_t)blockIdx.x * 32 + threadIdx.x, r0 = (int64_t)blockIdx.y * 32;
-    for (int k = threadIdx.y; k < 32; k += 8) tl[k][threadIdx.x] = in[(r0 + k) * Mp + c];
+    double ks = 0.0;
+    for (int k = threadIdx.y; k < 32; k += 8) {
+        const double v = in[(r0 + k) * Mp + c];
+        tl[k][threadIdx.x] = v;
+        ks += (r0 + k < M && c <= r0 + k) ? v * v : 0.0;
+    }
+    if (klpart) {
+        const int tid = threadIdx.y * 32 + threadIdx.x;
+        if (blockIdx.x == blockIdx.y && threadIdx.y == 0 && r0 + threadIdx.x < M) {
+            const int64_t ii = (r0 + threadIdx.x) * (Mp + 1) + z * zs;
+            const double l = klL[ii], ls = klLS[ii];
+            ks += 2.0 * log(l) - log(ls * ls);
+        }
+        ks = wave_sum(ks);
+        if ((tid & 63) == 0) shk[tid >> 6] = ks;
+    }
     {
         const int tid = threadIdx.y * 32 + threadIdx.x, wave = tid >> 6, lane = tid & 63;
         const int nblk = gridDim.x * gridDim.y, b = blockIdx.y * gridDim.x + blockIdx.x;
@@ -158,13 +174,16 @@
         }
     }
     __syncthreads();
+    if (klpart && threadIdx.x == 0 && threadIdx.y == 0)
+        klpart[z * zs + blockIdx.y * gridDim.x + blockIdx.x] = (shk[0] + shk[1]) + (shk[2] + shk[3]);
     const int64_t r = r0 + threadIdx.x, c0 = (int64_t)blockIdx.x * 32;
     for (int k = threadIdx.y; k < 32; k += 8) out[(c0 + k) * Mp + r] = tl[threadIdx.x][k];
 }
-int launch_transpose_gemv_z(const double* in, double* out, int Mp, const double* Mat, const double* vec, double* vout, int nz,
-                            int64_t zs, hipStream_t s) {
+bool kl_rides_in_transpose(int M, int Mp) { return M > 128 && (int64_t)(Mp / 32) * (Mp / 32) <= Mp; }
+int launch_transpose_gemv_z(const double* in, double* out, int Mp, const double* Mat, const double* vec, double* vout,
+                            const double* klL, const double* klLS, int M, double* klpart, int nz, int64_t zs, hipStream_t s) {
     hipLaunchKernelGGL(transpose_gemv_z_kernel, dim3((unsigned)(Mp / 32), (unsigned)(Mp / 32), (unsigned)nz), dim3(32, 8), 0, s, in,
-                       out, Mp, zs, Mat, vec, vout);
+                       out, Mp, zs, Mat, vec, vout, klL, klLS, M, klpart);
     return CHECK_LAUNCH();
 }
 int launch_transpose(const double* in, int64_t ldi, double* out, int64_t ldo, int64_t rows, int64_t cols, hipStream_t s) {
@@ -214,11 +233,15 @@
     if (threadIdx.x == 0) part[blockIdx.x] = s;
 }
 struct KlZ { double* p[MAX_ZL]; };
-__global__ void kl_final_kernel(const double* part, int np, int M, KlZ kl, int64_t zs) {
+__global__ void kl_final_kernel(const double* part, int np, int M, KlZ kl, int64_t zs, const double* a) {
     __shared__ double sh[4];
     double s = 0.0;
     part += blockIdx.x * zs;
     for (int i = threadIdx.x; i < np; i += 256) s += part[i];
+    if (a) {
+        a += blockIdx.x * zs;
+        for (int i = threadIdx.x; i < M; i += 256) s += a[i] * a[i];
+    }
     s = block_sum(s, sh);
     if (threadIdx.x == 0) kl.p[blockIdx.x][0] = 0.5 * (s - (double)M);
 }
@@ -249,7 +272,13 @@
     }
 }
 int launch_kl_z(const double* L, const double* LSp, const double* U, const double* a, int M, int Mp, double* const* kl,
-                double* part, int nz, int64_t zs, hipStream_t s) {
+                double* part, bool parts_ready, int nz, int64_t zs, hipStream_t s) {
+    if (parts_ready) {
+        KlZ kz = {};
+        for (int z = 0; z < nz; ++z) kz.p[z] = kl[z];
+        hipLaunchKernelGGL(kl_final_kernel, dim3(nz), dim3(256), 0, s, (const double*)part, (Mp / 32) * (Mp / 32), M, kz, zs, a);
+        return CHECK_LAUNCH();
+    }
     if (M <= 128) {
         KlZ kz1 = {};
         for (int z = 0; z < nz; ++z) kz1.p[z] = kl[z];
@@ -260,13 +289,13 @@
     hipLaunchKernelGGL(kl_part_kernel, dim3(nb, 1, nz), dim3(256), 0, s, L, LSp, U, a, M, Mp, part, zs);
     KlZ kz = {};
     for (int z = 0; z < nz; ++z) kz.p[z] = kl[z];
-    hipLaunchKernelGGL(kl_final_kernel, dim3(nz), dim3(256), 0, s, (const double*)part, nb, M, kz, zs);
+    hipLaunchKernelGGL(kl_final_kernel, dim3(nz), dim3(256), 0, s, (const double*)part, nb, M, kz, zs, (const double*)nullptr);
     return CHECK_LAUNCH();
 }
 int launch_kl(const double* L, const double* LSp, const double* U, const double* a, int M, int Mp, double* kl,
               double* part, hipStream_t s) {
     double* one[1] = {kl};
-    return launch_kl_z(L, LSp, U, a, M, Mp, one, part, 1, 0, s);
+    return launch_kl_z(L, LSp, U, a, M, Mp, one, part, false, 1, 0, s);
 }
 
 __global__ void moments_finish_kernel(const double* qpart, const double* mupart, const double* rpart, int nrb,
@@ -397,14 +426,24 @@
 }
 
 __global__ void dutot_y_kernel(const double* G1, const double* G2, const double* Hc, const double* U, const double* da,
-                               const double* a, ScalZ gklz, int Mp, double* dU, double* da_tot, double* Y, int64_t zs) {
+                               const double* a, ScalZ gklz, int Mp, double* dU, double* da_tot, double* Y, int64_t zs,
+                               const double* tr_in, double* tr_out) {
     __shared__ double tl[32][33];
+    const int64_t zo = blockIdx.z * zs;
+    const int nt = Mp / 32, ti = blockIdx.x / nt, tj = blockIdx.x % nt;
+    const int tx = threadIdx.x & 31, ty = threadIdx.x >> 5;
+    if (blockIdx.y == 1) {
+        tr_in += zo; tr_out += zo;
+#pragma unroll
+        for (int r = ty; r < 32; r += 8) tl[r][tx] = tr_in[(int64_t)(ti * 32 + r) * Mp + tj * 32 + tx];
+        __syncthreads();
+#pragma unroll
+        for (int r = ty; r < 32; r += 8) tr_out[(int64_t)(tj * 32 + r) * Mp + ti * 32 + tx] = tl[tx][r];
+        return;
+    }
     const double* gkl = gklz.p[blockIdx.z];
     const double g = gkl ? gkl[0] : 0.0;
-    const int64_t zo = blockIdx.z * zs;
     G1 += zo; G2 += zo; Hc += zo; U += zo; da += zo; a += zo; dU += zo; da_tot += zo; Y += zo;
-    const int nt = Mp / 32, ti = blockIdx.x / nt, tj = blockIdx.x % nt;
-    const int tx = threadIdx.x & 31, ty = threadIdx.x >> 5;
     if (tj <= ti) {
 #pragma unroll
         for (int r = ty; r < 32; r += 8) tl[r][tx] = G1[(int64_t)(tj * 32 + r) * Mp + ti * 32 + tx];
@@ -421,12 +460,13 @@
     }
 }
 int launch_dutot_y_z(const double* G1, const double* G2, const double* Hc, const double* U, const double* da, const double* a,
-                     const double* const* gkl, int Mp, double* dU, double* da_tot, double* Y, int nz, int64_t zs, hipStream_t s) {
+                     const double* const* gkl, int Mp, double* dU, double* da_tot, double* Y, const double* tr_in, double* tr_out,
+                     int nz, int64_t zs, hipStream_t s) {
     ScalZ t = {};
     for (int z = 0; z < nz; ++z) t.p[z] = gkl[z];
     const int nt = Mp / 32;
-    hipLaunchKernelGGL(dutot_y_kernel, dim3((unsigned)(nt * nt), 1, (unsigned)nz), dim3(256), 0, s, G1, G2, Hc, U, da, a, t, Mp,
-                       dU, da_tot, Y, zs);
+    hipLaunchKernelGGL(dutot_y_kernel, dim3((unsigned)(nt * nt), tr_in ? 2 : 1, (unsigned)nz), dim3(256), 0, s, G1, G2, Hc, U, da,
+                       a, t, Mp, dU, da_tot, Y, zs, tr_in, tr_out);
     return CHECK_LAUNCH();
 }
 
@@ -522,8 +562,16 @@
 
 struct ChainOutZ { const double* gkl[MAX_ZL]; double* gLS[MAX_ZL]; double* gm[MAX_ZL]; };
 __global__ void chain_outputs_z_kernel(const double* X, const double* LSp, const double* LinvT, const double* da_tot, int M,
-                                       int Mp, ChainOutZ t, int nb_ls, int64_t zs) {
+                                       int Mp, ChainOutZ t, int nb_ls, int nb_m, int64_t zs, const double* sym_in, double* sym_out) {
     const int z = blockIdx.y;
+    if ((int)blockIdx.x >= nb_ls + nb_m) {
+        const int64_t idx = (int64_t)((int)blockIdx.x - nb_ls - nb_m) * blockDim.x + threadIdx.x;
+        if (idx >= (int64_t)Mp * Mp) return;
+        sym_in += z * zs; sym_out += z * zs;
+        const int i = (int)(idx / Mp), j = (int)(idx % Mp);
+        sym_out[idx] = 0.5 * (sym_in[idx] + sym_in[(int64_t)j * Mp + i]);
+        return;
+    }
     X += z * zs; LSp += z * zs; LinvT += z * zs; da_tot += z * zs;
     if ((int)blockIdx.x < nb_ls) {
         const int64_t idx = (int64_t)blockIdx.x * blockDim.x + threadIdx.x;
@@ -546,12 +594,14 @@
     if (lane == 0) t.gm[z][row] = sacc;
 }
 int launch_chain_outputs_z(const double* X, const double* LSp, const double* LinvT, const double* da_tot, int M, int Mp,
-                           const double* const* gkl, double* const* gLS, double* const* gm, int nz, int64_t zs, hipStream_t s) {
+                           const double* const* gkl, double* const* gLS, double* const* gm, const double* sym_in, double* sym_out,
+                           int nz, int64_t zs, hipStream_t s) {
     ChainOutZ t = {};
     for (int z = 0; z < nz; ++z) { t.gkl[z] = gkl[z]; t.gLS[z] = gLS[z]; t.gm[z] = gm[z]; }
     const int nb_ls = (int)(((int64_t)M * M + 255) / 256), nb_m = (M + 3) / 4;
-    hipLaunchKernelGGL(chain_outputs_z_kernel, dim3((unsigned)(nb_ls + nb_m), (unsigned)nz), dim3(256), 0, s, X, LSp, LinvT, da_tot,
-                       M, Mp, t, nb_ls, zs);
+    const int nb_sym = sym_in ? (int)(((int64_t)Mp * Mp + 255) / 256) : 0;
+    hipLaunchKernelGGL(chain_outputs_z_kernel, dim3((unsigned)(nb_ls + nb_m + nb_sym), (unsigned)nz), dim3(256), 0, s, X, LSp, LinvT,
+                       da_tot, M, Mp, t, nb_ls, nb_m, zs, sym_in, sym_out);
     return CHECK_LAUNCH();
 }
 
diff --git a/mobocmf_amd/csrc/gemm_f64.hip b/mobocmf_amd/csrc/gemm_f64.hip
--- a/mobocmf_amd/csrc/gemm_f64.hip
+++ b/mobocmf_amd/csrc/gemm_f64.hip
@@ -1332,18 +1332,39 @@
 #define MS_BK 64
 #define MS_LDA (MS_BK + 2)
 #define MS_ASWZ(row) ((((row) & 1) << 1) | ((((row) >> 1) & 1) << 4))
-template <bool B_T>
+template <bool B_T, int MEPI = MID_EPI_NONE>
 __device__ __forceinline__ void gemm_mid32_body(const GemmArgs& g, int nrb, int ncb) {
     __shared__ __attribute__((aligned(16))) double As[MS_BM * MS_BK];
     __shared__ __attribute__((aligned(16))) double Bs[B_T ? MD_BN * MS_LDA : MS_BK * MD_LDB];
     const int tid = threadIdx.x, lane = tid & 63, wave = tid >> 6;
     const int wr = wave >> 1, wc = wave & 1, li = lane & 15, lk = lane >> 4;
     const int rb = nrb - 1 - (int)(blockIdx.x / ncb), cb = (int)(blockIdx.x % ncb);
-    if (g.lower_out && cb > (rb >> 1 | 1)) return;
     const int z = blockIdx.z;
+    double* C = g.C + (g.zlayers > 1 ? z * g.zsC : 0);
+    double* cp = C + ((int64_t)rb * MS_BM + wr * 16 + lk) * g.ldc + (int64_t)cb * MD_BN + wc * 32 + 2 * li;
+    if (g.lower_out && cb > (rb >> 1 | 1)) {
+        if (MEPI) {
+#pragma unroll
+            for (int r = 0; r < 4; ++r) *(v2f64*)(cp + (int64_t)(4 * r) * g.ldc) = (v2f64){0.0, 0.0};
+        }
+        return;
+    }
     const double* A = g.A + (g.zlayers > 1 ? z * g.zsA : 0);
     const double* B = g.B + (g.zlayers > 1 ? z * g.zsB : 0);
-    double* C = g.C + (g.zlayers > 1 ? z * g.zsC : 0);
+    double epi_gk = 0.0, epi_lii[4] = {1.0, 1.0, 1.0, 1.0};
+    bool epi_has_gk = false;
+    if (MEPI == MID_EPI_DL && g.epi_gkl[z]) {
+        epi_has_gk = true;
+        epi_gk = g.epi_gkl[z][0];
+        if ((rb >> 1) == cb) {
+            const double* Lz = g.epi_L + (g.zlayers > 1 ? z * g.zsC : 0);
+#pragma unroll
+            for (int r = 0; r < 4; ++r) {
+                const int i = rb * MS_BM + wr * 16 + 4 * r + lk;
+                if (i < g.epi_M) epi_lii[r] = Lz[(int64_t)i * g.ldc + i];
+            }
+        }
+    }
     int64_t k0 = 0, k1 = g.Kd;
     if (g.Kreal > 0) { const int64_t ke = (g.Kreal + MS_BK - 1) / MS_BK * MS_BK; if (k1 > ke) k1 = ke; }
     if (g.tri & TRI_LOWER_A) { const int64_t e = (int64_t)(rb / 2 + 1) * 64; if (k1 > e) k1 = e; }
@@ -1417,7 +1438,30 @@
             __builtin_amdgcn_sched_barrier(0);
         }
     }
-    double* cp = C + ((int64_t)rb * MS_BM + wr * 16 + lk) * g.ldc + (int64_t)cb * MD_BN + wc * 32 + 2 * li;
+    if (MEPI) {
+        const int j0 = cb * MD_BN + wc * 32 + 2 * li;
+#pragma unroll
+        for (int r = 0; r < 4; ++r) {
+            const int i = rb * MS_BM + wr * 16 + 4 * r + lk;
+            double v[2];
+#pragma unroll
+            for (int nt = 0; nt < 2; ++nt) {
+                const int j = j0 + nt;
+                const double t = __dmul_rn(g.alpha, acc[nt][r]);
+                if (MEPI == MID_EPI_DL) {
+                    v[nt] = 0.0;
+                    if (i < g.epi_M && j <= i) {
+                        v[nt] = -t;
+                        if (i == j && epi_has_gk) v[nt] += epi_gk / epi_lii[r];
+                    }
+                } else {
+                    v[nt] = j < i ? t : (j == i ? 0.5 * t : 0.0);
+                }
+            }
+            *(v2f64*)(cp + (int64_t)(4 * r) * g.ldc) = (v2f64){v[0], v[1]};
+        }
+        return;
+    }
 #pragma unroll
     for (int r = 0; r < 4; ++r) {
         double* q = cp + (int64_t)(4 * r) * g.ldc;
@@ -1429,6 +1473,10 @@
 template <bool B_T>
 __global__ __launch_bounds__(256) void gemm_mid32_kernel(GemmArgs g, int nrb, int ncb) {
     gemm_mid32_body<B_T>(g, nrb, ncb);
+}
+template <int MEPI>
+__global__ __launch_bounds__(256) void gemm_mid32_epi_kernel(GemmArgs g, int nrb, int ncb) {
+    gemm_mid32_body<false, MEPI>(g, nrb, ncb);
 }
 __global__ __launch_bounds__(256) void gemm_mid32x2_kernel(GemmArgs g0, GemmArgs g1, int nrb, int ncb) {
     if (blockIdx.y == 0) gemm_mid32_body<false>(g0, nrb, ncb);
@@ -1459,13 +1507,23 @@
            !(g.lda & 1) && !(g.ldb & 1) && !(g.ldc & 1) && !((uintptr_t)g.A & 15) && !((uintptr_t)g.B & 15) &&
            !((uintptr_t)g.C & 15) && (g.zlayers <= 1 || (!(g.zsA & 1) && !(g.zsB & 1) && !(g.zsC & 1)));
 }
+static bool mid32_form(const GemmArgs& g) { return tune().mid_gemm_waves == 32 && g.Kd % MS_BK == 0; }
+bool gemm_takes_mid_epilogue(const GemmArgs& g) {
+    if (g.batched > 1 || g.accumulate) return false;
+    GemmArgs g1 = g;
+    if (g.zlayers > 1) g1.batched = 1;
+    return !small_gemm_ok(g1, false) && mid_gemm_ok(g) && mid32_form(g);
+}
 static int launch_mid_gemm(const GemmArgs& g, bool B_T, hipStream_t s) {
+    if (g.mid_epi && (!mid32_form(g) || g.accumulate || B_T)) return MOBOCMF_BAD_ARG;
     const int nrb = g.Mr / MD_BM, ncb = (int)(g.Nc / MD_BN);
     const dim3 grid((unsigned)(nrb * ncb), 1, (unsigned)(g.zlayers > 1 ? g.zlayers : 1));
     if (tune().mid_gemm_waves == 32 && g.Kd % MS_BK == 0) {
         const int nrb32 = g.Mr / MS_BM;
         const dim3 grid32((unsigned)(nrb32 * ncb), 1, (unsigned)(g.zlayers > 1 ? g.zlayers : 1));
-        if (B_T) hipLaunchKernelGGL(gemm_mid32_kernel<true>, grid32, dim3(256), 0, s, g, nrb32, ncb);
+        if (g.mid_epi == MID_EPI_DL) hipLaunchKernelGGL(gemm_mid32_epi_kernel<MID_EPI_DL>, grid32, dim3(256), 0, s, g, nrb32, ncb);
+        else if (g.mid_epi == MID_EPI_PHI) hipLaunchKernelGGL(gemm_mid32_epi_kernel<MID_EPI_PHI>, grid32, dim3(256), 0, s, g, nrb32, ncb);
+        else if (B_T) hipLaunchKernelGGL(gemm_mid32_kernel<true>, grid32, dim3(256), 0, s, g, nrb32, ncb);
         else hipLaunchKernelGGL(gemm_mid32_kernel<false>, grid32, dim3(256), 0, s, g, nrb32, ncb);
     } else if (tune().mid_gemm_waves == 8) {
         if (B_T) hipLaunchKernelGGL(gemm_mid8_kernel<true>, grid, dim3(512), 0, s, g, nrb, ncb);
@@ -1507,6 +1565,7 @@
 
 int launch_gemm_auto(const GemmArgs& g0, bool B_T, double* ws, int64_t ws_elems, hipStream_t s) {
     const int nz = g0.zlayers > 1 ? g0.zlayers : 1;
+    if (g0.mid_epi && (B_T || !gemm_takes_mid_epilogue(g0))) return MOBOCMF_BAD_ARG;
     if (nz > 1 && g0.batched > 1) return launch_gemm(g0, B_T, 1, s);
     if (nz > 1) {
         GemmArgs g1 = g0;
diff --git a/mobocmf_amd/csrc/gram.hip b/mobocmf_amd/csrc/gram.hip
--- a/mobocmf_amd/csrc/gram.hip
+++ b/mobocmf_amd/csrc/gram.hip
@@ -16,6 +16,8 @@
     const int tid = threadIdx.x;
     const int gm = g.gm;
     const int m0 = blockIdx.y * gm;
+    if (g.zero_words && blockIdx.x == 0 && blockIdx.y == 0)
+        for (int e = tid; e < g.n_zero_words; e += GT) g.zero_words[e] = 0ull;
     const double* hyp = g.hyp;
     double a1, af = 0, nu = 0, a2 = 0, ilf = 0;
     if (KIND == 0) {
```

Result: no change. 1073, median of 6 (+0.8%).
